# Scoobadood/TSDF

Hardware: AMD Instinct MI355X
Metric: Mvoxels/s integrate + Mrays/s raycast, 512^3 grid, 640x480 depth; 1/2/4/8 GPU (higher is better)
Workload: dtype f32

## Files before the change

### include/tsdf_amd.h

```cpp
#ifndef TSDF_AMD_H
#define TSDF_AMD_H

#include <stddef.h>
#include <stdint.h>

#ifdef __cplusplus
extern "C" {
#endif

#define TSDF_OK 0
#define TSDF_ERR_INVALID 1
#define TSDF_ERR_DEVICE 2
#define TSDF_ERR_NOMEM 3

typedef struct tsdf_volume tsdf_volume;
typedef struct tsdf_bilateral tsdf_bilateral;
typedef struct tsdf_icp tsdf_icp;

typedef struct tsdf_volume_info {
    uint32_t size[3];
    uint32_t z_begin, z_end;
    uint32_t z_store_begin, z_store_end;
    float physical_size[3];
    float voxel_size[3];
// ... 2 lines not shown
    float truncation_distance;
    float max_weight;
    float global_translation[3];
    float global_rotation[3];
    int32_t deformation_materialised;
    int32_t fast_division_verified;
} tsdf_volume_info;

typedef struct tsdf_deformation_node {
    float translation[3];
    float rotation[3];
} tsdf_deformation_node;

const char *tsdf_last_error(void);
int tsdf_device_count(int *count);
int tsdf_set_device(int device);
int tsdf_get_device(int *device);
const char *tsdf_build_arch(void);

int tsdf_device_alloc(size_t bytes, void **device_ptr);
int tsdf_device_free(void *device_ptr);
int tsdf_device_upload(void *device_dst, const void *host_src, size_t bytes);
int tsdf_device_download(void *host_dst, const void *device_src, size_t bytes);
int tsdf_stream_synchronize(void *hip_stream);

int tsdf_volume_create(uint32_t size_x, uint32_t size_y, uint32_t size_z, float physical_x,
                       float physical_y, float physical_z, tsdf_volume **out);
int tsdf_volume_create_slab(uint32_t size_x, uint32_t size_y, uint32_t size_z, float physical_x,
                            float physical_y, float physical_z, uint32_t z_begin, uint32_t z_end,
                            tsdf_volume **out);
int tsdf_volume_destroy(tsdf_volume *volume);
int tsdf_volume_set_stream(tsdf_volume *volume, void *hip_stream);
int tsdf_volume_stream(const tsdf_volume *volume, void **hip_stream);
int tsdf_volume_synchronize(const tsdf_volume *volume);
int tsdf_volume_clear(tsdf_volume *volume);
int tsdf_volume_get_info(const tsdf_volume *volume, tsdf_volume_info *info);
int tsdf_volume_set_offset(tsdf_volume *volume, float ox, float oy, float oz);

int tsdf_volume_set_header(tsdf_volume *volume, const float offset[3], float truncation_distance,
                           float max_weight, const float global_translation[3],
                           const float global_rotation[3]);

int tsdf_volume_distances(const tsdf_volume *volume, float **device_ptr);
int tsdf_volume_mark_dirty(tsdf_volume *volume);
int tsdf_volume_weights(const tsdf_volume *volume, float **device_ptr);
int tsdf_volume_weight_storage(const tsdf_volume *volume, int *bits_per_weight, int *pinned);
int tsdf_volume_set_weight_storage(tsdf_volume *volume, int bits_per_weight);
int tsdf_selftest_count_division(uint32_t b_begin, uint32_t b_end, unsigned long long *mismatches);
int tsdf_volume_deformation(tsdf_volume *volume, tsdf_deformation_node **device_ptr);
int tsdf_volume_set_distance_data(tsdf_volume *volume, const float *host);
int tsdf_volume_set_weight_data(tsdf_volume *volume, const float *host);
int tsdf_volume_set_deformation(tsdf_volume *volume, const tsdf_deformation_node *host);
int tsdf_volume_deform_points(const tsdf_volume *volume, int num_points, float *host_points);
int tsdf_volume_deform_points_device(const tsdf_volume *volume, int num_points, float *device_points);
int tsdf_volume_get_distance_data(const tsdf_volume *volume, float *host);
int tsdf_volume_get_weight_data(const tsdf_volume *volume, float *host);
int tsdf_volume_get_deformation_planes(const tsdf_volume *volume, uint32_t plane_begin, uint32_t plane_count,
                                       tsdf_deformation_node *host);
int tsdf_volume_set_offset_at_clear(tsdf_volume *volume, const float offset_at_clear[3]);

int tsdf_integrate(tsdf_volume *volume, const uint16_t *host_depth, uint32_t width, uint32_t height,
                   const float pose[16], const float inv_pose[16], const float k[9], const float kinv[9]);
int tsdf_integrate_device(tsdf_volume *volume, const uint16_t *device_depth, uint32_t width,
                          uint32_t height, const float pose[16], const float inv_pose[16],
                          const float k[9], const float kinv[9]);
int tsdf_integrate_device_tiles(tsdf_volume *volume, const uint16_t *device_depth, uint32_t width,
                                uint32_t height, const float pose[16], const float inv_pose[16],
                                const float k[9], const float kinv[9], const uint16_t *device_tile_max);
int tsdf_integrate_prepare_device_tiles(tsdf_volume *volume, const uint16_t *device_depth, uint32_t width,
                                        uint32_t height, const float pose[16], const float inv_pose[16],
                                        const float k[9], const float kinv[9], const uint16_t *device_tile_max,
                                        void *hip_stream);
int tsdf_integrate_discard_prepared(tsdf_volume *volume);
int tsdf_volume_set_timing(tsdf_volume *volume, int enabled);
int tsdf_volume_kernel_time(tsdf_volume *volume, int which, uint32_t *launches, float *average_ms);

int tsdf_volume_set_counting(tsdf_volume *volume, int enabled);
int tsdf_volume_last_updated_voxels(const tsdf_volume *volume, uint64_t *count);

int tsdf_raycast(const tsdf_volume *volume, uint32_t width, uint32_t height, const float pose[16],
                 const float kinv[9], float *host_vertices, float *host_normals);
int tsdf_raycast_device(const tsdf_volume *volume, uint32_t width, uint32_t height,
                        const float pose[16], const float kinv[9], float *device_vertices,
                        float *device_normals);
int tsdf_normals_device(uint32_t width, uint32_t height, const float *device_vertices,
                        float *device_normals, void *hip_stream);
int tsdf_vertices_to_depth_device(uint32_t width, uint32_t height, const float *device_vertices,
                                  const float inv_pose[16], uint16_t *device_depth, void *hip_stream);
int tsdf_raycast_depth_device(const tsdf_volume *volume, uint32_t width, uint32_t height, const float pose[16],
                              const float inv_pose[16], const float kinv[9], uint16_t *device_depth, float *device_vertices);
int tsdf_volume_last_raycast_kind(const tsdf_volume *volume, int *cell_parallel);
int tsdf_volume_last_cell_list(const tsdf_volume *volume, uint32_t *listed);
int tsdf_raycast_stats(const tsdf_volume *volume, uint32_t width, uint32_t height, const float pose[16],
                       const float kinv[9], uint64_t *samples, uint64_t *touched_voxels, uint64_t *hits);

int tsdf_raycast_evaluated_samples(const tsdf_volume *volume, uint32_t width, uint32_t height,
                                   const float pose[16], const float kinv[9], uint64_t *evaluated,
                                   float *host_per_ray );
int tsdf_volume_occupancy(const tsdf_volume *volume, uint64_t *occupied_bricks, uint64_t *total_bricks);
int tsdf_volume_get_occupancy_data(const tsdf_volume *volume, int force_rebuild, uint8_t *host_fine, uint8_t *host_cell,
                                   uint8_t *host_reach);

int tsdf_volume_marching_cubes(const tsdf_volume *volume, const int8_t *table, uint64_t *n_vertices, float *host_vertices,
                               uint64_t capacity);

#define TSDF_NO_HIT 0xffffffffu
typedef struct tsdf_hit_record {
    uint32_t k;
    float t;
} tsdf_hit_record;
int tsdf_raycast_slab_device(const tsdf_volume *volume, uint32_t width, uint32_t height,
                             const float pose[16], const float kinv[9], tsdf_hit_record *device_hits);
int tsdf_merge_hits_device(const tsdf_volume *volume, const tsdf_hit_record *device_hits_all, uint32_t n_slabs,
                           uint32_t width, uint32_t height, const float pose[16], const float kinv[9],
                           float *device_vertices, void *hip_stream);
int tsdf_merge_hits_normals_device(const tsdf_volume *volume, const tsdf_hit_record *device_hits_all, uint32_t n_slabs,
                                   uint32_t width, uint32_t height, const float pose[16], const float kinv[9],
                                   float *device_vertices, float *device_normals, void *hip_stream);

typedef struct tsdf_slab_exchange tsdf_slab_exchange;
#define TSDF_EXCHANGE_ID_BYTES 128
int tsdf_slab_exchange_unique_id(uint8_t id[TSDF_EXCHANGE_ID_BYTES], const char *rccl_library);
int tsdf_slab_exchange_create(int rank, int world, const uint8_t id[TSDF_EXCHANGE_ID_BYTES], const char *rccl_library,
                              tsdf_slab_exchange **out);
typedef int (*tsdf_exchange_fn)(void *user, const tsdf_hit_record *device_mine, tsdf_hit_record *device_all, uint32_t n_pixels,
                                void *hip_stream);
int tsdf_slab_exchange_create_callback(int rank, int world, tsdf_exchange_fn all_gather, void *user, tsdf_slab_exchange **out);
int tsdf_slab_exchange_create_loopback(int rank, int world, tsdf_slab_exchange **out);
int tsdf_slab_exchange_world(const tsdf_slab_exchange *exchange, int *rank, int *world);
int tsdf_slab_exchange_ranks_seen(const tsdf_slab_exchange *exchange, int *ranks);
int tsdf_slab_validate_merge(tsdf_volume *slab_volume, tsdf_slab_exchange *exchange, uint32_t width, uint32_t height,
                             const float pose[16], const float kinv[9], const float *device_merged_vertices,
                             const float *device_merged_normals, uint64_t *differing_words);
int tsdf_slab_exchange_all_gather(tsdf_slab_exchange *exchange, const tsdf_hit_record *device_mine, tsdf_hit_record *device_all,
                                  uint32_t n_pixels, void *hip_stream);
int tsdf_slab_exchange_destroy(tsdf_slab_exchange *exchange);

typedef struct tsdf_pipeline tsdf_pipeline;
typedef struct tsdf_camera_matrices {
    float pose[16], inv_pose[16], k[9], kinv[9];
} tsdf_camera_matrices;
#define TSDF_PIPELINE_OVERLAP 1
#define TSDF_PIPELINE_EQUAL_PRIORITY 2
#define TSDF_PIPELINE_EXCHANGE_STREAM 4
#define TSDF_PIPELINE_NO_TIGHTEN_AHEAD 8
int tsdf_pipeline_create(tsdf_volume *volume, const tsdf_bilateral *filter, uint32_t width, uint32_t height, int flags,
                         tsdf_slab_exchange *exchange , tsdf_pipeline **out);
int tsdf_pipeline_step(tsdf_pipeline *pipeline, const uint16_t *device_depth, const tsdf_camera_matrices *camera,
                       float *device_vertices, float *device_normals, const uint16_t *next_device_depth ,
                       const tsdf_camera_matrices *next_camera );
int tsdf_pipeline_synchronize(tsdf_pipeline *pipeline);
int tsdf_pipeline_streams(const tsdf_pipeline *pipeline, void **main_stream, void **side_stream);
int tsdf_pipeline_hit_buffers(const tsdf_pipeline *pipeline, tsdf_hit_record **device_mine, tsdf_hit_record **device_all);
int tsdf_pipeline_destroy(tsdf_pipeline *pipeline);

typedef struct tsdf_tracker tsdf_tracker;
int tsdf_tracker_create(tsdf_volume *volume, const tsdf_bilateral *filter, tsdf_icp *icp, uint32_t width, uint32_t height,
                        float depth_cutoff, int flags , tsdf_tracker **out);
int tsdf_tracker_filter(tsdf_tracker *tracker, const uint16_t *device_depth);
int tsdf_tracker_align(tsdf_tracker *tracker, const tsdf_camera_matrices *previous, double T_prev_curr[16] ,
                       float *last_error, float *last_inliers);
int tsdf_tracker_integrate(tsdf_tracker *tracker, const tsdf_camera_matrices *camera);
int tsdf_tracker_synchronize(tsdf_tracker *tracker);
int tsdf_tracker_streams(const tsdf_tracker *tracker, void **main_stream, void **side_stream);
int tsdf_tracker_buffers(const tsdf_tracker *tracker, const uint16_t **device_model, const uint16_t **device_filtered);
int tsdf_tracker_destroy(tsdf_tracker *tracker);

int tsdf_icp_create(int width, int height, float cx, float cy, float fx, float fy, float dist_thresh, float angle_thresh,
                    tsdf_icp **out);
void tsdf_icp_destroy(tsdf_icp *icp);
int tsdf_icp_set_stream(tsdf_icp *icp, void *hip_stream);
int tsdf_icp_stream(const tsdf_icp *icp, void **hip_stream);
int tsdf_icp_init(tsdf_icp *icp, int model, const uint16_t *host_depth, float depth_cutoff);
int tsdf_icp_init_device(tsdf_icp *icp, int model, const uint16_t *device_depth, float depth_cutoff);
int tsdf_icp_estimate_step(tsdf_icp *icp, int level, const float R[9], const float t[3], float A[36], float b[6],
                           float residual_inliers[2]);
int tsdf_icp_get_incremental_transformation(tsdf_icp *icp, double T_prev_curr[16], float *last_error, float *last_inliers);
int tsdf_icp_get_map(const tsdf_icp *icp, int which, int level, float *host_map);
int tsdf_icp_get_depth_level(const tsdf_icp *icp, int level, uint16_t *host_depth);

int tsdf_bilateral_create(float sigma_colour, float sigma_space, tsdf_bilateral **out);
int tsdf_bilateral_destroy(tsdf_bilateral *filter);
int tsdf_bilateral_filter_u8(const tsdf_bilateral *filter, uint8_t *host_image, int width, int height);
int tsdf_bilateral_filter_u16(const tsdf_bilateral *filter, uint16_t *host_image, int width, int height);
int tsdf_bilateral_filter_u8_device(const tsdf_bilateral *filter, const uint8_t *device_in,
                                    uint8_t *device_out, int width, int height, void *hip_stream);
int tsdf_bilateral_filter_u16_device(const tsdf_bilateral *filter, const uint16_t *device_in,
                                     uint16_t *device_out, int width, int height, void *hip_stream);
#define TSDF_DEPTH_TILE 16
int tsdf_bilateral_filter_u16_device_tiles(const tsdf_bilateral *filter, const uint16_t *device_in,
                                           uint16_t *device_out, int width, int height,
                                           uint16_t *device_tile_max, void *hip_stream);

int tsdf_measure_copy_bandwidth(size_t bytes, int reps, void *hip_stream, double *gb_per_s);
int tsdf_measure_update_bandwidth(int reps, void *hip_stream, double *gb_per_s);

#ifdef __cplusplus
}
#endif
#endif
```

### tsdf_amd/_capi.py

```python
import ctypes as C
import os

_HERE = os.path.dirname(os.path.abspath(__file__))
LIB_PATH = os.environ.get("TSDF_HIP_LIB") or os.path.join(_HERE, "lib", "libtsdf_hip.so")

TSDF_OK, TSDF_ERR_INVALID, TSDF_ERR_DEVICE, TSDF_ERR_NOMEM = 0, 1, 2, 3


class TsdfError(RuntimeError):
    """A C-ABI call failed with TSDF_ERR_DEVICE / TSDF_ERR_NOMEM."""


class VolumeInfo(C.Structure):
    _fields_ = [("size", C.c_uint32 * 3), ("z_begin", C.c_uint32), ("z_end", C.c_uint32),
                ("z_store_begin", C.c_uint32), ("z_store_end", C.c_uint32),
                ("physical_size", C.c_float * 3), ("voxel_size", C.c_float * 3), ("offset", C.c_float * 3),
                ("offset_at_clear", C.c_float * 3), ("truncation_distance", C.c_float),
                ("max_weight", C.c_float), ("global_translation", C.c_float * 3),
                ("global_rotation", C.c_float * 3), ("deformation_materialised", C.c_int32),
                ("fast_division_verified", C.c_int32)]


class CameraMatrices(C.Structure):
    _fields_ = [("pose", C.c_float * 16), ("inv_pose", C.c_float * 16), ("k", C.c_float * 9), ("kinv", C.c_float * 9)]


EXCHANGE_FN = C.CFUNCTYPE(C.c_int, C.c_void_p, C.c_void_p, C.c_void_p, C.c_uint32, C.c_void_p)


def _load():
    if not os.path.exists(LIB_PATH):
        raise ImportError(
            "tsdf_amd: %s is missing -- build it with `make hip` (or `python -c 'import __graft_entry__ as g; "
            "g.build()'`). There is no CPU fallback." % LIB_PATH)
    return C.CDLL(LIB_PATH, mode=C.RTLD_GLOBAL)


lib = _load()

_vp, _fp = C.c_void_p, C.POINTER(C.c_float)
_u32, _f, _i = C.c_uint32, C.c_float, C.c_int
_SIGS = {
    "tsdf_last_error": (C.c_char_p, []),
    "tsdf_build_arch": (C.c_char_p, []),
    "tsdf_device_count": (_i, [C.POINTER(_i)]),
    "tsdf_set_device": (_i, [_i]),
    "tsdf_get_device": (_i, [C.POINTER(_i)]),
    "tsdf_device_alloc": (_i, [C.c_size_t, C.POINTER(_vp)]),
    "tsdf_device_free": (_i, [_vp]),
    "tsdf_device_upload": (_i, [_vp, _vp, C.c_size_t]),
    "tsdf_device_download": (_i, [_vp, _vp, C.c_size_t]),
    "tsdf_stream_synchronize": (_i, [_vp]),
    "tsdf_volume_create": (_i, [_u32, _u32, _u32, _f, _f, _f, C.POINTER(_vp)]),
    "tsdf_volume_create_slab": (_i, [_u32, _u32, _u32, _f, _f, _f, _u32, _u32, C.POINTER(_vp)]),
    "tsdf_volume_destroy": (_i, [_vp]),
    "tsdf_volume_set_stream": (_i, [_vp, _vp]),
    "tsdf_volume_stream": (_i, [_vp, C.POINTER(_vp)]),
    "tsdf_volume_synchronize": (_i, [_vp]),
    "tsdf_volume_clear": (_i, [_vp]),
    "tsdf_volume_get_info": (_i, [_vp, C.POINTER(VolumeInfo)]),
    "tsdf_volume_set_offset": (_i, [_vp, _f, _f, _f]),
    "tsdf_volume_set_header": (_i, [_vp, _fp, _f, _f, _fp, _fp]),
    "tsdf_volume_mark_dirty": (_i, [_vp]),
    "tsdf_volume_distances": (_i, [_vp, C.POINTER(_vp)]),
    "tsdf_volume_weights": (_i, [_vp, C.POINTER(_vp)]),
    "tsdf_volume_weight_storage": (_i, [_vp, C.POINTER(_i), C.POINTER(_i)]),
    "tsdf_volume_last_raycast_kind": (_i, [_vp, C.POINTER(_i)]),
    "tsdf_volume_last_cell_list": (_i, [_vp, C.POINTER(C.c_uint32)]),
    "tsdf_volume_set_weight_storage": (_i, [_vp, _i]),
    "tsdf_selftest_count_division": (_i, [_u32, _u32, C.POINTER(C.c_uint64)]),
    "tsdf_volume_deformation": (_i, [_vp, C.POINTER(_vp)]),
    "tsdf_volume_set_distance_data": (_i, [_vp, _vp]),
    "tsdf_volume_set_weight_data": (_i, [_vp, _vp]),
    "tsdf_volume_set_deformation": (_i, [_vp, _vp]),
    "tsdf_volume_get_distance_data": (_i, [_vp, _vp]),
    "tsdf_measure_copy_bandwidth": (_i, [C.c_size_t, _i, _vp, C.POINTER(C.c_double)]),
    "tsdf_measure_update_bandwidth": (_i, [_i, _vp, C.POINTER(C.c_double)]),
    "tsdf_volume_get_weight_data": (_i, [_vp, _vp]),
    "tsdf_volume_get_deformation_planes": (_i, [_vp, C.c_uint32, C.c_uint32, _vp]),
    "tsdf_volume_set_offset_at_clear": (_i, [_vp, _vp]),
    "tsdf_integrate": (_i, [_vp, _vp, _u32, _u32, _fp, _fp, _fp, _fp]),
    "tsdf_integrate_device": (_i, [_vp, _vp, _u32, _u32, _fp, _fp, _fp, _fp]),
    "tsdf_integrate_device_tiles": (_i, [_vp, _vp, _u32, _u32, _fp, _fp, _fp, _fp, _vp]),
    "tsdf_integrate_prepare_device_tiles": (_i, [_vp, _vp, _u32, _u32, _fp, _fp, _fp, _fp, _vp, _vp]),
    "tsdf_integrate_discard_prepared": (_i, [_vp]),
    "tsdf_volume_set_timing": (_i, [_vp, _i]),
    "tsdf_volume_kernel_time": (_i, [_vp, _i, C.POINTER(C.c_uint32), C.POINTER(C.c_float)]),
    "tsdf_volume_set_counting": (_i, [_vp, _i]),
    "tsdf_volume_last_updated_voxels": (_i, [_vp, C.POINTER(C.c_uint64)]),
    "tsdf_raycast": (_i, [_vp, _u32, _u32, _fp, _fp, _vp, _vp]),
    "tsdf_raycast_device": (_i, [_vp, _u32, _u32, _fp, _fp, _vp, _vp]),
    "tsdf_normals_device": (_i, [_u32, _u32, _vp, _vp, _vp]),
    "tsdf_raycast_stats": (_i, [_vp, _u32, _u32, _fp, _fp, C.POINTER(C.c_uint64), C.POINTER(C.c_uint64),
                                C.POINTER(C.c_uint64)]),
    "tsdf_raycast_evaluated_samples": (_i, [_vp, _u32, _u32, _fp, _fp, C.POINTER(C.c_uint64), _vp]),
    "tsdf_volume_deform_points": (_i, [_vp, _i, _vp]),
    "tsdf_volume_deform_points_device": (_i, [_vp, _i, _vp]),
    "tsdf_volume_occupancy": (_i, [_vp, C.POINTER(C.c_uint64), C.POINTER(C.c_uint64)]),
    "tsdf_volume_get_occupancy_data": (_i, [_vp, C.c_int, _vp, _vp, _vp]),
    "tsdf_raycast_slab_device": (_i, [_vp, _u32, _u32, _fp, _fp, _vp]),
    "tsdf_vertices_to_depth_device": (_i, [_u32, _u32, _vp, _vp, _vp, _vp]),
    "tsdf_raycast_depth_device": (_i, [_vp, _u32, _u32, _fp, _fp, _fp, _vp, _vp]),
    "tsdf_volume_marching_cubes": (_i, [_vp, _vp, _vp, _vp, C.c_uint64]),
    "tsdf_merge_hits_device": (_i, [_vp, _vp, _u32, _u32, _u32, _fp, _fp, _vp, _vp]),
    "tsdf_merge_hits_normals_device": (_i, [_vp, _vp, _u32, _u32, _u32, _fp, _fp, _vp, _vp, _vp]),
    "tsdf_slab_exchange_unique_id": (_i, [_vp, C.c_char_p]),
    "tsdf_slab_exchange_create": (_i, [_i, _i, _vp, C.c_char_p, C.POINTER(_vp)]),
    "tsdf_slab_exchange_create_callback": (_i, [_i, _i, EXCHANGE_FN, _vp, C.POINTER(_vp)]),
    "tsdf_slab_exchange_create_loopback": (_i, [_i, _i, C.POINTER(_vp)]),
    "tsdf_slab_exchange_world": (_i, [_vp, C.POINTER(_i), C.POINTER(_i)]),
    "tsdf_slab_exchange_ranks_seen": (_i, [_vp, C.POINTER(_i)]),
    "tsdf_slab_validate_merge": (_i, [_vp, _vp, _u32, _u32, _fp, _fp, _vp, _vp, C.POINTER(C.c_uint64)]),
    "tsdf_slab_exchange_all_gather": (_i, [_vp, _vp, _vp, _u32, _vp]),
    "tsdf_slab_exchange_destroy": (_i, [_vp]),
    "tsdf_pipeline_create": (_i, [_vp, _vp, _u32, _u32, _i, _vp, C.POINTER(_vp)]),
    "tsdf_pipeline_step": (_i, [_vp, _vp, C.POINTER(CameraMatrices), _vp, _vp, _vp, C.POINTER(CameraMatrices)]),
    "tsdf_pipeline_synchronize": (_i, [_vp]),
    "tsdf_pipeline_streams": (_i, [_vp, C.POINTER(_vp), C.POINTER(_vp)]),
    "tsdf_pipeline_hit_buffers": (_i, [_vp, C.POINTER(_vp), C.POINTER(_vp)]),
    "tsdf_pipeline_destroy": (_i, [_vp]),
    "tsdf_tracker_create": (_i, [_vp, _vp, _vp, _u32, _u32, _f, _i, C.POINTER(_vp)]),
    "tsdf_tracker_filter": (_i, [_vp, _vp]),
    "tsdf_tracker_align": (_i, [_vp, C.POINTER(CameraMatrices), _vp, C.POINTER(C.c_float), C.POINTER(C.c_float)]),
    "tsdf_tracker_integrate": (_i, [_vp, C.POINTER(CameraMatrices)]),
    "tsdf_tracker_synchronize": (_i, [_vp]),
    "tsdf_tracker_streams": (_i, [_vp, C.POINTER(_vp), C.POINTER(_vp)]),
    "tsdf_tracker_buffers": (_i, [_vp, C.POINTER(_vp), C.POINTER(_vp)]),
    "tsdf_tracker_destroy": (_i, [_vp]),
    "tsdf_icp_create": (_i, [_i, _i, _f, _f, _f, _f, _f, _f, C.POINTER(_vp)]),
    "tsdf_icp_destroy": (None, [_vp]),
    "tsdf_icp_set_stream": (_i, [_vp, _vp]),
    "tsdf_icp_stream": (_i, [_vp, C.POINTER(_vp)]),
    "tsdf_icp_init": (_i, [_vp, _i, _vp, _f]),
    "tsdf_icp_init_device": (_i, [_vp, _i, _vp, _f]),
    "tsdf_icp_estimate_step": (_i, [_vp, _i, _vp, _vp, _vp, _vp, _vp]),
    "tsdf_icp_get_incremental_transformation": (_i, [_vp, _vp, C.POINTER(C.c_float), C.POINTER(C.c_float)]),
    "tsdf_icp_get_map": (_i, [_vp, _i, _i, _vp]),
    "tsdf_icp_get_depth_level": (_i, [_vp, _i, _vp]),
    "tsdf_bilateral_create": (_i, [_f, _f, C.POINTER(_vp)]),
    "tsdf_bilateral_destroy": (_i, [_vp]),
    "tsdf_bilateral_filter_u8": (_i, [_vp, _vp, _i, _i]),
    "tsdf_bilateral_filter_u16": (_i, [_vp, _vp, _i, _i]),
    "tsdf_bilateral_filter_u8_device": (_i, [_vp, _vp, _vp, _i, _i, _vp]),
    "tsdf_bilateral_filter_u16_device": (_i, [_vp, _vp, _vp, _i, _i, _vp]),
    "tsdf_bilateral_filter_u16_device_tiles": (_i, [_vp, _vp, _vp, _i, _i, _vp, _vp]),
}
EXPORTS = tuple(_SIGS)
for _name, (_res, _args) in _SIGS.items():
    _fn = getattr(lib, _name)
    _fn.restype = _res
    _fn.argtypes = _args


def last_error():
    return lib.tsdf_last_error().decode("utf-8", "replace")


def check(rc):
    if rc == TSDF_OK:
        return
    msg = last_error()
    if rc == TSDF_ERR_INVALID:
        raise ValueError(msg)
    if rc == TSDF_ERR_NOMEM:
        raise MemoryError(msg)
    raise TsdfError(msg)

HOST_LIB_PATH = os.path.join(_HERE, "lib", "libtsdf_host.so")
if not os.path.exists(HOST_LIB_PATH):
    raise ImportError("tsdf_amd: %s is missing -- build it with `make host`." % HOST_LIB_PATH)
host = C.CDLL(HOST_LIB_PATH)
_ip = C.POINTER(C.c_int)
_HOST_SIGS = {
    "tsdf_camera_create": (_vp, [_f, _f, _f, _f]),
    "tsdf_camera_destroy": (None, [_vp]),
    "tsdf_camera_get": (None, [_vp, _fp, _fp, _fp, _fp]),
    "tsdf_camera_set_pose": (None, [_vp, _fp]),
    "tsdf_camera_set_pose_tum": (None, [_vp, _fp]),
    "tsdf_camera_move_to": (None, [_vp, _f, _f, _f]),
    "tsdf_camera_look_at": (None, [_vp, _f, _f, _f]),
    "tsdf_camera_world_to_camera": (None, [_vp, _fp, _fp]),
    "tsdf_camera_camera_to_world": (None, [_vp, _fp, _fp]),
    "tsdf_camera_world_to_pixel": (None, [_vp, _fp, _ip]),
    "tsdf_camera_pixel_to_image_plane": (None, [_vp, C.c_uint16, C.c_uint16, _fp]),
    "tsdf_camera_image_plane_to_pixel": (None, [_vp, _fp, _ip]),
    "tsdf_host_marching_cubes_c": (C.c_size_t, [_vp, C.c_uint, C.c_uint, C.c_uint, _vp, _vp, _vp, C.c_size_t]),
    "tsdf_host_mc_table": (None, [_vp]),
    "tsdf_host_tum_open": (_vp, [C.c_char_p]),
    "tsdf_host_tum_next": (_i, [_vp, _vp, C.c_size_t, C.POINTER(C.c_uint), _fp]),
    "tsdf_host_tum_close": (None, [_vp]),
    "tsdf_host_block_loader_parse": (_i, [C.c_char_p, _vp, _vp, _vp, _vp, C.c_size_t]),
    "tsdf_host_write_ply": (None, [C.c_char_p, _vp, C.c_size_t, _vp, C.c_size_t]),
    "tsdf_host_read_nyu_depth_map": (C.c_size_t, [C.c_char_p, C.POINTER(C.c_uint), _vp, C.c_size_t]),
    "tsdf_host_match_file_name": (_i, [C.c_char_p, _i, C.c_char_p, C.c_char_p, C.c_char_p]),
    "tsdf_host_process_file_by_lines": (C.c_size_t, [C.c_char_p, C.POINTER(_i), C.c_char_p, C.c_size_t]),
    "tsdf_host_read_last_line": (C.c_size_t, [C.c_char_p, C.c_char_p, C.POINTER(_i), C.c_char_p, C.c_size_t]),
    "tsdf_host_files_in_directory": (C.c_size_t, [C.c_char_p, C.c_char_p, _i, C.c_char_p, C.c_char_p, C.c_char_p, C.c_size_t]),
    "tsdf_host_file_exists": (_i, [C.c_char_p, C.POINTER(_i)]),
}
for _name, (_res, _args) in _HOST_SIGS.items():
    _fn = getattr(host, _name)
    _fn.restype = _res
    _fn.argtypes = _args
```

### tsdf_amd/csrc/bilateral.hip

```cpp
#include <cmath>
#include <cstdlib>
#include <new>
#include <type_traits>
#include <vector>

#include "common.hpp"

namespace tsdf {

constexpr int kBTile = 16;
constexpr int kMaxRadius = 24;

constexpr int kSimLds = 4096;

__device__ inline void bilateral_tap(float weight, double intensity, float &sum, float &total_weight) {
    sum = (float)__builtin_fma((double)weight, intensity, (double)sum);
    total_weight = total_weight + weight;
}

__device__ inline unsigned sad_u32(unsigned a, unsigned b) {
    unsigned d;
    asm("v_sad_u32 %0, %1, %2, 0" : "=v"(d) : "v"(a), "v"(b));
    return d;
}

template <typename PIX, int R>
__global__ __launch_bounds__(256) void bilateral_kernel(const PIX *__restrict__ in, PIX *__restrict__ out,
                                                        int width, int height, int radius_arg,
                                                        const float *__restrict__ kernel,
                                                        const float *__restrict__ similarity,
                                                        uint16_t *__restrict__ tile_max) {
    constexpr bool STAGED = R > 0;
    __shared__ unsigned wg_max;
    if (threadIdx.x == 0) wg_max = 0u;
    extern __shared__ __align__(16) unsigned char smem_raw[];
    const int radius = R > 0 ? R : radius_arg;
    const int n = 2 * radius + 1;
    const int span = kBTile + 2 * radius;
    double *tile_d = reinterpret_cast<double *>(smem_raw);
    float *kern_lds = reinterpret_cast<float *>(tile_d + (STAGED ? 0 : span * span));
    float *sim_lds = kern_lds + n * n;
    uint32_t *tile4 = reinterpret_cast<uint32_t *>(sim_lds + (STAGED ? kSimLds : 0));
    const int tx0 = blockIdx.x * kBTile - radius;
    const int ty0 = blockIdx.y * kBTile - radius;
    {
        constexpr int kAhead = 4;
        for (int i0 = threadIdx.x; i0 < span * span; i0 += 256 * kAhead) {
            unsigned v_[kAhead];
#pragma unroll
            for (int u = 0; u < kAhead; u++) {
                const int i = min(i0 + u * 256, span * span - 1);
                const int ly = i / span, lx = i - ly * span;
                const int gx = min(max(tx0 + lx, 0), width - 1), gy = min(max(ty0 + ly, 0), height - 1);
                v_[u] = in[(size_t)gy * width + gx];
            }
#pragma unroll
            for (int u = 0; u < kAhead; u++) {
                const int i = i0 + u * 256;
                const int ly = i / span, lx = i - ly * span;
                const int gx = tx0 + lx, gy = ty0 + ly;
                const unsigned v = (gx >= 0 && gx < width && gy >= 0 && gy < height) ? v_[u] : 0u;
                if (i < span * span) {
                    tile4[i] = v * 4u;
                    if (!STAGED) tile_d[i] = (double)(int)v;
                }
            }
        }
    }
    {
        const int n_sim = !STAGED ? 0 : (sizeof(PIX) == 1 ? 256 : kSimLds);
        constexpr int kAhead = 16;
        float k_ = 0.0f;
        if ((int)threadIdx.x < n * n) k_ = kernel[threadIdx.x];
        for (int i0 = threadIdx.x; i0 < n_sim; i0 += 256 * kAhead) {
            float s_[kAhead];
#pragma unroll
            for (int u = 0; u < kAhead; u++) s_[u] = similarity[min(i0 + u * 256, n_sim - 1)];
#pragma unroll
            for (int u = 0; u < kAhead; u++)
                if (i0 + u * 256 < n_sim) sim_lds[i0 + u * 256] = s_[u];
        }
        if ((int)threadIdx.x < n * n) kern_lds[threadIdx.x] = k_;
        for (int i = threadIdx.x + 256; i < n * n; i += 256) kern_lds[i] = kernel[i];
    }
    __syncthreads();

    const int lx = threadIdx.x & 15, ly = threadIdx.x >> 4;
    const int x = blockIdx.x * kBTile + lx;
    const int y = blockIdx.y * kBTile + ly;
    const uint32_t *t0 = tile4 + ly * span + lx;
    const double *d0 = tile_d + ly * span + lx;
    const unsigned current4 = t0[radius * span + radius];
    float total_weight = 0;
    float sum = 0;
    const int wy0 = (blockIdx.y * kBTile + (ly & ~3)) - radius;
    const bool interior = tx0 >= 0 && tx0 + span <= width && wy0 >= 0 && wy0 + 4 + 2 * radius <= height;
    const bool inside = x < width && y < height;
    const int i0 = max(0, radius - x), i1 = inside ? min(n - 1, width - 1 - x + radius) : -1;
    const int j0 = max(0, radius - y), j1 = inside ? min(n - 1, height - 1 - y + radius) : -1;
    const int nyv = j1 - j0 + 1;

    if (STAGED) {
        constexpr int N = 2 * (R > 0 ? R : 1) + 1;
        constexpr int SPAN = kBTile + 2 * (R > 0 ? R : 1);
        constexpr unsigned kStagedBytes = (sizeof(PIX) == 1 ? 256u : (unsigned)kSimLds) * 4u;
        constexpr int NA = (N + 1) / 2, NB = N - NA;
        float w_a[NA], w_b[NB > 0 ? NB : 1];
        unsigned v_a[NA], v_b[NB > 0 ? NB : 1];
        auto fetch = [&](const int i, auto first_row, auto count, float *w, unsigned *v4, const auto rim) {
            constexpr int J0 = decltype(first_row)::value, CNT = decltype(count)::value;
            unsigned delta4[CNT];
#pragma unroll
            for (int j = 0; j < CNT; j++) {
                v4[j] = t0[(J0 + j) * SPAN + i];
                delta4[j] = sad_u32(v4[j], current4);
            }
#pragma unroll
            for (int j = 0; j < CNT; j++)
                w[j] = *reinterpret_cast<const float *>(reinterpret_cast<const char *>(sim_lds) + delta4[j]);
            if (sizeof(PIX) != 1) {
                unsigned big = delta4[0];
#pragma unroll
                for (int j = 1; j < CNT; j++) big = max(big, delta4[j]);
                if (__builtin_expect(big >= kStagedBytes, 0)) {
#pragma unroll
                    for (int j = 0; j < CNT; j++)
                        if (delta4[j] >= kStagedBytes) {
                            const char *p = reinterpret_cast<const char *>(similarity) + delta4[j];
                            asm volatile("global_load_dword %0, %1, off\n\ts_waitcnt vmcnt(0)" : "=v"(w[j]) : "v"(p) : "memory");
                        }
                }
            }
            if (!decltype(rim)::value) {
#pragma unroll
                for (int j = 0; j < CNT; j++) w[j] = kernel[i * N + J0 + j] * w[j];
            } else {
                const bool col_ok = i >= i0 && i <= i1;
                const int base = (i - i0) * nyv - j0;
#pragma unroll
                for (int j = 0; j < CNT; j++) {
                    const bool ok = col_ok && J0 + j >= j0 && J0 + j <= j1;
                    const float k = kern_lds[(base + J0 + j) & (ok ? 255 : 0)];
                    w[j] = __builtin_bit_cast(float, __builtin_bit_cast(unsigned, k * w[j]) & (ok ? 0xffffffffu : 0u));
                }
            }
        };
        auto chain = [&](const int i, auto first_row, auto count, const float *w, const unsigned *v4) {
            constexpr int CNT = decltype(count)::value;
            (void)i;
#pragma unroll
            for (int j = 0; j < CNT; j++) bilateral_tap(w[j], (double)v4[j], sum, total_weight);
        };
        using Lo = std::integral_constant<int, 0>;
        using Hi = std::integral_constant<int, NA>;
        using CntA = std::integral_constant<int, NA>;
        using CntB = std::integral_constant<int, NB>;
        auto run = [&](const auto rim) {
            fetch(0, Lo{}, CntA{}, w_a, v_a, rim);
#pragma unroll 1
            for (int i = 0; i + 1 < N; i++) {
                fetch(i, Hi{}, CntB{}, w_b, v_b, rim);
                chain(i, Lo{}, CntA{}, w_a, v_a);
                fetch(i + 1, Lo{}, CntA{}, w_a, v_a, rim);
                chain(i, Hi{}, CntB{}, w_b, v_b);
            }
            fetch(N - 1, Hi{}, CntB{}, w_b, v_b, rim);
            chain(N - 1, Lo{}, CntA{}, w_a, v_a);
            chain(N - 1, Hi{}, CntB{}, w_b, v_b);
        };
        if (interior) {
            run(std::false_type{});
        } else {
            __builtin_amdgcn_s_setprio(3);
            run(std::true_type{});
        }
        sum *= 0.25f;
    } else {
#pragma unroll 1
        for (int i = 0; i < n; i++) {
            const bool col_ok = i >= i0 && i <= i1;
            const int base = (i - i0) * nyv - j0;
#pragma unroll 1
            for (int j = 0; j < n; j++) {
                const int o = j * span + i;
                const bool ok = col_ok && j >= j0 && j <= j1;
                const unsigned delta = sad_u32(t0[o], current4) >> 2;
                const float k = kern_lds[ok ? base + j : 0];
                const float weight = ok ? k * similarity[delta] : 0.0f;
                bilateral_tap(weight, d0[o], sum, total_weight);
            }
        }
    }
    const PIX filtered = inside ? (PIX)(int)floorf(sum / total_weight) : (PIX)0;
    if (inside) out[(size_t)y * width + x] = filtered;
    if (tile_max) {
        unsigned m = (unsigned)filtered;
        for (int o = 32; o > 0; o >>= 1) m = max(m, (unsigned)__shfl_down((int)m, o));
        if ((threadIdx.x & 63) == 0 && m) atomicMax(&wg_max, m);
        __syncthreads();
        if (threadIdx.x == 0) tile_max[blockIdx.y * gridDim.x + blockIdx.x] = (uint16_t)wg_max;
    }
}

template <typename PIX>
static int launch_bilateral(const tsdf_bilateral *f, const PIX *in, PIX *out, int width, int height, hipStream_t s,
                            uint16_t *tile_max = nullptr) {
    dim3 grid((width + kBTile - 1) / kBTile, (height + kBTile - 1) / kBTile);
    const int span = kBTile + 2 * f->radius, n = 2 * f->radius + 1;
    const bool staged = f->radius == 7 && f->scale_exact;
    size_t smem = (size_t)span * span * ((staged ? 0 : sizeof(double)) + sizeof(uint32_t)) + (size_t)n * n * sizeof(float) +
                  (staged ? kSimLds * sizeof(float) : 0);
    if (staged)
        hipLaunchKernelGGL((bilateral_kernel<PIX, 7>), grid, dim3(256), smem, s, in, out, width, height, f->radius, f->kernel_dev,
                           f->similarity_dev, tile_max);
    else
        hipLaunchKernelGGL((bilateral_kernel<PIX, 0>), grid, dim3(256), smem, s, in, out, width, height, f->radius, f->kernel_dev,
                           f->similarity_dev, tile_max);
    TSDF_HIP(hipGetLastError(), "bilateral filter kernel failed");
    return TSDF_OK;
}

template <typename PIX>
static int filter_host(const tsdf_bilateral *cf, PIX *host_image, int width, int height) {
    TSDF_REQUIRE(cf && host_image && width > 0 && height > 0, "tsdf_bilateral_filter: bad argument");
    tsdf_bilateral *f = const_cast<tsdf_bilateral *>(cf);
    size_t bytes = (size_t)width * height * sizeof(PIX);
    if (f->img_cap < bytes) {
        if (f->img_in) (void)hipFree(f->img_in);
        if (f->img_out) (void)hipFree(f->img_out);
        f->img_in = f->img_out = nullptr;
        f->img_cap = 0;
        TSDF_HIP(hipMalloc(&f->img_in, bytes), "bilateral image alloc");
        TSDF_HIP(hipMalloc(&f->img_out, bytes), "bilateral image alloc");
        f->img_cap = bytes;
    }
    TSDF_HIP(hipMemcpy(f->img_in, host_image, bytes, hipMemcpyHostToDevice), "bilateral H2D");
    int rc = launch_bilateral<PIX>(f, (const PIX *)f->img_in, (PIX *)f->img_out, width, height, nullptr);
    if (rc != TSDF_OK) return rc;
    TSDF_HIP(hipMemcpy(host_image, f->img_out, bytes, hipMemcpyDeviceToHost), "bilateral D2H");
    return TSDF_OK;
}

}

using namespace tsdf;

extern "C" {

int tsdf_bilateral_create(float sigma_colour, float sigma_space, tsdf_bilateral **out) {
    TSDF_REQUIRE(out, "tsdf_bilateral_create: null out pointer");
    *out = nullptr;
    TSDF_REQUIRE(sigma_colour > 0 && sigma_space > 0, "tsdf_bilateral_create: sigmas must be positive");
    int kernel_radius = (int)std::ceil(sigma_space * 1.5f);
    TSDF_REQUIRE(kernel_radius <= kMaxRadius, "tsdf_bilateral_create: kernel radius %d exceeds %d", kernel_radius, kMaxRadius);
    float inv_sigma_colour_squared = 1.0f / (sigma_colour * sigma_colour);
    float inv_sigma_space_squared = 1.0f / (sigma_space * sigma_space);
    int kernel_size = kernel_radius * 2 + 1;
    int center = (kernel_size - 1) / 2;
    std::vector<float> kernel((size_t)kernel_size * kernel_size);
    int idx = 0;
    for (int x = -center; x < kernel_size - center; x++) {
        for (int y = -center; y < kernel_size - center; y++) {
            float dist_squared = (float)(x * x + y * y);
            kernel[idx] = std::exp(-dist_squared * inv_sigma_space_squared);
            idx++;
        }
    }
    std::vector<float> similarity(65536);
    for (int i = 0; i < 65536; i++) similarity[i] = std::exp(-i * inv_sigma_colour_squared);

    tsdf_bilateral *f = new (std::nothrow) tsdf_bilateral();
    if (!f) {
        set_error("out of host memory");
        return TSDF_ERR_NOMEM;
    }
    memset(f, 0, sizeof(*f));
    f->sigma_colour = sigma_colour;
    f->sigma_space = sigma_space;
    f->radius = kernel_radius;
    {
        float min_k = 0.0f, min_s = 0.0f;
        for (float k : kernel) if (k > 0.0f && (min_k == 0.0f || k < min_k)) min_k = k;
        for (float x : similarity) if (x > 0.0f && (min_s == 0.0f || x < min_s)) min_s = x;
        f->scale_exact = (min_k * min_s >= 0x1p-120f) ? 1 : 0;
    }
    hipError_t e = hipGetDevice(&f->device);
    if (e == hipSuccess) e = hipMalloc((void **)&f->kernel_dev, kernel.size() * sizeof(float));
    if (e == hipSuccess) e = hipMalloc((void **)&f->similarity_dev, similarity.size() * sizeof(float));

    if (e == hipSuccess) e = hipMemcpy(f->kernel_dev, kernel.data(), kernel.size() * sizeof(float), hipMemcpyHostToDevice);
    if (e == hipSuccess) e = hipMemcpy(f->similarity_dev, similarity.data(), similarity.size() * sizeof(float), hipMemcpyHostToDevice);
    if (e != hipSuccess) {
        int rc = hip_fail(e, "bilateral filter tables");
        tsdf_bilateral_destroy(f);
        return rc;
    }
    *out = f;
    return TSDF_OK;
}

int tsdf_bilateral_destroy(tsdf_bilateral *f) {
    if (!f) return TSDF_OK;
    if (f->kernel_dev) (void)hipFree(f->kernel_dev);
    if (f->similarity_dev) (void)hipFree(f->similarity_dev);
    if (f->img_in) (void)hipFree(f->img_in);
    if (f->img_out) (void)hipFree(f->img_out);
    delete f;
    return TSDF_OK;
}

int tsdf_bilateral_filter_u8(const tsdf_bilateral *f, uint8_t *host_image, int width, int height) {
    return filter_host<uint8_t>(f, host_image, width, height);
}

int tsdf_bilateral_filter_u16(const tsdf_bilateral *f, uint16_t *host_image, int width, int height) {
    return filter_host<uint16_t>(f, host_image, width, height);
}

int tsdf_bilateral_filter_u8_device(const tsdf_bilateral *f, const uint8_t *in, uint8_t *out, int width,
                                    int height, void *hip_stream) {
    TSDF_REQUIRE(f && in && out && in != out && width > 0 && height > 0, "tsdf_bilateral_filter: bad argument");
    return launch_bilateral<uint8_t>(f, in, out, width, height, (hipStream_t)hip_stream);
}

int tsdf_bilateral_filter_u16_device(const tsdf_bilateral *f, const uint16_t *in, uint16_t *out, int width,
                                     int height, void *hip_stream) {
    TSDF_REQUIRE(f && in && out && in != out && width > 0 && height > 0, "tsdf_bilateral_filter: bad argument");
    return launch_bilateral<uint16_t>(f, in, out, width, height, (hipStream_t)hip_stream);
}

int tsdf_bilateral_filter_u16_device_tiles(const tsdf_bilateral *f, const uint16_t *in, uint16_t *out, int width,
                                           int height, uint16_t *tile_max, void *hip_stream) {
    TSDF_REQUIRE(f && in && out && in != out && tile_max && width > 0 && height > 0, "tsdf_bilateral_filter: bad argument");
    static_assert(kBTile == TSDF_DEPTH_TILE, "the filter's workgroup tile is the depth tile of integrate's culling");
    return launch_bilateral<uint16_t>(f, in, out, width, height, (hipStream_t)hip_stream, tile_max);
}

}
```

### tsdf_amd/csrc/common.hpp

```cpp
#pragma once

#include <hip/hip_runtime.h>
#include <hip/hip_ext.h>

#include <cstdarg>
#include <cstdint>
#include <cstdio>
#include <cstring>
#include <vector>

#include "tsdf_amd.h"

struct tsdf_volume;

namespace tsdf {

struct PreparedCull {
    const uint16_t *depth, *tile_max;
    uint32_t width, height;
    float inv_pose[16], k[9], kinv[9];
};

#ifndef TSDF_CHUNK_Z
#define TSDF_CHUNK_Z 32
#endif
constexpr int kIntBrickX = 64, kIntBrickY = 4, kIntBrickZ = TSDF_CHUNK_Z;

void set_error(const char *fmt, ...);
int hip_fail(hipError_t e, const char *what);
struct Tuning {
    int ray_segments;
    int ray_slab_ranges;
    int ray_trip_budget;
    int ray_tail_lanes;
    int ray_tail_grid;
    int ray_tail_piece;
    int ray_range_order;
    int ray_tile_map;
    int ray_learned_order;
    int ray_heavy_passes;
    int ray_cells;
    int ray_cells_limit;
    float ray_cells_footprint;
    int ray_cells_pairs;
    int ray_cells_look;
    int ray_cells_grid;
    int ray_cells_sort;
    int ray_chooser;
    int ray_entry_bound;
    int icp_persistent;
    int occ_rebuild_period;
    int occ_scan_all;
    int reach_lds;
    int int_grid_per_cu;
    int weight_pack;
    int pipe_release;
    int pipe_word_release;
    int pipe_host_wait;
    int event_scope;
    int timing_bracket;
    int verbose;
    int debug_rays;
};
const Tuning &tuning();
inline unsigned stream_order_event_flags() {
    const int scope = tuning().event_scope;
    return hipEventDisableTiming | (scope == 1 ? hipEventReleaseToDevice : scope == 2 ? hipEventDisableSystemFence : 0u);
}
int occupancy_rebuild(struct ::tsdf_volume *v);
int occupancy_join(struct ::tsdf_volume *v);
int occupancy_tighten_on(struct ::tsdf_volume *v, hipStream_t stream);
struct EntryParams;
int occupancy_refresh(struct ::tsdf_volume *v, const EntryParams *entry = nullptr);
bool raycast_takes_cells(const struct ::tsdf_volume *v, uint32_t width, uint32_t height, const float pose[16], const float kinv[9]);
int occupancy_flags_refresh(struct ::tsdf_volume *v);
int build_t_table(struct ::tsdf_volume *v);
bool timing_pair(struct ::tsdf_volume *v, int which, hipEvent_t *start, hipEvent_t *stop);
void timing_begin(struct ::tsdf_volume *v, int which);
void timing_end(struct ::tsdf_volume *v, int which);
#define TSDF_LAUNCH_TIMED_LDS(v, which, kernel, grid, block, lds_bytes, ...)                                            \
    do {                                                                                                                \
        hipEvent_t ts0__ = nullptr, ts1__ = nullptr;                                                                    \
        if (tsdf::timing_pair(v, which, &ts0__, &ts1__))                                                                \
            hipExtLaunchKernelGGL(kernel, grid, block, (uint32_t)(lds_bytes), (v)->stream, ts0__, ts1__, 0, __VA_ARGS__); \
        else {                                                                                                          \
            tsdf::timing_begin(v, which);                                                                               \
            hipLaunchKernelGGL(kernel, grid, block, (uint32_t)(lds_bytes), (v)->stream, __VA_ARGS__);                   \
            tsdf::timing_end(v, which);                                                                                 \
        }                                                                                                               \
    } while (0)
#define TSDF_LAUNCH_TIMED(v, which, kernel, grid, block, ...) TSDF_LAUNCH_TIMED_LDS(v, which, kernel, grid, block, 0, __VA_ARGS__)
int verify_fast_division(struct ::tsdf_volume *v);
int weights_create(struct ::tsdf_volume *v);
void weights_destroy(struct ::tsdf_volume *v);
int weights_clear(struct ::tsdf_volume *v);
int weights_require_f32(struct ::tsdf_volume *v);
int weights_make_room(struct ::tsdf_volume *v);
int weights_upload(struct ::tsdf_volume *v, const float *host);
int weights_download(const struct ::tsdf_volume *v, float *host);

#define TSDF_HIP(call, what)                                  \
    do {                                                      \
        hipError_t e__ = (call);                              \
        if (e__ != hipSuccess) return tsdf::hip_fail(e__, what); \
    } while (0)

#define TSDF_REQUIRE(cond, ...)              \
    do {                                     \
        if (!(cond)) {                       \
            tsdf::set_error(__VA_ARGS__);    \
            return TSDF_ERR_INVALID;         \
        }                                    \
    } while (0)

struct Mat44 {
    float m11, m21, m31, m41;
    float m12, m22, m32, m42;
    float m13, m23, m33, m43;
    float m14, m24, m34, m44;
};
struct Mat33 {
    float m11, m21, m31;
    float m12, m22, m32;
    float m13, m23, m33;
};
struct F3 {
    float x, y, z;
};

struct Geom {
    uint32_t X, Y, Z;
    uint32_t z_store_begin;
    uint32_t z_store_end;
    F3 vs;
    F3 offset;
    F3 offset_clear;
    F3 phys;
    float trunc;
};

constexpr float kFastDivMin = 1.0e-30f;
constexpr int kBrick = 4;
constexpr int kBrickShift = 2;
constexpr int kBrickGrow = 2;
constexpr int kReachLevels = 5;
constexpr int kSlabSkip = 32;
constexpr int kSlabSkipShift = 5;
struct OccGrid {
    uint8_t *fine;
    uint8_t *cell;
    uint8_t *reach;
    uint32_t nbx, nby, nbz;
    float tau;
    float flat_lo, flat_hi;
    __host__ __device__ bool in_rim_zone(uint32_t v, uint32_t nb) const { return v < (uint32_t)(kBrick + kBrickGrow) || v + kBrickGrow >= (uint32_t)kBrick * (nb - 1u); }
    __host__ __device__ bool not_flat(float d) const { return !(d >= flat_lo && d <= flat_hi); }
    __host__ __device__ size_t fine_count() const { return (size_t)nbx * nby * nbz; }
};

constexpr int kEntryTile = 16;
constexpr uint32_t kEntryFar = 0x7f7f7f7fu;
struct EntryParams {
    float r[3][4];
    float r_scale;
    float k[2][3];
    F3 vs, offset;
    uint32_t width, height, tiles_x, tiles_y;
    float slack_z;
    float z_clip;
    float z_near;
    uint32_t cell_pairs;
    uint32_t *ztile;
    uint32_t *ztile_next;
    uint32_t units_x, units_y, units_z;
};

__host__ __device__ inline int f2i_sat(float f) {
    if (f != f) return 0;
    if (f >= 2147483648.0f) return 2147483647;
    if (f <= -2147483648.0f) return (-2147483647 - 1);
    return (int)f;
}

}

namespace tsdf {
struct CastChooser {
    float ms[2];
    uint32_t seen[2];
    uint64_t measured_at[2];
    uint64_t casts, next_trial;
    uint32_t gap;
    bool pending, pending_trial, blocked;
    int pending_kind, last_kind, trial_kind, trial_left;
    hipEvent_t ev[2];
    float trial_origin[3], trial_axis[3];
};
}

struct tsdf_volume {
    tsdf::Geom g;
    uint32_t z_begin, z_end;
    float max_weight;
    float global_translation[3];
    float global_rotation[3];
    int device;
    hipStream_t stream;
    const void *attached;
    float *dist;
    float *weight;
    uint32_t *wpacked;
    int wmode;
    uint32_t weight_bound;
    int weight_pinned;
    tsdf_deformation_node *nodes;
    uint16_t *depth_buf;
    size_t depth_cap;
    float *vert_buf;
    float *norm_buf;
    size_t ray_cap;
    uint32_t *release_word;
    uint32_t release_value;
    hipEvent_t after_bulk;
    uint64_t *ray_best;
    size_t ray_best_cap;
    int ray_best_side;
    size_t ray_best_pixels;
    int ray_best_dirty;
    void *tail_entries;
    uint32_t *tail_count;
    size_t tail_cap;
    void *cell_rays;
    size_t cell_rays_cap;
    uint32_t *cell_bricks;
    uint32_t *cell_count_scratch;
    tsdf::CastChooser chooser;
    int cell_recount_wait;
    size_t cell_bricks_cap;
    uint32_t *cell_cast_host;
    int last_cast_cells;
    uint8_t *ray_heavy;
    uint32_t *ray_order;
    uint32_t ray_order_tiles, ray_order_ranges;
    int ray_order_valid;
    uint32_t *ztile;
    size_t ztile_words;
    int ztile_side;
    float *t_table;
    int fast_div;
    unsigned long long fast_div_mismatches;
    tsdf::OccGrid occ;
    int occ_dirty;
    int occ_tighten_due;
    hipEvent_t occ_tightened;
    int occ_tighten_pending;
    int reach_dirty;
    uint16_t *occ_bits;
    uint8_t *occ_rim_bits;
    uint8_t *touched;
    uint32_t touched_nx, touched_ny, touched_nz;
    int occ_scan_all;
    uint32_t integrations_since_rebuild;
    uint32_t integrations_total;
    uint32_t *brick_list;
    size_t brick_list_cap;
    tsdf::PreparedCull prepared;
    int prepared_valid;
    uint32_t brick_count_side;
    uint32_t *brick_boxes;
    size_t brick_box_cap;
    uint16_t *tile_max;
    size_t tile_max_cap;
    float *plane_const;
    uint16_t *depth_pad;
    uint32_t depth_pad_w, depth_pad_h;
    int timing;
    uint32_t timing_launches[3];
    std::vector<hipEvent_t> *tev[3];
    int counting;
    unsigned long long *counter_dev;
    uint64_t last_updated;
    size_t resident_voxels() const { return (size_t)g.X * g.Y * (g.z_store_end - g.z_store_begin); }
};

struct tsdf_bilateral {
    float sigma_colour, sigma_space;
    int radius;
    int device;
    int scale_exact;
    float *kernel_dev;
    float *similarity_dev;
    void *img_in;
    void *img_out;
    size_t img_cap;
};
```

### tsdf_amd/csrc/pipeline.hip

```cpp
#include <dlfcn.h>

#include <new>

#include <cstdlib>
#include <cstring>

#include <algorithm>
#include <vector>

#include "common.hpp"

namespace {
struct NcclUniqueId {
    char internal[128];
};
typedef int (*nccl_get_unique_id_fn)(NcclUniqueId *);
typedef int (*nccl_comm_init_rank_fn)(void **comm, int nranks, NcclUniqueId id, int rank);
typedef int (*nccl_all_gather_fn)(const void *send, void *recv, size_t count, int dtype, void *comm, hipStream_t stream);
typedef int (*nccl_comm_destroy_fn)(void *comm);
typedef const char *(*nccl_get_error_string_fn)(int);
typedef int (*nccl_comm_count_fn)(const void *comm, int *count);
constexpr int kNcclUint8 = 1;

struct Rccl {
    void *dl = nullptr;
    nccl_get_unique_id_fn get_unique_id = nullptr;
    nccl_comm_init_rank_fn comm_init_rank = nullptr;
    nccl_all_gather_fn all_gather = nullptr;
    nccl_comm_destroy_fn comm_destroy = nullptr;
    nccl_get_error_string_fn error_string = nullptr;
    nccl_comm_count_fn comm_count = nullptr;
};

int open_rccl(const char *library, Rccl &r) {
    const char *fallbacks[] = {"librccl.so", "librccl.so.1", "/opt/rocm/lib/librccl.so.1", "/opt/rocm/lib/librccl.so"};
    if (library && *library) {
        r.dl = dlopen(library, RTLD_NOW | RTLD_LOCAL);
    } else {
        for (const char *f : fallbacks)
            if (!r.dl) r.dl = dlopen(f, RTLD_NOW | RTLD_LOCAL | RTLD_NOLOAD);
        for (const char *f : fallbacks)
            if (!r.dl) r.dl = dlopen(f, RTLD_NOW | RTLD_LOCAL);
    }
    if (!r.dl) {
        tsdf::set_error("slab exchange: cannot open librccl (%s)", dlerror());
        return TSDF_ERR_DEVICE;
    }
    r.get_unique_id = (nccl_get_unique_id_fn)dlsym(r.dl, "ncclGetUniqueId");
    r.comm_init_rank = (nccl_comm_init_rank_fn)dlsym(r.dl, "ncclCommInitRank");
    r.all_gather = (nccl_all_gather_fn)dlsym(r.dl, "ncclAllGather");
    r.comm_destroy = (nccl_comm_destroy_fn)dlsym(r.dl, "ncclCommDestroy");
    r.error_string = (nccl_get_error_string_fn)dlsym(r.dl, "ncclGetErrorString");
    r.comm_count = (nccl_comm_count_fn)dlsym(r.dl, "ncclCommCount");
    if (!r.get_unique_id || !r.comm_init_rank || !r.all_gather || !r.comm_destroy || !r.error_string) {
        tsdf::set_error("slab exchange: librccl lacks a symbol (ncclGetUniqueId / ncclCommInitRank / ncclAllGather / ncclCommDestroy / ncclGetErrorString)");
        dlclose(r.dl);
        r.dl = nullptr;
        return TSDF_ERR_DEVICE;
    }
    return TSDF_OK;
}

int rccl_fail(const Rccl &r, int rc, const char *what) {
    tsdf::set_error("%s failed: %s", what, r.error_string ? r.error_string(rc) : "?");
    return TSDF_ERR_DEVICE;
}
}

struct tsdf_slab_exchange {
    Rccl rccl;
    void *comm;
    int rank, world;
    tsdf_exchange_fn callback;
    void *user;
};

struct tsdf_pipeline {
    tsdf_volume *volume;
    const tsdf_bilateral *filter;
    tsdf_slab_exchange *exchange;
    uint32_t width, height;
    int flags;
    hipStream_t main, side, xstream;
    hipStream_t volume_stream_before;
    uint16_t *filtered[2], *tile_max[2];
    hipEvent_t done[2], ready[2];
    hipEvent_t bulk;
    uint32_t *release_word;
    uint32_t release_seq;
    hipEvent_t cast, merged;
    bool merged_pending;
    const uint16_t *ahead_depth;
    int ahead_buf;
    bool ahead_culled;
    uint64_t frames;
    tsdf_hit_record *hits_mine, *hits_all;
};

struct tsdf_tracker {
    tsdf_volume *volume;
    const tsdf_bilateral *filter;
    tsdf_icp *icp;
    uint32_t width, height;
    float depth_cutoff;
    hipStream_t main, side;
    hipStream_t volume_stream_before, icp_stream_before;
    uint16_t *filtered[2], *tile_max[2], *model;
    hipEvent_t integrated[2];
    hipEvent_t ready;
    bool ready_pending;
    int cur;
    bool have_frame;
    uint64_t frames;
};

using namespace tsdf;

static int run_filter(tsdf_pipeline *p, const uint16_t *depth, int b, hipStream_t s) {
    return tsdf_bilateral_filter_u16_device_tiles(p->filter, depth, p->filtered[b], (int)p->width, (int)p->height, p->tile_max[b], s);
}

extern "C" {

int tsdf_slab_exchange_unique_id(uint8_t id[TSDF_EXCHANGE_ID_BYTES], const char *rccl_library) {
    TSDF_REQUIRE(id, "tsdf_slab_exchange_unique_id: null argument");
    Rccl r;
    int rc = open_rccl(rccl_library, r);
    if (rc != TSDF_OK) return rc;
    NcclUniqueId u;
    memset(&u, 0, sizeof(u));
    const int e = r.get_unique_id(&u);
    if (e != 0) return rccl_fail(r, e, "ncclGetUniqueId");
    static_assert(sizeof(u) == TSDF_EXCHANGE_ID_BYTES, "unique id size");
    memcpy(id, &u, sizeof(u));
    return TSDF_OK;
}

int tsdf_slab_exchange_create(int rank, int world, const uint8_t id[TSDF_EXCHANGE_ID_BYTES], const char *rccl_library,
                              tsdf_slab_exchange **out) {
    TSDF_REQUIRE(out && id, "tsdf_slab_exchange_create: null argument");
    *out = nullptr;
    TSDF_REQUIRE(world >= 1 && rank >= 0 && rank < world, "tsdf_slab_exchange_create: rank %d outside a world of %d", rank, world);
    tsdf_slab_exchange *x = new (std::nothrow) tsdf_slab_exchange();
    if (!x) {
        set_error("out of host memory");
        return TSDF_ERR_NOMEM;
    }
    x->comm = nullptr;
    x->rank = rank;
    x->world = world;
    x->callback = nullptr;
    x->user = nullptr;
    int rc = open_rccl(rccl_library, x->rccl);
    if (rc != TSDF_OK) {
        delete x;
        return rc;
    }
    NcclUniqueId u;
    memcpy(&u, id, sizeof(u));
    const int e = x->rccl.comm_init_rank(&x->comm, world, u, rank);
    if (e != 0) {
        rc = rccl_fail(x->rccl, e, "ncclCommInitRank");
        delete x;
        return rc;
    }
    *out = x;
    return TSDF_OK;
}

int tsdf_slab_exchange_create_callback(int rank, int world, tsdf_exchange_fn all_gather, void *user, tsdf_slab_exchange **out) {
    TSDF_REQUIRE(out && all_gather, "tsdf_slab_exchange_create_callback: null argument");
    *out = nullptr;
    TSDF_REQUIRE(world >= 1 && rank >= 0 && rank < world, "tsdf_slab_exchange_create_callback: rank %d outside a world of %d", rank, world);
    tsdf_slab_exchange *x = new (std::nothrow) tsdf_slab_exchange();
    if (!x) {
        set_error("out of host memory");
        return TSDF_ERR_NOMEM;
    }
    x->comm = nullptr;
    x->rank = rank;
    x->world = world;
    x->callback = all_gather;
    x->user = user;
    *out = x;
    return TSDF_OK;
}

static int loopback_all_gather(void *user, const tsdf_hit_record *device_mine, tsdf_hit_record *device_all, uint32_t n_pixels, void *hip_stream) {
    const tsdf_slab_exchange *x = static_cast<const tsdf_slab_exchange *>(user);
    for (int r = 0; r < x->world; r++)
        if (hipMemcpyAsync(device_all + (size_t)r * n_pixels, device_mine, (size_t)n_pixels * sizeof(tsdf_hit_record), hipMemcpyDeviceToDevice,
                           (hipStream_t)hip_stream) != hipSuccess)
            return TSDF_ERR_DEVICE;
    return TSDF_OK;
}

int tsdf_slab_exchange_create_loopback(int rank, int world, tsdf_slab_exchange **out) {
    const int rc = tsdf_slab_exchange_create_callback(rank, world, loopback_all_gather, nullptr, out);
    if (rc == TSDF_OK) (*out)->user = *out;
    return rc;
}

int tsdf_slab_exchange_world(const tsdf_slab_exchange *x, int *rank, int *world) {
    TSDF_REQUIRE(x, "null exchange");
    if (rank) *rank = x->rank;
    if (world) *world = x->world;
    return TSDF_OK;
}

int tsdf_slab_exchange_ranks_seen(const tsdf_slab_exchange *x, int *ranks) {
    TSDF_REQUIRE(x && ranks, "null argument");
    *ranks = x->world;
    if (!x->callback && x->comm && x->rccl.comm_count) {
        int n = 0;
        const int e = x->rccl.comm_count(x->comm, &n);
        if (e != 0) return rccl_fail(x->rccl, e, "ncclCommCount");
        *ranks = n;
    }
    return TSDF_OK;
}

namespace {
__global__ __launch_bounds__(256) void count_differing_words_kernel(const float *__restrict__ a, const float *__restrict__ b, size_t n,
                                                                    unsigned long long *__restrict__ count) {
    unsigned long long c = 0;
    for (size_t i = (size_t)blockIdx.x * 256 + threadIdx.x; i < n; i += (size_t)gridDim.x * 256) {
        const float x = a[i], y = b[i];
        c += (__float_as_uint(x) != __float_as_uint(y) && !(x != x && y != y)) ? 1ull : 0ull;
    }
    for (int o = 32; o > 0; o >>= 1) c += __shfl_down(c, o);
    if ((threadIdx.x & 63u) == 0 && c) atomicAdd(count, c);
}
}

int tsdf_slab_validate_merge(tsdf_volume *slab, tsdf_slab_exchange *x, uint32_t width, uint32_t height, const float pose[16],
                             const float kinv[9], const float *device_merged_vertices, const float *device_merged_normals,
                             uint64_t *differing_words) {
    TSDF_REQUIRE(slab && x && pose && kinv && device_merged_vertices && differing_words, "tsdf_slab_validate_merge: null argument");
    *differing_words = ~0ull;
    const Geom &g = slab->g;
    const size_t xy = (size_t)g.X * g.Y;
    hipStream_t s = slab->stream;
    int rc = occupancy_join(slab);
    if (rc != TSDF_OK) return rc;
    tsdf_hit_record *ranges_dev = nullptr;
    std::vector<tsdf_hit_record> ranges((size_t)x->world);
// ... 81 lines not shown
        memcpy(&zb, reinterpret_cast<const char *>(&ranges[r]), 4);
        memcpy(&ze, reinterpret_cast<const char *>(&ranges[r]) + 4, 4);
        e = hipMemcpyAsync(whole->dist + (size_t)zb * xy, reinterpret_cast<const float *>(recv + (size_t)r * per_rank), (size_t)(ze - zb) * xy * sizeof(float),
                           hipMemcpyDeviceToDevice, s);
    }
    if (e != hipSuccess) { cleanup(); return hip_fail(e, "validate merge: assembling the volume"); }
    rc = tsdf_volume_mark_dirty(whole);
    if (rc == TSDF_OK) rc = tsdf_raycast_device(whole, width, height, pose, kinv, V, device_merged_normals ? N : nullptr);
    if (rc != TSDF_OK) { cleanup(); return rc; }
    hipLaunchKernelGGL(count_differing_words_kernel, dim3(256), dim3(256), 0, s, V, device_merged_vertices, words, count_dev);
    if (device_merged_normals) hipLaunchKernelGGL(count_differing_words_kernel, dim3(256), dim3(256), 0, s, N, device_merged_normals, words, count_dev);
    unsigned long long n_diff = 0;
    e = hipGetLastError();
    if (e == hipSuccess) e = hipMemcpyAsync(&n_diff, count_dev, sizeof(n_diff), hipMemcpyDeviceToHost, s);
    if (e == hipSuccess) e = hipStreamSynchronize(s);
    cleanup();
    if (e != hipSuccess) return hip_fail(e, "validate merge: comparing the pictures");
    *differing_words = n_diff;
    return TSDF_OK;
}

int tsdf_slab_exchange_all_gather(tsdf_slab_exchange *x, const tsdf_hit_record *device_mine, tsdf_hit_record *device_all,
                                  uint32_t n_pixels, void *hip_stream) {
    TSDF_REQUIRE(x && device_mine && device_all && n_pixels > 0, "tsdf_slab_exchange_all_gather: bad argument");
    if (x->callback) {
        const int rc = x->callback(x->user, device_mine, device_all, n_pixels, hip_stream);
        if (rc != TSDF_OK) {
            set_error("slab exchange: the caller's all-gather returned %d", rc);
            return TSDF_ERR_DEVICE;
        }
        return TSDF_OK;
    }
    const int e = x->rccl.all_gather(device_mine, device_all, (size_t)n_pixels * sizeof(tsdf_hit_record), kNcclUint8, x->comm,
                                     (hipStream_t)hip_stream);
    if (e != 0) return rccl_fail(x->rccl, e, "ncclAllGather");
    return TSDF_OK;
}

int tsdf_slab_exchange_destroy(tsdf_slab_exchange *x) {
    if (!x) return TSDF_OK;
    if (x->comm && x->rccl.comm_destroy) (void)x->rccl.comm_destroy(x->comm);
    delete x;
    return TSDF_OK;
}

int tsdf_pipeline_destroy(tsdf_pipeline *p) {
    if (!p) return TSDF_OK;
    if (p->main) (void)hipStreamSynchronize(p->main);
    if (p->side) (void)hipStreamSynchronize(p->side);
    if (p->xstream) (void)hipStreamSynchronize(p->xstream);
    if (p->volume && p->volume->attached == p) {
        (void)tsdf_integrate_discard_prepared(p->volume);
        (void)tsdf_volume_set_stream(p->volume, p->volume_stream_before);
        p->volume->attached = nullptr;
    }
    for (int b = 0; b < 2; b++) {
        if (p->filtered[b]) (void)hipFree(p->filtered[b]);
        if (p->tile_max[b]) (void)hipFree(p->tile_max[b]);
        if (p->done[b]) (void)hipEventDestroy(p->done[b]);
        if (p->ready[b]) (void)hipEventDestroy(p->ready[b]);
    }
    if (p->bulk) (void)hipEventDestroy(p->bulk);
    if (p->cast) (void)hipEventDestroy(p->cast);
    if (p->merged) (void)hipEventDestroy(p->merged);
    if (p->hits_mine) (void)hipFree(p->hits_mine);
    if (p->hits_all) (void)hipFree(p->hits_all);
    if (p->release_word) (void)hipFree(p->release_word);
    if (p->side) (void)hipStreamDestroy(p->side);
    if (p->xstream) (void)hipStreamDestroy(p->xstream);
    if (p->main) (void)hipStreamDestroy(p->main);
    delete p;
    return TSDF_OK;
}

int tsdf_pipeline_create(tsdf_volume *volume, const tsdf_bilateral *filter, uint32_t width, uint32_t height, int flags,
                         tsdf_slab_exchange *exchange, tsdf_pipeline **out) {
    TSDF_REQUIRE(out, "tsdf_pipeline_create: null out pointer");
    *out = nullptr;
    TSDF_REQUIRE(volume && filter && width > 0 && height > 0 && width <= 65535 && height <= 65535, "tsdf_pipeline_create: bad argument");
    const bool slab = volume->z_begin != 0 || volume->z_end != volume->g.Z;
    TSDF_REQUIRE(exchange || !slab, "tsdf_pipeline_create: a Z-slab needs a slab exchange");
    TSDF_REQUIRE(!volume->attached, "tsdf_pipeline_create: the volume is attached to another pipeline or tracker (destroy that one first)");
    tsdf_pipeline *p = new (std::nothrow) tsdf_pipeline();
    if (!p) {
        set_error("out of host memory");
        return TSDF_ERR_NOMEM;
    }
    memset(p, 0, sizeof(*p));
    p->volume = volume;
    p->filter = filter;
    p->exchange = exchange;
    p->width = width;
    p->height = height;
    p->flags = flags;
    p->volume_stream_before = volume->stream;
    int least = 0, greatest = 0;
    hipError_t e = hipDeviceGetStreamPriorityRange(&least, &greatest);
    const bool overlap = (flags & TSDF_PIPELINE_OVERLAP) != 0;
    const bool equal = (flags & TSDF_PIPELINE_EQUAL_PRIORITY) != 0 || exchange != nullptr || !overlap;
    const int normal = (greatest <= 0 && 0 <= least) ? 0 : least;
    if (e == hipSuccess) e = hipStreamCreateWithPriority(&p->main, hipStreamNonBlocking, equal ? normal : greatest);
    if (e == hipSuccess && overlap) e = hipStreamCreateWithPriority(&p->side, hipStreamNonBlocking, normal);
    if (e == hipSuccess && exchange && (flags & TSDF_PIPELINE_EXCHANGE_STREAM)) e = hipStreamCreateWithPriority(&p->xstream, hipStreamNonBlocking, normal);
    const size_t n = (size_t)width * height;
    const size_t tiles = (size_t)((width + TSDF_DEPTH_TILE - 1) / TSDF_DEPTH_TILE) * ((height + TSDF_DEPTH_TILE - 1) / TSDF_DEPTH_TILE);
    for (int b = 0; b < 2 && e == hipSuccess; b++) {
        e = hipMalloc((void **)&p->filtered[b], n * sizeof(uint16_t));
        if (e == hipSuccess) e = hipMalloc((void **)&p->tile_max[b], tiles * sizeof(uint16_t));
        if (e == hipSuccess) e = hipEventCreateWithFlags(&p->done[b], stream_order_event_flags());
        if (e == hipSuccess) e = hipEventCreateWithFlags(&p->ready[b], stream_order_event_flags());
    }
    if (e == hipSuccess && overlap) e = hipEventCreateWithFlags(&p->bulk, stream_order_event_flags());
    if (e == hipSuccess && overlap && !exchange && tuning().pipe_word_release) {
        if (hipExtMallocWithFlags((void **)&p->release_word, 2 * sizeof(uint32_t), hipMallocSignalMemory) != hipSuccess) {
            (void)hipGetLastError();
            p->release_word = nullptr;
        } else if (hipMemset(p->release_word, 0, 2 * sizeof(uint32_t)) != hipSuccess) {
            (void)hipFree(p->release_word);
            p->release_word = nullptr;
        }
    }
    if (e == hipSuccess && p->xstream) e = hipEventCreateWithFlags(&p->cast, hipEventDisableTiming);
    if (e == hipSuccess && p->xstream) e = hipEventCreateWithFlags(&p->merged, hipEventDisableTiming);
    if (e == hipSuccess && exchange) {
        e = hipMalloc((void **)&p->hits_mine, n * sizeof(tsdf_hit_record));
        if (e == hipSuccess) e = hipMalloc((void **)&p->hits_all, n * sizeof(tsdf_hit_record) * (size_t)exchange->world);
    }
    if (e != hipSuccess) {
        const int rc = hip_fail(e, "tsdf_pipeline_create");
        tsdf_pipeline_destroy(p);
        return rc;
    }
    (void)hipStreamSynchronize(volume->stream);
    (void)tsdf_volume_set_stream(volume, p->main);
    volume->attached = p;
    *out = p;
    return TSDF_OK;
}

int tsdf_pipeline_streams(const tsdf_pipeline *p, void **main_stream, void **side_stream) {
    TSDF_REQUIRE(p, "null pipeline");
    if (main_stream) *main_stream = p->main;
    if (side_stream) *side_stream = p->side;
    return TSDF_OK;
}

int tsdf_pipeline_hit_buffers(const tsdf_pipeline *p, tsdf_hit_record **device_mine, tsdf_hit_record **device_all) {
    TSDF_REQUIRE(p, "null pipeline");
    if (device_mine) *device_mine = p->hits_mine;
    if (device_all) *device_all = p->hits_all;
    return TSDF_OK;
}

int tsdf_pipeline_step(tsdf_pipeline *p, const uint16_t *device_depth, const tsdf_camera_matrices *cam, float *device_vertices,
                       float *device_normals, const uint16_t *next_device_depth, const tsdf_camera_matrices *next_cam) {
    TSDF_REQUIRE(p && device_depth && cam && device_vertices, "tsdf_pipeline_step: null argument");
    const uint32_t W = p->width, H = p->height;
    const int b = (int)(p->frames & 1u);
    int rc;
    const bool early_filter = p->side && next_device_depth && !p->exchange && tuning().pipe_release == 2;
    if (early_filter) {
        TSDF_HIP(hipEventRecord(p->bulk, p->main), "pipeline: previous step done");
        TSDF_HIP(hipStreamWaitEvent(p->side, p->bulk, 0), "pipeline: release the next frame's filter");
        rc = run_filter(p, next_device_depth, 1 - b, p->side);
        if (rc != TSDF_OK) return rc;
    }
    if (p->ahead_depth && p->ahead_depth == device_depth && p->ahead_buf == b) {
        if (hipEventQuery(p->ready[b]) != hipSuccess) {
            if (tuning().pipe_host_wait) TSDF_HIP(hipEventSynchronize(p->ready[b]), "pipeline: wait for the frame filtered ahead");
            else TSDF_HIP(hipStreamWaitEvent(p->main, p->ready[b], 0), "pipeline: wait for the frame filtered ahead");
        }
    } else {
        if (p->ahead_depth) {
            TSDF_HIP(hipStreamWaitEvent(p->main, p->ready[p->ahead_buf], 0), "pipeline: wait for the side stream");
            (void)tsdf_integrate_discard_prepared(p->volume);
        }
        rc = run_filter(p, device_depth, b, p->main);
        if (rc != TSDF_OK) return rc;
    }
    p->ahead_depth = nullptr;
    rc = tsdf_integrate_device_tiles(p->volume, p->filtered[b], W, H, cam->pose, cam->inv_pose, cam->k, cam->kinv, p->tile_max[b]);
    if (rc != TSDF_OK) return rc;
    bool late_release = false;
    bool by_word = false;
    struct WordGuard {
        tsdf_pipeline *p = nullptr;
        ~WordGuard() {
            if (!p || !p->volume->release_word) return;
            p->volume->release_word = nullptr;
            if (hipStreamWriteValue32(p->main, p->release_word, p->release_seq, 0) != hipSuccess) {
                (void)hipGetLastError();
                set_error("tsdf_pipeline_step: the release word could not be stored; the side stream is left waiting (destroy the pipeline)");
            }
        }
    } word_guard;
    auto filter_ahead = [&](hipEvent_t release) -> int {
        if (by_word) TSDF_HIP(hipStreamWaitValue32(p->side, p->release_word, p->release_seq, hipStreamWaitValueGte, 0xffffffffu), "pipeline: release the next frame's filter");
        else TSDF_HIP(hipStreamWaitEvent(p->side, release, 0), "pipeline: release the next frame's filter");
        int rc_ = early_filter ? TSDF_OK : run_filter(p, next_device_depth, 1 - b, p->side);
        if (rc_ != TSDF_OK) return rc_;
        if (next_cam) {
            rc_ = tsdf_integrate_prepare_device_tiles(p->volume, p->filtered[1 - b], W, H, next_cam->pose, next_cam->inv_pose, next_cam->k,
                                                      next_cam->kinv, p->tile_max[1 - b], p->side);
            if (rc_ != TSDF_OK) return rc_;
        }
        TSDF_HIP(hipEventRecord(p->ready[1 - b], p->side), "pipeline: next frame ready");
        p->ahead_depth = next_device_depth;
        p->ahead_buf = 1 - b;
        return TSDF_OK;
    };
    if (p->side) {
        const bool tighten_ahead = p->volume->occ_tighten_due && !p->volume->occ_dirty && !(p->flags & TSDF_PIPELINE_NO_TIGHTEN_AHEAD);
        by_word = p->release_word && next_device_depth && !p->exchange && !tighten_ahead && tuning().pipe_release == 0 &&
                  raycast_takes_cells(p->volume, W, H, cam->pose, cam->kinv);
        if (by_word) {
            p->release_seq++;
            p->volume->release_word = p->release_word;
            p->volume->release_value = p->release_seq;
            word_guard.p = p;
        } else {
            TSDF_HIP(hipEventRecord(p->done[b], p->main), "pipeline: integrate done");
        }
        if (p->volume->occ_tighten_due && !p->volume->occ_dirty && !(p->flags & TSDF_PIPELINE_NO_TIGHTEN_AHEAD)) {
            TSDF_HIP(hipStreamWaitEvent(p->side, p->done[b], 0), "pipeline: release the occupancy rebuild");
            rc = occupancy_tighten_on(p->volume, p->side);
            if (rc != TSDF_OK) return rc;
        }
        late_release = next_device_depth && !p->exchange && tuning().pipe_release == 1;
        if (next_device_depth && !late_release) {
            rc = filter_ahead(p->done[b]);
            if (rc != TSDF_OK) return rc;
        }
    }
    if (!p->exchange) {
        p->volume->after_bulk = late_release ? p->bulk : nullptr;
        rc = tsdf_raycast_device(p->volume, W, H, cam->pose, cam->kinv, device_vertices, device_normals);
        p->volume->after_bulk = nullptr;
        if (rc != TSDF_OK) return rc;
        if (late_release) {
            rc = filter_ahead(p->bulk);
            if (rc != TSDF_OK) return rc;
        }
    } else {
        if (p->xstream && p->merged_pending)
            TSDF_HIP(hipStreamWaitEvent(p->main, p->merged, 0), "pipeline: wait for the previous exchange");
        rc = tsdf_raycast_slab_device(p->volume, W, H, cam->pose, cam->kinv, p->hits_mine);
        if (rc != TSDF_OK) return rc;
        hipStream_t xs = p->main;
        if (p->xstream) {
            TSDF_HIP(hipEventRecord(p->cast, p->main), "pipeline: slab cast done");
            TSDF_HIP(hipStreamWaitEvent(p->xstream, p->cast, 0), "pipeline: exchange after the slab cast");
            xs = p->xstream;
        }
        rc = tsdf_slab_exchange_all_gather(p->exchange, p->hits_mine, p->hits_all, W * H, xs);
        if (rc != TSDF_OK) return rc;
        if (device_normals)
            rc = tsdf_merge_hits_normals_device(p->volume, p->hits_all, (uint32_t)p->exchange->world, W, H, cam->pose, cam->kinv, device_vertices,
                                                device_normals, xs);
        else
            rc = tsdf_merge_hits_device(p->volume, p->hits_all, (uint32_t)p->exchange->world, W, H, cam->pose, cam->kinv, device_vertices, xs);
        if (rc != TSDF_OK) return rc;
        if (p->xstream) {
            TSDF_HIP(hipEventRecord(p->merged, p->xstream), "pipeline: merge done");
            p->merged_pending = true;
        }
    }
    p->frames++;
    return TSDF_OK;
}

int tsdf_pipeline_synchronize(tsdf_pipeline *p) {
    TSDF_REQUIRE(p, "null pipeline");
    TSDF_HIP(hipStreamSynchronize(p->main), "pipeline synchronize");
    if (p->side) TSDF_HIP(hipStreamSynchronize(p->side), "pipeline synchronize");
    if (p->xstream) TSDF_HIP(hipStreamSynchronize(p->xstream), "pipeline synchronize");
    return TSDF_OK;
}

int tsdf_tracker_destroy(tsdf_tracker *t) {
    if (!t) return TSDF_OK;
    if (t->main) (void)hipStreamSynchronize(t->main);
    if (t->side) (void)hipStreamSynchronize(t->side);
    if (t->volume && t->volume->attached == t) {
        (void)tsdf_volume_set_stream(t->volume, t->volume_stream_before);
        t->volume->attached = nullptr;
        if (t->icp) (void)tsdf_icp_set_stream(t->icp, t->icp_stream_before);
    }
    for (int b = 0; b < 2; b++) {
        if (t->filtered[b]) (void)hipFree(t->filtered[b]);
        if (t->tile_max[b]) (void)hipFree(t->tile_max[b]);
        if (t->integrated[b]) (void)hipEventDestroy(t->integrated[b]);
    }
    if (t->ready) (void)hipEventDestroy(t->ready);
    if (t->model) (void)hipFree(t->model);
    if (t->side) (void)hipStreamDestroy(t->side);
    if (t->main) (void)hipStreamDestroy(t->main);
    delete t;
    return TSDF_OK;
}

int tsdf_tracker_create(tsdf_volume *volume, const tsdf_bilateral *filter, tsdf_icp *icp, uint32_t width, uint32_t height,
                        float depth_cutoff, int flags, tsdf_tracker **out) {
    TSDF_REQUIRE(out, "tsdf_tracker_create: null out pointer");
    *out = nullptr;
    TSDF_REQUIRE(volume && filter && icp && width > 0 && height > 0 && width <= 65535 && height <= 65535, "tsdf_tracker_create: bad argument");
    TSDF_REQUIRE(volume->z_begin == 0 && volume->z_end == volume->g.Z, "tsdf_tracker_create: tracking needs a whole volume");
    TSDF_REQUIRE(!volume->attached, "tsdf_tracker_create: the volume is attached to another pipeline or tracker (destroy that one first)");
    tsdf_tracker *t = new (std::nothrow) tsdf_tracker();
    if (!t) {
        set_error("out of host memory");
        return TSDF_ERR_NOMEM;
    }
    memset(t, 0, sizeof(*t));
    t->filter = filter;
    t->width = width;
    t->height = height;
    t->depth_cutoff = depth_cutoff;
    t->volume_stream_before = volume->stream;
    int least = 0, greatest = 0;
    hipError_t e = hipDeviceGetStreamPriorityRange(&least, &greatest);
    const bool overlap = (flags & TSDF_PIPELINE_OVERLAP) != 0;
    const int normal = (greatest <= 0 && 0 <= least) ? 0 : least;
    if (e == hipSuccess) e = hipStreamCreateWithPriority(&t->main, hipStreamNonBlocking, overlap ? greatest : normal);
    if (e == hipSuccess && overlap) e = hipStreamCreateWithPriority(&t->side, hipStreamNonBlocking, normal);
    const size_t n = (size_t)width * height;
    const size_t tiles = (size_t)((width + TSDF_DEPTH_TILE - 1) / TSDF_DEPTH_TILE) * ((height + TSDF_DEPTH_TILE - 1) / TSDF_DEPTH_TILE);
    for (int b = 0; b < 2 && e == hipSuccess; b++) {
        e = hipMalloc((void **)&t->filtered[b], n * sizeof(uint16_t));
        if (e == hipSuccess) e = hipMalloc((void **)&t->tile_max[b], tiles * sizeof(uint16_t));
        if (e == hipSuccess) e = hipEventCreateWithFlags(&t->integrated[b], stream_order_event_flags());
    }
    if (e == hipSuccess) e = hipEventCreateWithFlags(&t->ready, stream_order_event_flags());
    if (e == hipSuccess) e = hipMalloc((void **)&t->model, n * sizeof(uint16_t));
    if (e != hipSuccess) {
        const int rc = hip_fail(e, "tsdf_tracker_create");
        tsdf_tracker_destroy(t);
        return rc;
    }
    (void)hipStreamSynchronize(volume->stream);
    t->volume = volume;
    t->icp = icp;
    {
        void *before = nullptr;
        (void)tsdf_icp_stream(icp, &before);
        t->icp_stream_before = (hipStream_t)before;
    }
    (void)tsdf_volume_set_stream(volume, t->main);
    (void)tsdf_icp_set_stream(icp, t->main);
    volume->attached = t;
    *out = t;
    return TSDF_OK;
}

int tsdf_tracker_streams(const tsdf_tracker *t, void **main_stream, void **side_stream) {
    TSDF_REQUIRE(t, "null tracker");
    if (main_stream) *main_stream = t->main;
    if (side_stream) *side_stream = t->side;
    return TSDF_OK;
}

int tsdf_tracker_buffers(const tsdf_tracker *t, const uint16_t **device_model, const uint16_t **device_filtered) {
    TSDF_REQUIRE(t, "null tracker");
    if (device_model) *device_model = t->model;
    if (device_filtered) *device_filtered = t->filtered[t->cur];
    return TSDF_OK;
}

int tsdf_tracker_filter(tsdf_tracker *t, const uint16_t *device_depth) {
    TSDF_REQUIRE(t && device_depth, "tsdf_tracker_filter: null argument");
    const int b = (int)(t->frames & 1u);
    const hipStream_t s = t->side ? t->side : t->main;
    if (t->side) TSDF_HIP(hipStreamWaitEvent(t->side, t->integrated[b], 0), "tracker: the frame buffer is free");
    int rc = tsdf_bilateral_filter_u16_device_tiles(t->filter, device_depth, t->filtered[b], (int)t->width, (int)t->height, t->tile_max[b], s);
    if (rc != TSDF_OK) return rc;
    if (t->frames > 0) {
        (void)tsdf_icp_set_stream(t->icp, s);
        rc = tsdf_icp_init_device(t->icp, 0, t->filtered[b], t->depth_cutoff);
        (void)tsdf_icp_set_stream(t->icp, t->main);
        if (rc != TSDF_OK) return rc;
    }
    if (t->side) {
        TSDF_HIP(hipEventRecord(t->ready, t->side), "tracker: frame ready");
        t->ready_pending = true;
    }
    t->cur = b;
    t->have_frame = true;
    return TSDF_OK;
}

static int tracker_join(tsdf_tracker *t) {
    if (t->ready_pending) {
        TSDF_HIP(hipStreamWaitEvent(t->main, t->ready, 0), "tracker: wait for the filtered frame");
        t->ready_pending = false;
// ... 41 lines not shown
```

### tsdf_amd/csrc/raycast.hip

```cpp
#include <algorithm>
#include <cmath>
#include <cstdlib>

#include "common.hpp"

namespace tsdf {

struct InvDiv {
    float b, y;
};

struct TriConst {
    float max_x, max_y, max_z;
    float clamp_x, clamp_y, clamp_z;
    InvDiv dx, dy, dz;
    uint32_t row, plane;
};
__host__ __device__ inline TriConst make_tri_const(const Geom &g) {
    TriConst c;
    c.max_x = g.X * g.vs.x;
    c.max_y = g.Y * g.vs.y;
    c.max_z = g.Z * g.vs.z;
    c.clamp_x = c.max_x - (g.vs.x / 10.0f);
    c.clamp_y = c.max_y - (g.vs.y / 10.0f);
    c.clamp_z = c.max_z - (g.vs.z / 10.0f);
    c.dx = {g.vs.x, 1.0f / g.vs.x};
    c.dy = {g.vs.y, 1.0f / g.vs.y};
    c.dz = {g.vs.z, 1.0f / g.vs.z};
    c.row = g.X;
    c.plane = g.X * g.Y;
    return c;
}

struct RayParams {
    F3 origin;
    Mat33 rot;
    Mat33 kinv;
    F3 space_min;
    F3 space_max;
    uint32_t width, height;
    uint32_t own_lo, own_hi;
    uint32_t seg_len;
    uint32_t slab_ranges;
    uint32_t tile_map;
    uint32_t range_order;
    TriConst tc;
    const uint32_t *ztile;
    uint32_t ztile_pitch, ztile_count;
};

template <bool FASTDIV>
__device__ inline float div_by(float a, const InvDiv &d) {
    if (FASTDIV) {
        const float mag = fabsf(a);
        const bool verified = mag >= kFastDivMin && mag < INFINITY;
        const float q0 = a * d.y;
        const float r = __builtin_fmaf(-d.b, q0, a);
        float q = __builtin_fmaf(r, d.y, q0);
        if (__builtin_expect(__ballot(!verified) != 0ull, 0)) {
            if (!verified) q = a / d.b;
        }
        return q;
    }
    return a / d.b;
}

template <bool SLAB, bool STATS, bool FASTDIV>
__device__ inline float trilinear(float px, float py, float pz, const float *__restrict__ dist, const Geom &g,
                                  const TriConst &tc, const RayParams &rp, bool &owned,
                                  unsigned int *__restrict__ touched) {
    float ax = px, ay = py, az = pz;
    if (px >= tc.max_x) ax = tc.clamp_x;
    if (py >= tc.max_y) ay = tc.clamp_y;
    if (pz >= tc.max_z) az = tc.clamp_z;
    if (px < 0.0f) ax = 0.0f;
    if (py < 0.0f) ay = 0.0f;
    if (pz < 0.0f) az = 0.0f;

    int vx = f2i_sat(floorf(div_by<FASTDIV>(ax, tc.dx)));
    int vy = f2i_sat(floorf(div_by<FASTDIV>(ay, tc.dy)));
    int vz = f2i_sat(floorf(div_by<FASTDIV>(az, tc.dz)));

    owned = true;
    if (vx < 0 || vy < 0 || vz < 0 || (uint32_t)vx >= g.X || (uint32_t)vy >= g.Y || (uint32_t)vz >= g.Z) {
        return NAN;
    }

    float ccx = (vx + 0.5f) * g.vs.x + 0.0f;
    float ccy = (vy + 0.5f) * g.vs.y + 0.0f;
    float ccz = (vz + 0.5f) * g.vs.z + 0.0f;

    int lx = (px < ccx) ? vx - 1 : vx;
    int ly = (py < ccy) ? vy - 1 : vy;
    int lz = (pz < ccz) ? vz - 1 : vz;
    lx = max(lx, 0);
    ly = max(ly, 0);
    lz = max(lz, 0);

    if (SLAB) {
        if (!((uint32_t)lz >= rp.own_lo && (uint32_t)lz < rp.own_hi)) {
            owned = false;
            return NAN;
        }
    }

    float lcx = (lx + 0.5f) * g.vs.x + 0.0f;
    float lcy = (ly + 0.5f) * g.vs.y + 0.0f;
    float lcz = (lz + 0.5f) * g.vs.z + 0.0f;
    float u = div_by<FASTDIV>(px - lcx, tc.dx);
    float v = div_by<FASTDIV>(py - lcy, tc.dy);
    float w = div_by<FASTDIV>(pz - lcz, tc.dz);

    const uint32_t ox = ((uint32_t)lx + 1 < g.X) ? 1u : 0u;
    const uint32_t oy = ((uint32_t)ly + 1 < g.Y) ? tc.row : 0u;
    const uint32_t oz = ((uint32_t)lz + 1 < g.Z) ? tc.plane : 0u;
    const float *b000 = dist + ((size_t)tc.plane * ((uint32_t)lz - g.z_store_begin) + (__umul24(tc.row, (uint32_t)ly) + (uint32_t)lx));
    if (STATS) {
        const size_t gi = (size_t)tc.plane * (uint32_t)lz + (size_t)tc.row * (uint32_t)ly + (uint32_t)lx;
        const uint32_t offs[8] = {0, oz, oy, oy + oz, ox, ox + oz, ox + oy, ox + oy + oz};
        for (int i = 0; i < 8; i++) {
            size_t q = gi + offs[i];
            atomicOr(&touched[q >> 5], 1u << (q & 31));
        }
    }
    float c000 = b000[0];
    float c001 = b000[oz];
    float c010 = b000[oy];
    float c011 = b000[oy + oz];
    float c100 = b000[ox];
    float c101 = b000[ox + oz];
    float c110 = b000[ox + oy];
    float c111 = b000[ox + oy + oz];

    float interpolated = c000 * (1 - u) * (1 - v) * (1 - w) +
                         c001 * (1 - u) * (1 - v) * w +
                         c010 * (1 - u) * v * (1 - w) +
                         c011 * (1 - u) * v * w +
                         c100 * u * (1 - v) * (1 - w) +
                         c101 * u * (1 - v) * w +
                         c110 * u * v * (1 - w) +
                         c111 * u * v * w;
    return interpolated;
}

__device__ inline bool can_intersect_in_dimension(float space_min, float space_max, float origin, float direction,
                                                  float &near_t, float &far_t) {
    bool can_intersect = true;
    if (direction == 0) {
        if (origin < space_min || origin > space_max) can_intersect = false;
    } else {
        float dmin = (space_min - origin) / direction;
        float dmax = (space_max - origin) / direction;
        if (dmin > dmax) {
            float t = dmin;
            dmin = dmax;
            dmax = t;
// ... 785 lines not shown
            kind = other;
            c.trial_kind = other;
            c.trial_left = kTrialCasts - 1;
            c.next_trial = c.casts + c.gap;
            c.blocked = false;
            c.trial_origin[0] = rp.origin.x; c.trial_origin[1] = rp.origin.y; c.trial_origin[2] = rp.origin.z;
            c.trial_axis[0] = rp.rot.m13; c.trial_axis[1] = rp.rot.m23; c.trial_axis[2] = rp.rot.m33;
        } else {
            c.next_trial = c.casts + c.gap;
        }
    }
    if (kind == 1 && (v->cell_cast_host ? *v->cell_cast_host : 0u) > (uint32_t)tuning().ray_cells_limit) kind = 0;
    if (!c.pending && c.casts > 1u && (trial || (c.trial_left == 0 && (c.seen[kind] < 3u || (c.casts & 15u) == 0u)))) {
        if (!c.ev[0]) {
            if (hipEventCreate(&c.ev[0]) != hipSuccess || hipEventCreate(&c.ev[1]) != hipSuccess) { (void)hipGetLastError(); c.ev[0] = nullptr; }
        }
        if (c.ev[0]) {
            *sample = true;
            c.pending_kind = kind;
            c.pending_trial = trial;
        }
    }
    c.last_kind = kind;
    return kind == 1;
}
static int cast_whole(tsdf_volume *v, RayParams &rp, float *out, float *normals, const float *depth_inv_pose, uint16_t *depth_out);

template <bool SLAB>
static int march_and_resolve(tsdf_volume *v, RayParams &rp, float *out, float *normals = nullptr, const float *depth_inv_pose = nullptr,
                             uint16_t *depth_out = nullptr, const EntryParams *cells = nullptr) {
    const size_t n_pix = (size_t)rp.width * rp.height;
    const int n_segments = SLAB ? slab_ray_ranges(v) : ray_segments();
    const int max_len = (kMaxSamples + n_segments - 1) / n_segments;
    const int max_pieces = std::min(kTailPieces, (max_len + tail_piece_min() - 1) / tail_piece_min());
    const size_t n_entries = n_pix * n_segments * (size_t)std::max(max_pieces, 1);
    if (v->ray_best_cap < n_pix) {
        if (v->ray_best) (void)hipFree(v->ray_best);
        v->ray_best = nullptr;
        v->ray_best_cap = 0;
        TSDF_HIP(hipMalloc((void **)&v->ray_best, 2 * n_pix * sizeof(uint64_t)), "ray result alloc");
        v->ray_best_cap = n_pix;
        v->ray_best_dirty = 1;
    }
    if (cells) {
        const size_t n_bricks_max = cell_list_capacity(v->occ.fine_count());
        if (v->cell_rays_cap < n_pix) {
            if (v->cell_rays) (void)hipFree(v->cell_rays);
            v->cell_rays = nullptr;
            v->cell_rays_cap = 0;
            TSDF_HIP(hipMalloc(&v->cell_rays, n_pix * sizeof(RayRecord)), "ray record alloc");
            v->cell_rays_cap = n_pix;
        }
        if (v->cell_bricks_cap < n_bricks_max) {
            if (v->cell_bricks) (void)hipFree(v->cell_bricks);
            v->cell_bricks = nullptr;
            v->cell_bricks_cap = 0;
            TSDF_HIP(hipMalloc((void **)&v->cell_bricks, 2 * n_bricks_max * sizeof(uint2)), "brick list alloc");
            v->cell_bricks_cap = n_bricks_max;
        }
        if (!v->cell_cast_host) {
            TSDF_HIP(hipHostMalloc((void **)&v->cell_cast_host, sizeof(uint32_t), hipHostMallocDefault), "brick count mirror alloc");
            *v->cell_cast_host = 0;
        }
    }
    if (v->tail_cap < n_entries) {
        if (v->tail_entries) (void)hipFree(v->tail_entries);
        v->tail_entries = nullptr;
        v->tail_cap = 0;
        TSDF_HIP(hipMalloc(&v->tail_entries, n_entries * sizeof(uint2)), "ray tail queue alloc");
        v->tail_cap = n_entries;
    }
    if (!v->tail_count) {
        TSDF_HIP(hipMalloc((void **)&v->tail_count, kTailSignals * sizeof(uint32_t)), "ray tail counter alloc");
        v->ray_best_dirty = 1;
    }
    if (v->ray_best_pixels != n_pix) {
        v->ray_best_pixels = n_pix;
        v->ray_best_dirty = 1;
    }
    if (v->ray_best_dirty) {
        TSDF_HIP(hipMemsetAsync(v->ray_best, 0xff, 2 * v->ray_best_cap * sizeof(uint64_t), v->stream), "ray result reset");
        TSDF_HIP(hipMemsetAsync(v->tail_count, 0, kTailSignals * sizeof(uint32_t), v->stream), "ray tail counter reset");
    }
    v->ray_best_dirty = 1;
    TailQueue tail = {reinterpret_cast<uint2 *>(v->tail_entries), v->tail_count, (uint32_t)trip_budget(), (uint32_t)tail_lanes(), v->ray_best + (size_t)v->ray_best_side * v->ray_best_cap, tail_piece_min(), nullptr};
    uint64_t *best_next = v->ray_best + (size_t)(1 - v->ray_best_side) * v->ray_best_cap;
    const bool learn_order = tuning().ray_learned_order != 0;
    const uint32_t n_tiles = ((rp.width + 15) / 16) * ((rp.height + 15) / 16);
    OrderJob order_job = {nullptr, nullptr, 0, 0, 0};
    if (learn_order && n_tiles <= 65535u && (uint32_t)n_segments <= kOrderMaxRanges) {
        if (!v->ray_heavy || v->ray_order_tiles != n_tiles || v->ray_order_ranges != (uint32_t)n_segments) {
            if (v->ray_heavy) (void)hipFree(v->ray_heavy);
            if (v->ray_order) (void)hipFree(v->ray_order);
            v->ray_heavy = nullptr;
            v->ray_order = nullptr;
            v->ray_order_valid = 0;
            TSDF_HIP(hipMalloc((void **)&v->ray_heavy, (size_t)2 * n_tiles * n_segments), "ray order alloc");
            TSDF_HIP(hipMalloc((void **)&v->ray_order, (size_t)n_tiles * n_segments * sizeof(uint32_t)), "ray order alloc");
            TSDF_HIP(hipMemsetAsync(v->ray_heavy, 0, (size_t)2 * n_tiles * n_segments, v->stream), "ray order reset");
            v->ray_order_tiles = n_tiles;
            v->ray_order_ranges = (uint32_t)n_segments;
        }
        tail.heavy_passes = tuning().ray_heavy_passes > 0 ? (uint32_t)tuning().ray_heavy_passes : std::max(1u, tail.trip_budget * 3u / 4u);
        tail.heavy = v->ray_heavy;
        tail.order = v->ray_order_valid ? v->ray_order : nullptr;
        order_job = {v->ray_heavy, v->ray_order, n_tiles, (uint32_t)n_segments, 0};
    }
    bool order_built = false;
    v->last_cast_cells = cells ? 1 : 0;
    if (cells) {
        const bool sort_list = tuning().ray_cells_sort == 2 || (tuning().ray_cells_sort == 1 && cells->z_clip == 0.0f);
        float depth0 = 0.0f, depth_scale = 0.0f;
        if (sort_list) {
            float dmin = INFINITY, dmax = -INFINITY;
            for (int c = 0; c < 8; c++) {
                const float wx = v->g.offset.x + ((c & 1) ? v->g.phys.x : 0.0f), wy = v->g.offset.y + ((c & 2) ? v->g.phys.y : 0.0f), wz = v->g.offset.z + ((c & 4) ? v->g.phys.z : 0.0f);
                const float d = cells->r[2][0] * wx + cells->r[2][1] * wy + cells->r[2][2] * wz + cells->r[2][3];
                dmin = std::min(dmin, d); dmax = std::max(dmax, d);
            }
            dmin = std::max(dmin, 0.0f);
            depth0 = dmin;
            depth_scale = dmax > dmin ? (float)kDepthBins / (dmax - dmin) : 0.0f;
            if (!std::isfinite(depth0) || !std::isfinite(depth_scale)) { depth0 = 0.0f; depth_scale = 0.0f; }
        }
        CellCast cc = {reinterpret_cast<RayRecord *>(v->cell_rays), reinterpret_cast<uint2 *>(v->cell_bricks), v->tail_count + 3, v->cell_cast_host, cells->cell_pairs,
                       sort_list ? v->tail_count + 4 : nullptr, reinterpret_cast<uint2 *>(v->cell_bricks) + v->cell_bricks_cap, depth0, depth_scale,
                       v->dist, tail.best, v->release_word, v->release_value};
        v->release_word = nullptr;
        const size_t table_lds = ((size_t)kMaxSamples + 1) * sizeof(float);
        const uint32_t n_ray_blocks = (uint32_t)((n_pix + 255) / 256);
        const uint32_t n_list_blocks = (uint32_t)std::min<size_t>((v->occ.fine_count() / 4 + 255) / 256 + 1, 2048);
        hipLaunchKernelGGL((cell_cast_prepare_kernel<SLAB>), dim3(n_ray_blocks + n_list_blocks), dim3(256), (uint32_t)table_lds, v->stream, v->g, rp, *cells, v->t_table,
                           v->occ, cc, n_list_blocks);
        if (sort_list) {
            hipLaunchKernelGGL(cell_list_sort_kernel, dim3(128), dim3(1024), 0, v->stream, v->g, *cells, cc);
        }
        if (getenv("TSDF_DEBUG_CELLS_SORT")) {
            TSDF_HIP(hipStreamSynchronize(v->stream), "cells sort");
            uint32_t n_listed = 0;
            TSDF_HIP(hipMemcpy(&n_listed, cc.n_bricks, sizeof(n_listed), hipMemcpyDeviceToHost), "cells sort");
            std::vector<uint2> list(n_listed);
            TSDF_HIP(hipMemcpy(list.data(), cc.bricks, n_listed * sizeof(uint2), hipMemcpyDeviceToHost), "cells sort");
            const bool back_first = atoi(getenv("TSDF_DEBUG_CELLS_SORT")) == 2;
            auto depth_of = [&](const uint2 &e_) {
                const float mid = 0.5f * ((float)kBrick + 1.5f);
                const float wx = ((float)((e_.y & 1023u) * kBrick) + mid) * v->g.vs.x + cells->offset.x, wy = ((float)(((e_.y >> 10) & 1023u) * kBrick) + mid) * v->g.vs.y + cells->offset.y,
                            wz = ((float)((e_.y >> 20) * kBrick) + mid) * v->g.vs.z + cells->offset.z;
                const float d = cells->r[2][0] * wx + cells->r[2][1] * wy + cells->r[2][2] * wz + cells->r[2][3];
                return back_first ? -d : d;
            };
            std::stable_sort(list.begin(), list.end(), [&](const uint2 &a_, const uint2 &b_) { return depth_of(a_) < depth_of(b_); });
            TSDF_HIP(hipMemcpy(cc.bricks, list.data(), n_listed * sizeof(uint2), hipMemcpyHostToDevice), "cells sort");
        }
        const dim3 cgrid((unsigned)tuning().ray_cells_grid + kShellWorkgroups);
        if (v->fast_div)
            TSDF_LAUNCH_TIMED(v, 1, (cast_cells_kernel<SLAB, true>), cgrid, dim3(256), v->dist, v->g, rp, *cells, v->occ, v->t_table, cc, tail.best);
        else
            TSDF_LAUNCH_TIMED(v, 1, (cast_cells_kernel<SLAB, false>), cgrid, dim3(256), v->dist, v->g, rp, *cells, v->occ, v->t_table, cc, tail.best);
        if (getenv("TSDF_DEBUG_CELLS_TWICE")) {
            if (v->fast_div)
                TSDF_LAUNCH_TIMED(v, 2, (cast_cells_kernel<SLAB, true>), cgrid, dim3(256), v->dist, v->g, rp, *cells, v->occ, v->t_table, cc, tail.best);
            else
                TSDF_LAUNCH_TIMED(v, 2, (cast_cells_kernel<SLAB, false>), cgrid, dim3(256), v->dist, v->g, rp, *cells, v->occ, v->t_table, cc, tail.best);
        }
        TSDF_HIP(hipGetLastError(), "cell-parallel cast failed");
        if (v->after_bulk) TSDF_HIP(hipEventRecord(v->after_bulk, v->stream), "process_ray: bulk kernel event");
    } else {
    rp.seg_len = (kMaxSamples + n_segments - 1) / n_segments;
    rp.slab_ranges = SLAB ? (uint32_t)n_segments : 0u;
    rp.tile_map = (uint32_t)tuning().ray_tile_map;
    rp.range_order = (uint32_t)tuning().ray_range_order;
    dim3 grid((rp.width + 15) / 16, (rp.height + 15) / 16, n_segments);
    const size_t table_lds = ray_table_lds_bytes(rp, (SLAB && rp.slab_ranges > 0) || tail.order != nullptr);
    if (v->fast_div)
        TSDF_LAUNCH_TIMED_LDS(v, 1, (process_ray_kernel<SLAB, false, true, true, true, true>), grid, dim3(256), table_lds, v->dist, v->g, rp,
                              (float *)nullptr, (unsigned long long *)nullptr, (unsigned int *)nullptr, v->occ, v->t_table, tail);
    else
        TSDF_LAUNCH_TIMED_LDS(v, 1, (process_ray_kernel<SLAB, false, true, false, true, true>), grid, dim3(256), table_lds, v->dist, v->g, rp,
                              (float *)nullptr, (unsigned long long *)nullptr, (unsigned int *)nullptr, v->occ, v->t_table, tail);
    TSDF_HIP(hipGetLastError(), "process_ray failed");
    if (v->after_bulk) TSDF_HIP(hipEventRecord(v->after_bulk, v->stream), "process_ray: bulk kernel event");
    const bool fixed_lanes = tail_lanes() == kTailLanesDefault;
    order_job.range_order = rp.range_order;
    dim3 tgrid_(tail_grid() + kOrderWorkgroups);
    order_built = order_job.n_ranges != 0;
    if (v->fast_div && fixed_lanes)
        TSDF_LAUNCH_TIMED(v, 2, (process_ray_tail_kernel<SLAB, true, kTailLanesDefault>), tgrid_, dim3(256), v->dist, v->g, rp, v->occ, v->t_table, tail, order_job);
    else if (v->fast_div)
        TSDF_LAUNCH_TIMED(v, 2, (process_ray_tail_kernel<SLAB, true, 0>), tgrid_, dim3(256), v->dist, v->g, rp, v->occ, v->t_table, tail, order_job);
    else if (fixed_lanes)
        TSDF_LAUNCH_TIMED(v, 2, (process_ray_tail_kernel<SLAB, false, kTailLanesDefault>), tgrid_, dim3(256), v->dist, v->g, rp, v->occ, v->t_table, tail, order_job);
    else
        TSDF_LAUNCH_TIMED(v, 2, (process_ray_tail_kernel<SLAB, false, 0>), tgrid_, dim3(256), v->dist, v->g, rp, v->occ, v->t_table, tail, order_job);
    TSDF_HIP(hipGetLastError(), "process_ray (tail) failed");
    if (tuning().debug_rays) {
        uint32_t n_tail = 0;
        (void)hipMemcpy(&n_tail, v->tail_count, sizeof(n_tail), hipMemcpyDeviceToHost);
        fprintf(stderr, "tsdf: %u pieces of the %zu (ray, range) pairs finished by the tail kernel\n", n_tail, n_pix * n_segments);
    }
    }
    const dim3 rgrid((unsigned)((n_pix + 255) / 256)), tgrid((rp.width + 15) / 16, (rp.height + 15) / 16);
    if (!SLAB && normals) {
        hipLaunchKernelGGL(resolve_normals_kernel, tgrid, dim3(kResolveThreads), 0, v->stream, v->g, rp, v->t_table, tail.best, best_next, out, normals,
                           v->tail_count);
    } else {
        Mat44 ip;
        memset(&ip, 0, sizeof(ip));
        if (depth_inv_pose) memcpy(&ip, depth_inv_pose, sizeof(ip));
        hipLaunchKernelGGL((resolve_hits_kernel<SLAB>), rgrid, dim3(256), 0, v->stream, v->g, rp, v->t_table, tail.best, best_next, out, v->tail_count, ip,
                           SLAB ? (uint16_t *)nullptr : depth_out);
    }
    if (order_built) v->ray_order_valid = 1;
    TSDF_HIP(hipGetLastError(), "resolve ray hits failed");
    v->ray_best_side = 1 - v->ray_best_side;
    v->ray_best_dirty = 0;
    return TSDF_OK;
}

static int cast_whole(tsdf_volume *v, RayParams &rp, float *out, float *normals, const float *depth_inv_pose, uint16_t *depth_out) {
    int rc = count_after_bulk_change(v);
    if (rc != TSDF_OK) return rc;
    EntryParams view;
    bool sample = false;
    const bool cells = choose_cast(v, rp, view, &sample);
    CastChooser &c = v->chooser;
    if (sample && hipEventRecord(c.ev[0], v->stream) != hipSuccess) { (void)hipGetLastError(); sample = false; }
    if (cells) rc = occupancy_flags_refresh(v); else rc = refresh_for_cast(v, rp);
    if (rc != TSDF_OK) return rc;
    rc = cells ? march_and_resolve<false>(v, rp, out, normals, depth_inv_pose, depth_out, &view) : march_and_resolve<false>(v, rp, out, normals, depth_inv_pose, depth_out);
    if (sample && rc == TSDF_OK) {
        if (hipEventRecord(c.ev[1], v->stream) == hipSuccess) c.pending = true; else (void)hipGetLastError();
    }
    return rc;
}

bool raycast_takes_cells(const tsdf_volume *v, uint32_t width, uint32_t height, const float pose[16], const float kinv[9]) {
    if (!v || v->z_begin != 0 || v->z_end != v->g.Z || check_ray_args(v, width, height, pose, kinv) != TSDF_OK) return false;
    if (count_after_bulk_change(const_cast<tsdf_volume *>(v)) != TSDF_OK) return false;
    RayParams rp = make_params(v, width, height, pose, kinv);
    EntryParams view;
    return choose_cell_cast(v, rp, view);
}

}

using namespace tsdf;

extern "C" {

#ifdef TSDF_DIAG_RAY_MIX
int tsdf_debug_ray_mix(unsigned long long out[64]) {
    (void)hipDeviceSynchronize();
    if (hipMemcpyFromSymbol(out, HIP_SYMBOL(g_ray_mix), 64 * sizeof(unsigned long long)) != hipSuccess) return TSDF_ERR_INVALID;
    unsigned long long zero[64] = {};
    (void)hipMemcpyToSymbol(HIP_SYMBOL(g_ray_mix), zero, sizeof(zero));
    return TSDF_OK;
}
#endif

int tsdf_raycast_device(const tsdf_volume *v, uint32_t width, uint32_t height, const float pose[16],
                        const float kinv[9], float *device_vertices, float *device_normals) {
    int rc = check_ray_args(v, width, height, pose, kinv);
    if (rc != TSDF_OK) return rc;
    TSDF_REQUIRE(device_vertices, "tsdf_raycast: null vertex buffer");
    TSDF_REQUIRE(v->z_begin == 0 && v->z_end == v->g.Z, "tsdf_raycast on a slab: use tsdf_raycast_slab_device");
    RayParams rp = make_params(v, width, height, pose, kinv);
    return cast_whole(const_cast<tsdf_volume *>(v), rp, device_vertices, device_normals, nullptr, nullptr);
}

int tsdf_raycast(const tsdf_volume *cv, uint32_t width, uint32_t height, const float pose[16], const float kinv[9],
                 float *host_vertices, float *host_normals) {
    int rc = check_ray_args(cv, width, height, pose, kinv);
    if (rc != TSDF_OK) return rc;
    TSDF_REQUIRE(host_vertices, "tsdf_raycast: null vertex buffer");
    tsdf_volume *v = const_cast<tsdf_volume *>(cv);
    size_t bytes = (size_t)width * height * 3 * sizeof(float);
    if (v->ray_cap < bytes) {
        if (v->vert_buf) (void)hipFree(v->vert_buf);
        if (v->norm_buf) (void)hipFree(v->norm_buf);
        v->vert_buf = v->norm_buf = nullptr;
        v->ray_cap = 0;
        TSDF_HIP(hipMalloc((void **)&v->vert_buf, bytes), "Vertices alloc failed");
        TSDF_HIP(hipMalloc((void **)&v->norm_buf, bytes), "Normals alloc failed");
        v->ray_cap = bytes;
    }
    rc = tsdf_raycast_device(v, width, height, pose, kinv, v->vert_buf, host_normals ? v->norm_buf : nullptr);
    if (rc != TSDF_OK) return rc;
    TSDF_HIP(hipMemcpyAsync(host_vertices, v->vert_buf, bytes, hipMemcpyDeviceToHost, v->stream), "Vertices Memcpy failed");
    if (host_normals)
        TSDF_HIP(hipMemcpyAsync(host_normals, v->norm_buf, bytes, hipMemcpyDeviceToHost, v->stream), "Normals Memcpy failed");
    TSDF_HIP(hipStreamSynchronize(v->stream), "process_ray failed");
    return TSDF_OK;
}

int tsdf_volume_last_raycast_kind(const tsdf_volume *v, int *cell_parallel) {
    TSDF_REQUIRE(v && cell_parallel, "null argument");
    *cell_parallel = v->last_cast_cells;
    return TSDF_OK;
}

int tsdf_volume_last_cell_list(const tsdf_volume *v, uint32_t *listed) {
    TSDF_REQUIRE(v && listed, "tsdf_volume_last_cell_list: null argument");
    TSDF_HIP(hipStreamSynchronize(v->stream), "tsdf_volume_last_cell_list");
    *listed = v->cell_cast_host ? *v->cell_cast_host : 0u;
    return TSDF_OK;
}

int tsdf_raycast_depth_device(const tsdf_volume *v, uint32_t width, uint32_t height, const float pose[16], const float inv_pose[16],
                              const float kinv[9], uint16_t *device_depth, float *device_vertices) {
    int rc = check_ray_args(v, width, height, pose, kinv);
    if (rc != TSDF_OK) return rc;
    TSDF_REQUIRE(device_depth && inv_pose, "tsdf_raycast_depth: null argument");
    TSDF_REQUIRE(v->z_begin == 0 && v->z_end == v->g.Z, "tsdf_raycast_depth needs a whole volume");
    RayParams rp = make_params(v, width, height, pose, kinv);
    return cast_whole(const_cast<tsdf_volume *>(v), rp, device_vertices, nullptr, inv_pose, device_depth);
}
// ... 135 lines not shown
```

### tsdf_amd/csrc/raycast_cells.hpp

```cpp

struct RayRecord {
    float near_t;
    uint32_t k_range;
};
static_assert(sizeof(RayRecord) == 8, "one 8-byte load");

struct CellCast {
    RayRecord *rays;
    uint2 *bricks;
    uint32_t *n_bricks;
    uint32_t *n_bricks_host;
    uint32_t pairs_per_task;
    uint32_t *depth_hist;
    uint2 *unsorted;
    float depth0, depth_scale;
    const float *dist;
    uint64_t *best;
    uint32_t *release_word;
    uint32_t release_value;
};
constexpr uint32_t kCellTasks = 1u << 31, kShellTasks = 1u << 30;
constexpr uint32_t kDepthBins = 256;
__device__ inline uint32_t depth_bin(const CellCast &cc, const EntryParams &ep, const Geom &g, uint32_t coords) {
    const float mid = 0.5f * ((float)kBrick + 1.5f);
// ... 267 lines not shown
        const uint32_t a0 = start[4u * t], a1 = start[4u * t + 1u], a2 = start[4u * t + 2u], a3 = start[4u * t + 3u];
        uint32_t incl = (a0 + a1) + (a2 + a3);
        for (int o = 1; o < 64; o <<= 1) {
            const uint32_t up = __shfl_up(incl, o);
            if ((int)t >= o) incl += up;
        }
        const uint32_t ex = incl - ((a0 + a1) + (a2 + a3));
        start[4u * t] = ex; start[4u * t + 1u] = ex + a0; start[4u * t + 2u] = ex + a0 + a1; start[4u * t + 3u] = ex + a0 + a1 + a2;
    }
    uint32_t *fill = cc.depth_hist + kDepthBins;
    for (uint32_t c0 = blockIdx.x * 1024u; c0 < n; c0 += gridDim.x * 1024u) {
        __syncthreads();
        if (t < kDepthBins) mine[t] = 0u;
        __syncthreads();
        const uint32_t i = c0 + t;
        uint2 e = make_uint2(0u, 0u);
        uint32_t bin = 0, rank = 0;
        if (i < n) {
            e = cc.unsorted[i];
            bin = depth_bin(cc, ep, g, e.y);
            rank = atomicAdd(&mine[bin], 1u);
        }
        __syncthreads();
        if (t < kDepthBins && mine[t]) base[t] = atomicAdd(&fill[t], mine[t]);
        __syncthreads();
        if (i < n) cc.bricks[start[bin] + base[bin] + rank] = e;
    }
}

constexpr float kIntervalSlack = 0.125f;
__device__ inline bool sample_interval(const RayState &r, float lox, float loy, float loz, float hix, float hiy, float hiz, float inv_step, float step,
                                       const float *T, int k_first, int k_end, int &k_lo, int &k_hi) {
    float tin = 0.0f, tout = INFINITY;
    bool miss = false;
    auto axis = [&](float s, float d, float lo, float hi) {
        if (d != 0.0f) {
            const float rd = __builtin_amdgcn_rcpf(d);
            const float t0 = (lo - s) * rd, t1 = (hi - s) * rd;
            tin = fmaxf(tin, fminf(t0, t1));
            tout = fminf(tout, fmaxf(t0, t1));
        } else if (s < lo || s > hi) {
            miss = true;
        }
    };
    axis(r.sx, r.dx, lox, hix);
    axis(r.sy, r.dy, loy, hiy);
    axis(r.sz, r.dz, loz, hiz);
    if (miss || !(tin <= tout * 1.00001f + 1.0e-3f)) return false;
    const float kc = fminf(fmaxf(rintf(tin * inv_step), 0.0f), (float)kMaxSamples);
    const float drift = T[(int)kc] - kc * step;
    const float a = ceilf((tin - drift) * inv_step - kIntervalSlack), b = floorf((tout - drift) * inv_step + kIntervalSlack);
    k_lo = max(k_first, a > 0.0f ? (a < 8192.0f ? (int)a : 8192) : 0);
    k_hi = min(k_end - 1, b < 8192.0f ? (b > 0.0f ? (int)b : 0) : 8192);
    return k_lo <= k_hi;
}

#ifndef TSDF_SHELL_WGS
#define TSDF_SHELL_WGS 512
#endif
constexpr uint32_t kShellWorkgroups = TSDF_SHELL_WGS;
template <bool SLAB, bool FASTDIV>
__device__ inline void cast_shell_bricks(const float *__restrict__ dist, const Geom &g, const RayParams &rp, const EntryParams &ep, const float *T,
                                         const CellCast &cc, uint64_t *__restrict__ best, uint32_t n_bricks, uint2 *mine, uint32_t *n_mine) {
    const TriConst &tc = rp.tc;
    const float step_size = T[1];
    const SkipCtx sc = make_skip_ctx(g, step_size);
    const float e = sc.eps;
    const float size_[3] = {(float)g.X, (float)g.Y, (float)g.Z}, vs_[3] = {g.vs.x, g.vs.y, g.vs.z};
    for (uint32_t j0 = 0; blockIdx.x + (size_t)j0 * kShellWorkgroups < n_bricks; j0 += 256) {
        __syncthreads();
        if (threadIdx.x == 0) *n_mine = 0;
        __syncthreads();
        const size_t ei = blockIdx.x + (size_t)(j0 + threadIdx.x) * kShellWorkgroups;
        if (ei < n_bricks) {
            const uint2 en = cc.bricks[ei];
            if (en.x & kShellTasks) mine[atomicAdd(n_mine, 1u)] = en;
        }
        __syncthreads();
        const uint32_t n_shell = *n_mine;
        for (uint32_t si = 0; si < n_shell; si++) {
            const uint2 entry2 = mine[si];
            const uint32_t o_[3] = {(entry2.y & 1023u) * kBrick, ((entry2.y >> 10) & 1023u) * kBrick, (entry2.y >> 20) * kBrick};
            float lo_[3], hi_[3];
#pragma unroll
            for (int a_ = 0; a_ < 3; a_++) {
                lo_[a_] = (float)o_[a_] - e;
                hi_[a_] = fminf((float)(o_[a_] + kBrick), size_[a_]) + e;
            }
            PixelBox sb;
            if (!project_box(ep, lo_[0] * vs_[0], lo_[1] * vs_[1], lo_[2] * vs_[2], hi_[0] * vs_[0], hi_[1] * vs_[1], hi_[2] * vs_[2], sb)) continue;
            const uint32_t part = (entry2.x >> 10) & (kMaxParts - 1u), parts = (entry2.x & (kMaxParts - 1u)) + 1u;
            const uint32_t share = ((uint32_t)(sb.w * sb.h) + parts - 1u) / parts;
            const int pi_begin = (int)min(part * share, (uint32_t)(sb.w * sb.h)), n_pix = (int)min((uint32_t)pi_begin + share, (uint32_t)(sb.w * sb.h));
            if (threadIdx.x == 0) { RAY_MIX(42); }
            const int sub = (int)(threadIdx.x & 7u);
            for (int pi = pi_begin + (int)(threadIdx.x >> 3); pi < n_pix; pi += 32) {
                const int py = pi / sb.w, px = pi - py * sb.w;
                if (sub == 0) { RAY_MIX(43); }
                const uint32_t idx = (uint32_t)(sb.v0 + py) * rp.width + (uint32_t)(sb.u0 + px);
                const RayRecord rec_ = cc.rays[idx];
                const uint32_t known = (uint32_t)(best[idx] >> 32);
                const RayState ray = ray_from_near(ray_direction(sb.u0 + px, sb.v0 + py, rp), rec_.near_t, rp);
                const int k_first = (int)(rec_.k_range & 0xffffu), k_end = (int)(rec_.k_range >> 16);
#pragma unroll
                for (int a_ = 0; a_ < 3; a_++) {
#pragma unroll
                    for (int side = 0; side < 2; side++) {
                        float slo[3] = {lo_[0], lo_[1], lo_[2]}, shi[3] = {hi_[0], hi_[1], hi_[2]};
                        if (side == 0) {
                            if (o_[a_] != 0u) continue;
                            shi[a_] = 0.5f + e;
                        } else {
                            if ((float)(o_[a_] + kBrick) < size_[a_]) continue;
                            slo[a_] = size_[a_] - 0.5f - e;
                        }
                        int k, k_hi;
                        if (!sample_interval(ray, slo[0] * vs_[0], slo[1] * vs_[1], slo[2] * vs_[2], shi[0] * vs_[0], shi[1] * vs_[1], shi[2] * vs_[2], sc.inv_step, step_size, T,
                                             k_first, k_end, k, k_hi))
                            continue;
                        if (known <= (uint32_t)k) continue;
                        for (k += sub; k <= k_hi; k += 8) {
                            RAY_MIX(44);
                            const float t = T[k];
                            const float ppx = (t * ray.dx) + ray.sx, ppy = (t * ray.dy) + ray.sy, ppz = (t * ray.dz) + ray.sz;
                            const float f_[3] = {ppx * sc.inv_vx, ppy * sc.inv_vy, ppz * sc.inv_vz};
                            if (!(f_[0] >= slo[0] && f_[0] <= shi[0] && f_[1] >= slo[1] && f_[1] <= shi[1] && f_[2] >= slo[2] && f_[2] <= shi[2])) continue;
                            bool owned;
                            const float tsdf = trilinear<SLAB, false, FASTDIV>(ppx, ppy, ppz, dist, g, tc, rp, owned, nullptr);
                            if (tsdf <= 0) {
                                RAY_MIX(41);
                                lower_best(&best[idx], k, tsdf);
                                break;
                            }
                        }
                    }
                }
            }
        }
    }
}

#ifndef TSDF_CELLS_WAVES
#define TSDF_CELLS_WAVES 4
#endif
#ifndef TSDF_CELLS_SCAN_DECODE
#define TSDF_CELLS_SCAN_DECODE 1
#endif
template <bool SLAB, bool FASTDIV>
#if TSDF_CELLS_WAVES
__attribute__((amdgpu_waves_per_eu(TSDF_CELLS_WAVES, TSDF_CELLS_WAVES)))
#endif
__global__ __launch_bounds__(256) void cast_cells_kernel(const float *__restrict__ dist, const Geom g, const RayParams rp, const EntryParams ep,
                                                         const OccGrid occ, const float *__restrict__ t_table, const CellCast cc,
                                                         uint64_t *__restrict__ best) {
    __shared__ __attribute__((aligned(16))) float T[kTableLen];
    __shared__ float corner[4][128];
    __shared__ __attribute__((aligned(16))) int box_of[4][64][4];
    __shared__ int prefix[4][64];
#if TSDF_CELLS_SCAN_DECODE
    __shared__ uint32_t mark[4][64];
    mark[threadIdx.x >> 6][threadIdx.x & 63u] = 0u;
    uint32_t round = 0u;
#endif
    static_assert(kTableLen % 4 == 0, "the table in 16-byte pieces");
    for (int i = (int)threadIdx.x; i < kTableLen / 4; i += 256) reinterpret_cast<float4 *>(T)[i] = reinterpret_cast<const float4 *>(t_table)[i];
    const uint32_t n_bricks = *cc.n_bricks;
    if (cc.n_bricks_host && blockIdx.x == 0 && threadIdx.x == 0) *cc.n_bricks_host = n_bricks;
    static_assert(sizeof(box_of) >= 256 * sizeof(uint2), "a shell workgroup's list of bricks");
    if (blockIdx.x < kShellWorkgroups) {
        __syncthreads();
        cast_shell_bricks<SLAB, FASTDIV>(dist, g, rp, ep, T, cc, best, n_bricks, reinterpret_cast<uint2 *>(&box_of[0][0][0]), reinterpret_cast<uint32_t *>(&prefix[0][0]));
        return;
    }
    const uint32_t wave = threadIdx.x >> 6, lane = threadIdx.x & 63u;
    const float step_size = t_table[1];
    const TriConst &tc = rp.tc;
    const SkipCtx sc = make_skip_ctx(g, step_size);
    const float e = sc.eps;
    const size_t plane = (size_t)g.X * g.Y;
    const float ex = (1.0f + 2.0f * e) * g.vs.x, ey = (1.0f + 2.0f * e) * g.vs.y, ez = (1.0f + 2.0f * e) * g.vs.z;
    float nu_[3], nv_[3], nz_[3];
#pragma unroll
    for (int a_ = 0; a_ < 3; a_++) {
        const float ext = a_ == 0 ? ex : a_ == 1 ? ey : ez;
        const float cxa = ep.r[0][a_] * ext, cya = ep.r[1][a_] * ext, cza = ep.r[2][a_] * ext;
        nu_[a_] = ep.k[0][0] * cxa + ep.k[0][1] * cya + ep.k[0][2] * cza;
        nv_[a_] = ep.k[1][0] * cxa + ep.k[1][1] * cya + ep.k[1][2] * cza;
        nz_[a_] = cza;
    }
    const float half_dz = 0.5f * ((fabsf(nz_[0]) + fabsf(nz_[1])) + fabsf(nz_[2]));
    __syncthreads();
    auto wave_sync = [] {
        __builtin_amdgcn_fence(__ATOMIC_RELEASE, "wavefront");
        __builtin_amdgcn_s_waitcnt(0xc07f);
        __builtin_amdgcn_wave_barrier();
        __builtin_amdgcn_fence(__ATOMIC_ACQUIRE, "wavefront");
    };
    auto offset_of = [&](uint32_t i) { return (size_t)(i / 25u) * plane + (size_t)((i / 5u) % 5u) * g.X + (i % 5u); };
    const size_t off_a = offset_of(lane), off_b = offset_of(min(lane + 64u, 124u));
    auto brick_voxels = [&](uint2 entry_, float &va, float &vb) {
        va = vb = 0.0f;
        if (!(entry_.x & kCellTasks)) return;
        const uint32_t bx_ = entry_.y & 1023u, by_ = (entry_.y >> 10) & 1023u, bz_ = entry_.y >> 20;
        if (bx_ * kBrick + kBrick < g.X && by_ * kBrick + kBrick < g.Y && bz_ * kBrick >= g.z_store_begin && bz_ * kBrick + kBrick < g.z_store_end) {
            const float *first = dist + (plane * (bz_ * kBrick - g.z_store_begin) + (size_t)g.X * (by_ * kBrick) + bx_ * kBrick);
            va = first[off_a];
            vb = first[off_b];
            return;
        }
        auto voxel = [&](uint32_t i) {
            const uint32_t cx = i % 5u, cy = (i / 5u) % 5u, cz = i / 25u;
            const uint32_t vx = min(bx_ * kBrick + cx, g.X - 1u), vy = min(by_ * kBrick + cy, g.Y - 1u);
            const uint32_t vz = min(max(bz_ * kBrick + cz, g.z_store_begin), g.z_store_end - 1u);
            return dist[plane * (vz - g.z_store_begin) + (size_t)g.X * vy + vx];
        };
        va = voxel(lane);
        if (lane + 64u < 125u) vb = voxel(lane + 64u);
    };
    const uint32_t n_waves = (gridDim.x - kShellWorkgroups) * 4u;
    uint32_t ei = (blockIdx.x - kShellWorkgroups) * 4u + wave;
    uint2 entry_next = ei < n_bricks ? cc.bricks[ei] : make_uint2(0u, 0u);
    float va_next, vb_next;
    brick_voxels(entry_next, va_next, vb_next);
    for (; ei < n_bricks; ei += n_waves) {
        const uint2 entry2 = entry_next;
        const uint32_t entry = entry2.x;
        const float va = va_next, vb = vb_next;
        entry_next = ei + n_waves < n_bricks ? cc.bricks[ei + n_waves] : make_uint2(0u, 0u);
        brick_voxels(entry_next, va_next, vb_next);
        const uint32_t bx = entry2.y & 1023u, by = (entry2.y >> 10) & 1023u, bz = entry2.y >> 20;
        const uint32_t x0 = bx * kBrick, y0 = by * kBrick, z0 = bz * kBrick;
        wave_sync();
        corner[wave][lane] = va;
        corner[wave][lane + 64u] = vb;
        wave_sync();
        const uint32_t cx = lane & 3u, cy = (lane >> 2) & 3u, cz = lane >> 4;
        const uint32_t lx = x0 + cx, ly = y0 + cy, lz = z0 + cz;
        bool mixed = false;
        if (entry & kCellTasks) {
            bool valid = lx + 1u < g.X && ly + 1u < g.Y && lz + 1u < g.Z && lz >= g.z_store_begin && lz + 1u < g.z_store_end;
            if (SLAB) valid = valid && lz >= rp.own_lo && lz < rp.own_hi;
            const float *c = &corner[wave][cx + 5u * cy + 25u * cz];
            const bool positive = fminf(fminf(fminf(c[0], c[1]), fminf(c[5], c[6])), fminf(fminf(c[25], c[26]), fminf(c[30], c[31]))) > kCellPositive;
            mixed = valid && !positive;
        }
        PixelBox pb = {0, 0, 0, 0};
        if (mixed) {
            const float wx = ((float)lx + 1.0f) * g.vs.x + ep.offset.x, wy = ((float)ly + 1.0f) * g.vs.y + ep.offset.y, wz = ((float)lz + 1.0f) * g.vs.z + ep.offset.z;
            const float ccx = ep.r[0][0] * wx + ep.r[0][1] * wy + ep.r[0][2] * wz + ep.r[0][3];
            const float ccy = ep.r[1][0] * wx + ep.r[1][1] * wy + ep.r[1][2] * wz + ep.r[1][3];
            const float ccz = ep.r[2][0] * wx + ep.r[2][1] * wy + ep.r[2][2] * wz + ep.r[2][3];
            const float zmin = ccz - half_dz;
            if (zmin > ep.z_near) {
                const float rz = __builtin_amdgcn_rcpf(ccz), rm = __builtin_amdgcn_rcpf(zmin);
                const float uc = (ep.k[0][0] * ccx + ep.k[0][1] * ccy + ep.k[0][2] * ccz) * rz, vc = (ep.k[1][0] * ccx + ep.k[1][1] * ccy + ep.k[1][2] * ccz) * rz;
                const float su = 0.5f * ((fabsf(nu_[0] - uc * nz_[0]) + fabsf(nu_[1] - uc * nz_[1])) + fabsf(nu_[2] - uc * nz_[2]));
                const float sv = 0.5f * ((fabsf(nv_[0] - vc * nz_[0]) + fabsf(nv_[1] - vc * nz_[1])) + fabsf(nv_[2] - vc * nz_[2]));
                const float hu = su * rm * 1.0001f + 0.05f, hv = sv * rm * 1.0001f + 0.05f;
                const float a0 = fmaxf(ceilf(uc - hu), 0.0f), a1 = fminf(floorf(uc + hu), (float)(ep.width - 1u));
                const float b0 = fmaxf(ceilf(vc - hv), 0.0f), b1 = fminf(floorf(vc + hv), (float)(ep.height - 1u));
                mixed = a0 <= a1 && b0 <= b1;
                if (mixed) { pb.u0 = (int)a0; pb.v0 = (int)b0; pb.w = (int)a1 - (int)a0 + 1; pb.h = (int)b1 - (int)b0 + 1; }
            } else {
                const float clx = ((float)lx + 0.5f - e) * g.vs.x, chx = ((float)lx + 1.5f + e) * g.vs.x;
                const float cly = ((float)ly + 0.5f - e) * g.vs.y, chy = ((float)ly + 1.5f + e) * g.vs.y;
                const float clz = ((float)lz + 0.5f - e) * g.vs.z, chz = ((float)lz + 1.5f + e) * g.vs.z;
                mixed = project_box<false>(ep, clx, cly, clz, chx, chy, chz, pb);
            }
        }
        if (lane == 0) { RAY_MIX(32); }
        if (mixed) { RAY_MIX(33); }
#if TSDF_CELLS_SCAN_DECODE
        const int n_mine = mixed ? pb.w * pb.h : 0, incl = (int)wave_scan_add((uint32_t)n_mine);
        const int n_pairs = __builtin_amdgcn_readlane(incl, 63);
        const int first_mine = incl - n_mine;
        if (mixed) {
            box_of[wave][lane][0] = pb.u0; box_of[wave][lane][1] = pb.v0; box_of[wave][lane][2] = pb.w; box_of[wave][lane][3] = first_mine;
        }
#else
        int n_mine = mixed ? pb.w * pb.h : 0, incl = n_mine;
        for (int o = 1; o < 64; o <<= 1) {
            const int up = __shfl_up(incl, o);
            if ((int)lane >= o) incl += up;
        }
        const int n_pairs = __shfl(incl, 63);
        prefix[wave][lane] = incl - n_mine;
        if (mixed) {
            box_of[wave][lane][0] = pb.u0; box_of[wave][lane][1] = pb.v0; box_of[wave][lane][2] = pb.w; box_of[wave][lane][3] = pb.h;
        }
        wave_sync();
#endif
        int q_begin = 0, q_end = n_pairs;
        if (entry & (kMaxParts - 1u)) {
            const uint32_t part = (entry >> 10) & (kMaxParts - 1u), parts = (entry & (kMaxParts - 1u)) + 1u;
            const uint32_t share = ((uint32_t)n_pairs + parts - 1u) / parts;
            q_begin = (int)min(part * share, (uint32_t)n_pairs);
            q_end = (int)min((uint32_t)q_begin + share, (uint32_t)n_pairs);
        }
        for (int q0 = q_begin; q0 < q_end; q0 += 64) {
            const int q = q0 + (int)lane;
#if TSDF_CELLS_SCAN_DECODE
            round++;
            const int place = first_mine - q0;
            if (n_mine > 0 && place < 64 && place + n_mine > 0) mark[wave][max(place, 0)] = round << 6 | lane;
            wave_sync();
            const int cl = (int)(wave_scan_max(mark[wave][lane]) & 63u);
            if (q >= q_end) continue;
            const int4 box = *reinterpret_cast<const int4 *>(&box_of[wave][cl][0]);
            const int pi = q - box.w;
            const int u0 = box.x, v0 = box.y, bw = box.z;
#else
            if (q >= q_end) continue;
            int cl = 0, hi_ = 63;
#pragma unroll
            for (int it = 0; it < 6; it++) {
                const int mid = (cl + hi_ + 1) >> 1;
                if (prefix[wave][mid] <= q) cl = mid; else hi_ = mid - 1;
            }
            const int pi = q - prefix[wave][cl];
            const int u0 = box_of[wave][cl][0], v0 = box_of[wave][cl][1], bw = box_of[wave][cl][2];
#endif
            const uint32_t qx = (uint32_t)cl & 3u, qy = ((uint32_t)cl >> 2) & 3u, qz = (uint32_t)cl >> 4;
            const float lfx = (float)(x0 + qx), lfy = (float)(y0 + qy), lfz = (float)(z0 + qz);
            RAY_MIX(34);
            const int py = pi < (1 << 22) ? (int)(((float)pi + 0.5f) * __builtin_amdgcn_rcpf((float)bw)) : pi / bw, px = pi - py * bw;
            const int imx = u0 + px, imy = v0 + py;
            const uint32_t idx = (uint32_t)imy * rp.width + (uint32_t)imx;
            const RayRecord rec_ = cc.rays[idx];
            const uint32_t known = __hip_atomic_load(reinterpret_cast<const uint32_t *>(best + idx) + 1, __ATOMIC_RELAXED, __HIP_MEMORY_SCOPE_WORKGROUP);
            const RayState ray = ray_from_near(ray_direction(imx, imy, rp), rec_.near_t, rp);
            int k, k_hi;
            if (!sample_interval(ray, (lfx + 0.5f - e) * g.vs.x, (lfy + 0.5f - e) * g.vs.y, (lfz + 0.5f - e) * g.vs.z, (lfx + 1.5f + e) * g.vs.x,
                                 (lfy + 1.5f + e) * g.vs.y, (lfz + 1.5f + e) * g.vs.z, sc.inv_step, step_size, T, (int)(rec_.k_range & 0xffffu),
                                 (int)(rec_.k_range >> 16), k, k_hi))
                continue;
            RAY_MIX(35);
            if (known <= (uint32_t)k) continue;
            RAY_MIX(36);
            const float *c = &corner[wave][qx + 5u * qy + 25u * qz];
            const float d000 = c[0], d100 = c[1], d010 = c[5], d110 = c[6], d001 = c[25], d101 = c[26], d011 = c[30], d111 = c[31];
            const float lcx = (lfx + 0.5f) * g.vs.x, lcy = (lfy + 0.5f) * g.vs.y, lcz = (lfz + 0.5f) * g.vs.z;
            SkipCtx rs = sc;
            set_ray<true>(rs, ray, step_size, g);
            const CellBound cb = cell_bound(d000, d100, d010, d110, d001, d101, d011, d111, rs);
            bool entered = false;
            while (k <= k_hi) {
                RAY_MIX(37);
                const float t = T[k];
                const float ppx = (t * ray.dx) + ray.sx, ppy = (t * ray.dy) + ray.sy, ppz = (t * ray.dz) + ray.sz;
                const float rx = (ppx * rs.inv_vx - 0.5f) - lfx, ry = (ppy * rs.inv_vy - 0.5f) - lfy, rz = (ppz * rs.inv_vz - 0.5f) - lfz;
                const float far_ = fmaxf(fmaxf(fabsf(rx - 0.5f), fabsf(ry - 0.5f)), fabsf(rz - 0.5f));
                if (!(far_ <= 0.5f + e)) {
                    if (entered) break;
                    k++;
                    continue;
                }
                entered = true;
                if (far_ < 0.5f - e) {
                    RAY_MIX(38);
                    const float u = div_by<FASTDIV>(ppx - lcx, tc.dx);
                    const float v = div_by<FASTDIV>(ppy - lcy, tc.dy);
                    const float w = div_by<FASTDIV>(ppz - lcz, tc.dz);
                    const float val = d000 * (1 - u) * (1 - v) * (1 - w) +
                                      d001 * (1 - u) * (1 - v) * w +
                                      d010 * (1 - u) * v * (1 - w) +
                                      d011 * (1 - u) * v * w +
                                      d100 * u * (1 - v) * (1 - w) +
                                      d101 * u * (1 - v) * w +
                                      d110 * u * v * (1 - w) +
                                      d111 * u * v * w;
                    if (val <= 0) {
                        RAY_MIX(40);
// ... 26 lines not shown
```

### tsdf_amd/csrc/volume.hip

```cpp
#include <cmath>
#include <cstdlib>
#include <cstring>
#include <new>
#include <vector>

#include <algorithm>

#include "common.hpp"

namespace tsdf {

static thread_local char g_err[512] = "";

void set_error(const char *fmt, ...) {
    va_list ap;
    va_start(ap, fmt);
    vsnprintf(g_err, sizeof(g_err), fmt, ap);
    va_end(ap);
}

const Tuning &tuning() {
    static const Tuning t = [] {
        auto num = [](const char *name, int fallback) { const char *e = getenv(name); return e ? atoi(e) : fallback; };
        auto clamp = [](int v, int lo, int hi) { return v < lo ? lo : (v > hi ? hi : v); };
        Tuning u;
        u.ray_segments = clamp(num("TSDF_RAY_SEGMENTS", 6), 1, 64);
        u.ray_slab_ranges = clamp(num("TSDF_RAY_SLAB_RANGES", 0), 0, 64);
        u.ray_cells = clamp(num("TSDF_RAY_CELLS", 1), 0, 2);
        u.ray_cells_limit = std::max(num("TSDF_RAY_CELLS_LIMIT", 131072), 0);
        u.ray_cells_grid = clamp(num("TSDF_RAY_CELLS_GRID", 2048), 1, 65535);
        u.ray_cells_sort = clamp(num("TSDF_RAY_CELLS_SORT", 1), 0, 2);
        u.ray_chooser = clamp(num("TSDF_RAY_CHOOSER", 0), 0, 2);
        u.ray_cells_pairs = clamp(num("TSDF_RAY_CELLS_PAIRS", 1024), 0, 1 << 24);
        u.ray_cells_look = clamp(num("TSDF_RAY_CELLS_LOOK", 1), 0, 1);
        { const char *fp = getenv("TSDF_RAY_CELLS_FOOTPRINT"); u.ray_cells_footprint = fp ? (float)atof(fp) : 10.0f; }
        u.ray_trip_budget = std::max(num("TSDF_RAY_TRIP_BUDGET", 22), 1);
        u.ray_tail_lanes = num("TSDF_RAY_TAIL_LANES", 4);
        if (!(u.ray_tail_lanes >= 1 && u.ray_tail_lanes <= 64 && (u.ray_tail_lanes & (u.ray_tail_lanes - 1)) == 0)) u.ray_tail_lanes = 4;
        u.ray_tail_grid = std::max(num("TSDF_RAY_TAIL_GRID", 256 * 10), 1);
        u.ray_tail_piece = std::max(num("TSDF_RAY_TAIL_PIECE", 64), 1);
        u.ray_range_order = clamp(num("TSDF_RAY_RANGE_ORDER", 1), 0, 2);
        u.ray_tile_map = clamp(num("TSDF_RAY_TILE_MAP", 2), 0, 2);
        u.ray_learned_order = num("TSDF_RAY_LEARNED_ORDER", 1) != 0;
        u.ray_heavy_passes = std::max(num("TSDF_RAY_HEAVY_PASSES", 0), 0);
        u.ray_entry_bound = num("TSDF_RAY_ENTRY_BOUND", 1) != 0;
        u.icp_persistent = num("TSDF_ICP_PERSISTENT", 0);
        u.occ_rebuild_period = std::max(num("TSDF_OCC_REBUILD_PERIOD", 16), 0);
        u.occ_scan_all = num("TSDF_OCC_SCAN_ALL", 0) != 0;
        u.reach_lds = num("TSDF_REACH_LDS", 0) != 0;
        u.int_grid_per_cu = num("TSDF_INT_GRID_PER_CU", 0);
        u.weight_pack = num("TSDF_WEIGHT_PACK", 8);
        if (u.weight_pack != 0 && u.weight_pack != 16) u.weight_pack = 8;
        u.pipe_release = clamp(num("TSDF_PIPE_RELEASE", 0), 0, 2);
        u.pipe_host_wait = num("TSDF_PIPE_HOST_WAIT", 0) != 0;
        u.pipe_word_release = num("TSDF_PIPE_WORD_RELEASE", 0) != 0;
        u.event_scope = clamp(num("TSDF_EVENT_SCOPE", 2), 0, 2);
        u.timing_bracket = num("TSDF_TIMING_BRACKET", 0) != 0;
        u.verbose = getenv("TSDF_VERBOSE") != nullptr;
        u.debug_rays = getenv("TSDF_DEBUG_RAYS") != nullptr;
        return u;
    }();
    return t;
}

int hip_fail(hipError_t e, const char *what) {
    set_error("%s: %s", what, hipGetErrorString(e));
    return e == hipErrorOutOfMemory ? TSDF_ERR_NOMEM : TSDF_ERR_DEVICE;
}

__global__ __launch_bounds__(256) void fill_kernel(float *__restrict__ dist, size_t n, float dval) {
    size_t n4 = n >> 2;
    float4 d4 = make_float4(dval, dval, dval, dval);
    size_t stride = (size_t)gridDim.x * blockDim.x;
    for (size_t i = (size_t)blockIdx.x * blockDim.x + threadIdx.x; i < n4; i += stride) reinterpret_cast<float4 *>(dist)[i] = d4;
    size_t t = (n4 << 2) + (size_t)blockIdx.x * blockDim.x + threadIdx.x;
    if (t < n) dist[t] = dval;
}

__global__ __launch_bounds__(256) void copy4_kernel(const float4 *__restrict__ src, float4 *__restrict__ dst, size_t n) {
    const size_t stride = (size_t)gridDim.x * 256;
    size_t i = (size_t)blockIdx.x * 256 + threadIdx.x;
    for (; i + 3 * stride < n; i += 4 * stride) {
        const float4 a = src[i], b = src[i + stride], c = src[i + 2 * stride], d = src[i + 3 * stride];
        dst[i] = a; dst[i + stride] = b; dst[i + 2 * stride] = c; dst[i + 3 * stride] = d;
    }
    for (; i < n; i += stride) dst[i] = src[i];
}

__global__ __launch_bounds__(256) void update_walk_kernel(float *__restrict__ d, float *__restrict__ w) {
    const unsigned b = blockIdx.x, bx = b % 8, by = (b / 8) % 128, bz = b / (8 * 128);
    const size_t plane = (size_t)512 * 512;
    const size_t idx = (size_t)bz * 32 * plane + (size_t)(by * 4 + threadIdx.y) * 512 + bx * 64 + threadIdx.x;
#pragma unroll 1
    for (int z = 0; z < 32; z += 4) {
        float pd[4], pw[4];
#pragma unroll
        for (int j = 0; j < 4; j++) { pd[j] = d[idx + (z + j) * plane]; pw[j] = w[idx + (z + j) * plane]; }
#pragma unroll
        for (int j = 0; j < 4; j++) {
            const float nw = pw[j] + 1.0f;
            d[idx + (z + j) * plane] = (pd[j] * pw[j] + 3.0f) / nw;
            w[idx + (z + j) * plane] = nw;
        }
    }
}

__global__ __launch_bounds__(256) void init_nodes_kernel(tsdf_deformation_node *nodes, Geom g) {
    uint32_t vx = blockIdx.x * blockDim.x + threadIdx.x;
    uint32_t vy = blockIdx.y;
    uint32_t vz = g.z_store_begin + blockIdx.z;
    if (vx >= g.X) return;
    size_t idx = (size_t)g.X * g.Y * (vz - g.z_store_begin) + (size_t)g.X * vy + vx;
    tsdf_deformation_node nd;
    nd.translation[0] = (((int)vx + 0.5f) * g.vs.x) + g.offset.x;
    nd.translation[1] = (((int)vy + 0.5f) * g.vs.y) + g.offset.y;
    nd.translation[2] = (((int)vz + 0.5f) * g.vs.z) + g.offset.z;
    nd.rotation[0] = 0.0f;
    nd.rotation[1] = 0.0f;
    nd.rotation[2] = 0.0f;
    nodes[idx] = nd;
}

__global__ __launch_bounds__(256) void occupancy_init_kernel(OccGrid occ, uint32_t size_x, uint32_t size_y, uint32_t size_z) {
    size_t i = (size_t)blockIdx.x * 256 + threadIdx.x;
    if (i < occ.fine_count()) {
        uint32_t bx = i % occ.nbx, by = (i / occ.nbx) % occ.nby, bz = i / ((size_t)occ.nbx * occ.nby);
        occ.fine[i] = 0;
        bool partial = bx * kBrick + kBrick > size_x - 1 || by * kBrick + kBrick > size_y - 1 || bz * kBrick + kBrick > size_z - 1;
        occ.cell[i] = partial ? 1 : 0;
    }
}

constexpr uint32_t kScanRows = 8;
__global__ __launch_bounds__(256) void occupancy_scan_kernel(const float *__restrict__ dist, Geom g, OccGrid occ,
                                                             uint16_t *__restrict__ bits, uint8_t *__restrict__ rim_bits,
                                                             const uint8_t *__restrict__ touched,
                                                             const uint32_t tnx, const uint32_t tny, const uint32_t tnz) {
    __shared__ uint32_t acc[64];
    const uint32_t wave = threadIdx.x >> 6, lane = threadIdx.x & 63u;
    for (uint32_t row = 0; row < kScanRows; row++) {
    const uint32_t bx = blockIdx.x * 64 + lane, by = blockIdx.y * kScanRows + row, bz = blockIdx.z;
    if (by >= occ.nby) break;
    const uint32_t y = by * kBrick + wave;
    bool scan = true;
    if (touched) {
        const uint32_t z0 = bz * kBrick;
        const uint32_t ibx = min(bx * kBrick / kIntBrickX, tnx - 1u), iby = min(by * kBrick / kIntBrickY, tny - 1u);
        const uint32_t ibz = z0 >= g.z_store_begin ? min((z0 - g.z_store_begin) / kIntBrickZ, tnz - 1u) : 0u;
        scan = touched[((size_t)ibz * tny + iby) * tnx + ibx] != 0;
        scan = scan && bx < occ.nbx && occ.fine[((size_t)bz * occ.nby + by) * occ.nbx + bx] != 0;
        if (__syncthreads_or(scan) == 0) continue;
    }
    if (threadIdx.x < 64) acc[threadIdx.x] = 0;
    __syncthreads();
    uint32_t oct = 0, low = 0, rim = 0;
    if (scan && bx < occ.nbx && y < g.Y) {
        const uint32_t x0 = bx * kBrick;
        const bool vec = (g.X & 3u) == 0;
        const uint32_t y0f = wave == 0 ? 1u : 0u, yo = wave >> 1;
        for (uint32_t j = 0; j < (uint32_t)kBrick; j++) {
            const uint32_t z = bz * kBrick + j;
            if (z < g.z_store_begin || z >= g.z_store_end) continue;
            const float *row = dist + ((size_t)g.X * g.Y * (z - g.z_store_begin) + (size_t)g.X * y + x0);
            uint32_t m = 0;
            uint32_t nf = 0;
            if (vec) {
                const float4 d = *reinterpret_cast<const float4 *>(row);
                m = (!(d.x > occ.tau) ? 1u : 0u) | (!(d.y > occ.tau) ? 2u : 0u) | (!(d.z > occ.tau) ? 4u : 0u) | (!(d.w > occ.tau) ? 8u : 0u);
                nf = (occ.not_flat(d.x) ? 1u : 0u) | (occ.not_flat(d.y) ? 2u : 0u) | (occ.not_flat(d.z) ? 4u : 0u) | (occ.not_flat(d.w) ? 8u : 0u);
            } else {
                for (uint32_t i = 0; i < (uint32_t)kBrick; i++)
                    if (x0 + i < g.X) {
                        if (!(row[i] > occ.tau)) m |= 1u << i;
                        if (occ.not_flat(row[i])) nf |= 1u << i;
                    }
            }
            if (nf) {
                const uint32_t zo = j >> 1;
                if (nf & 3u) rim |= 1u << (0 + 2 * yo + 4 * zo);
                if (nf & 12u) rim |= 1u << (1 + 2 * yo + 4 * zo);
            }
            if (m) {
                const uint32_t zo = j >> 1, z0f = j == 0 ? 1u : 0u, fx = m & 1u;
                if (m & 3u) oct |= 1u << (0 + 2 * yo + 4 * zo);
                if (m & 12u) oct |= 1u << (1 + 2 * yo + 4 * zo);
                low |= 1u | (fx << 1) | (y0f << 2) | (z0f << 3) | ((fx & y0f) << 4) | ((fx & z0f) << 5) | ((y0f & z0f) << 6) |
                       ((fx & y0f & z0f) << 7);
            }
        }
    }
    const uint32_t both = oct | (low << 8) | (rim << 16);
    if (both) atomicOr(&acc[lane], both);
    __syncthreads();
    if (threadIdx.x < 64 && bx < occ.nbx && scan) {
        bits[((size_t)bz * occ.nby + by) * occ.nbx + bx] = (uint16_t)acc[lane];
        rim_bits[((size_t)bz * occ.nby + by) * occ.nbx + bx] = (uint8_t)(acc[lane] >> 16);
    }
    __syncthreads();
    }
}

__global__ __launch_bounds__(256) void occupancy_flags_kernel(const uint16_t *__restrict__ bits, const uint8_t *__restrict__ rim_bits, OccGrid occ, uint32_t size_x,
                                                              uint32_t size_y, uint32_t size_z, uint8_t *__restrict__ touched,
                                                              const uint32_t n_touched, const bool incremental) {
    for (size_t i = (size_t)blockIdx.x * 256 + threadIdx.x; i < max(occ.fine_count(), (size_t)n_touched); i += (size_t)gridDim.x * 256) {
    if (touched && i < n_touched) touched[i] = 0;
// ... 1059 lines not shown
```

### tsdf_amd/pipeline.py

```python
import ctypes as C

import numpy as np
import torch

from . import _capi
from ._capi import check, lib
from .api import _camera_matrices

OVERLAP, EQUAL_PRIORITY, EXCHANGE_STREAM, NO_TIGHTEN_AHEAD = 1, 2, 4, 8


def _matrices(camera):
    m = _capi.CameraMatrices()
    pose, ipose, k, kinv = _camera_matrices(camera)
    C.memmove(m.pose, pose.ctypes.data, 64)
    C.memmove(m.inv_pose, ipose.ctypes.data, 64)
    C.memmove(m.k, k.ctypes.data, 36)
    C.memmove(m.kinv, kinv.ctypes.data, 36)
    return m


class FusionPipeline:

    def __init__(self, volume, bilateral, raycaster, width, height, overlap=True, exchange=None, equal_priority=False, exchange_stream=False,
                 tighten_ahead=True):
        self.volume, self.bilateral, self.raycaster = volume, bilateral, raycaster
        self.width, self.height = int(width), int(height)
        self.overlap = bool(overlap)
        self.exchange = exchange
        flags = (OVERLAP if overlap else 0) | (EQUAL_PRIORITY if equal_priority else 0) | (EXCHANGE_STREAM if exchange_stream else 0) | \
            (0 if tighten_ahead else NO_TIGHTEN_AHEAD)
        self._h = C.c_void_p()
        check(lib.tsdf_pipeline_create(volume._h, bilateral._h, self.width, self.height, flags, exchange._h if exchange is not None else None,
                                       C.byref(self._h)))
        import weakref
        volume._dependents = list(getattr(volume, "_dependents", ())) + [weakref.ref(self)]
        m, s = C.c_void_p(), C.c_void_p()
        check(lib.tsdf_pipeline_streams(self._h, C.byref(m), C.byref(s)))
        dev = torch.device("cuda", torch.cuda.current_device())
        self.main = torch.cuda.ExternalStream(m.value, device=dev)
        self.side = torch.cuda.ExternalStream(s.value, device=dev) if s.value else None

    def hit_buffers(self):
        a, b = C.c_void_p(), C.c_void_p()
        check(lib.tsdf_pipeline_hit_buffers(self._h, C.byref(a), C.byref(b)))
        return a.value, b.value

    def step(self, depth_ptr, camera, vertices_ptr, normals_ptr=None, next_depth_ptr=None, next_camera=None):
        cam = _matrices(camera)
        nxt = _matrices(next_camera) if (next_camera is not None and next_depth_ptr is not None) else None
        check(lib.tsdf_pipeline_step(self._h, C.c_void_p(int(depth_ptr)), C.byref(cam), C.c_void_p(int(vertices_ptr)),
                                     C.c_void_p(int(normals_ptr)) if normals_ptr else None,
                                     C.c_void_p(int(next_depth_ptr)) if next_depth_ptr else None,
                                     C.byref(nxt) if nxt is not None else None))

    def synchronize(self):
        check(lib.tsdf_pipeline_synchronize(self._h))

    def close(self):
        if lib is not None and getattr(self, "_h", None) is not None and self._h.value:
            lib.tsdf_pipeline_destroy(self._h)
            self._h = C.c_void_p()

    __del__ = close
```

Before: 618,800.

## Fuse next-frame bilateral filter into raycast cell kernel on one stream

Moves the bilateral filter tile body into a shared header so it can run as extra workgroups appended to the cell-parallel raycast kernel, reusing that kernel's shared arrays as filter LDS. A new default-on one-stream pipeline mode launches the next frame's filter inside the cast launch and prepares integration tiles on the main stream, instead of using a side stream with events. This is meant to remove a separate kernel launch and cross-stream synchronisation. In exchange the cast kernel carries extra LDS aliasing constraints and a branch, and it applies only for radius 7 with an exact scale.

```diff
diff --git a/include/tsdf_amd.h b/include/tsdf_amd.h
--- a/include/tsdf_amd.h
+++ b/include/tsdf_amd.h
@@ -178,6 +178,8 @@
 int tsdf_pipeline_synchronize(tsdf_pipeline *pipeline);
 int tsdf_pipeline_streams(const tsdf_pipeline *pipeline, void **main_stream, void **side_stream);
 int tsdf_pipeline_hit_buffers(const tsdf_pipeline *pipeline, tsdf_hit_record **device_mine, tsdf_hit_record **device_all);
+int tsdf_pipeline_filtered_ahead(const tsdf_pipeline *pipeline, const uint16_t **device_filtered, const uint16_t **device_tile_max,
+                                 int *in_cast_launch);
 int tsdf_pipeline_destroy(tsdf_pipeline *pipeline);
 
 typedef struct tsdf_tracker tsdf_tracker;
diff --git a/tsdf_amd/_capi.py b/tsdf_amd/_capi.py
--- a/tsdf_amd/_capi.py
+++ b/tsdf_amd/_capi.py
@@ -118,6 +118,7 @@
     "tsdf_pipeline_synchronize": (_i, [_vp]),
     "tsdf_pipeline_streams": (_i, [_vp, C.POINTER(_vp), C.POINTER(_vp)]),
     "tsdf_pipeline_hit_buffers": (_i, [_vp, C.POINTER(_vp), C.POINTER(_vp)]),
+    "tsdf_pipeline_filtered_ahead": (_i, [_vp, C.POINTER(_vp), C.POINTER(_vp), C.POINTER(_i)]),
     "tsdf_pipeline_destroy": (_i, [_vp]),
     "tsdf_tracker_create": (_i, [_vp, _vp, _vp, _u32, _u32, _f, _i, C.POINTER(_vp)]),
     "tsdf_tracker_filter": (_i, [_vp, _vp]),
diff --git a/tsdf_amd/csrc/bilateral.hip b/tsdf_amd/csrc/bilateral.hip
--- a/tsdf_amd/csrc/bilateral.hip
+++ b/tsdf_amd/csrc/bilateral.hip
@@ -4,25 +4,9 @@
 #include <type_traits>
 #include <vector>
 
-#include "common.hpp"
+#include "bilateral_tile.hpp"
 
 namespace tsdf {
-
-constexpr int kBTile = 16;
-constexpr int kMaxRadius = 24;
-
-constexpr int kSimLds = 4096;
-
-__device__ inline void bilateral_tap(float weight, double intensity, float &sum, float &total_weight) {
-    sum = (float)__builtin_fma((double)weight, intensity, (double)sum);
-    total_weight = total_weight + weight;
-}
-
-__device__ inline unsigned sad_u32(unsigned a, unsigned b) {
-    unsigned d;
-    asm("v_sad_u32 %0, %1, %2, 0" : "=v"(d) : "v"(a), "v"(b));
-    return d;
-}
 
 template <typename PIX, int R>
 __global__ __launch_bounds__(256) void bilateral_kernel(const PIX *__restrict__ in, PIX *__restrict__ out,
@@ -32,174 +16,17 @@
                                                         uint16_t *__restrict__ tile_max) {
     constexpr bool STAGED = R > 0;
     __shared__ unsigned wg_max;
-    if (threadIdx.x == 0) wg_max = 0u;
     extern __shared__ __align__(16) unsigned char smem_raw[];
     const int radius = R > 0 ? R : radius_arg;
     const int n = 2 * radius + 1;
     const int span = kBTile + 2 * radius;
-    double *tile_d = reinterpret_cast<double *>(smem_raw);
-    float *kern_lds = reinterpret_cast<float *>(tile_d + (STAGED ? 0 : span * span));
-    float *sim_lds = kern_lds + n * n;
-    uint32_t *tile4 = reinterpret_cast<uint32_t *>(sim_lds + (STAGED ? kSimLds : 0));
-    const int tx0 = blockIdx.x * kBTile - radius;
-    const int ty0 = blockIdx.y * kBTile - radius;
-    {
-        constexpr int kAhead = 4;
-        for (int i0 = threadIdx.x; i0 < span * span; i0 += 256 * kAhead) {
-            unsigned v_[kAhead];
-#pragma unroll
-            for (int u = 0; u < kAhead; u++) {
-                const int i = min(i0 + u * 256, span * span - 1);
-                const int ly = i / span, lx = i - ly * span;
-                const int gx = min(max(tx0 + lx, 0), width - 1), gy = min(max(ty0 + ly, 0), height - 1);
-                v_[u] = in[(size_t)gy * width + gx];
-            }
-#pragma unroll
-            for (int u = 0; u < kAhead; u++) {
-                const int i = i0 + u * 256;
-                const int ly = i / span, lx = i - ly * span;
-                const int gx = tx0 + lx, gy = ty0 + ly;
-                const unsigned v = (gx >= 0 && gx < width && gy >= 0 && gy < height) ? v_[u] : 0u;
-                if (i < span * span) {
-                    tile4[i] = v * 4u;
-                    if (!STAGED) tile_d[i] = (double)(int)v;
-                }
-            }
-        }
-    }
-    {
-        const int n_sim = !STAGED ? 0 : (sizeof(PIX) == 1 ? 256 : kSimLds);
-        constexpr int kAhead = 16;
-        float k_ = 0.0f;
-        if ((int)threadIdx.x < n * n) k_ = kernel[threadIdx.x];
-        for (int i0 = threadIdx.x; i0 < n_sim; i0 += 256 * kAhead) {
-            float s_[kAhead];
-#pragma unroll
-            for (int u = 0; u < kAhead; u++) s_[u] = similarity[min(i0 + u * 256, n_sim - 1)];
-#pragma unroll
-            for (int u = 0; u < kAhead; u++)
-                if (i0 + u * 256 < n_sim) sim_lds[i0 + u * 256] = s_[u];
-        }
-        if ((int)threadIdx.x < n * n) kern_lds[threadIdx.x] = k_;
-        for (int i = threadIdx.x + 256; i < n * n; i += 256) kern_lds[i] = kernel[i];
-    }
-    __syncthreads();
-
-    const int lx = threadIdx.x & 15, ly = threadIdx.x >> 4;
-    const int x = blockIdx.x * kBTile + lx;
-    const int y = blockIdx.y * kBTile + ly;
-    const uint32_t *t0 = tile4 + ly * span + lx;
-    const double *d0 = tile_d + ly * span + lx;
-    const unsigned current4 = t0[radius * span + radius];
-    float total_weight = 0;
-    float sum = 0;
-    const int wy0 = (blockIdx.y * kBTile + (ly & ~3)) - radius;
-    const bool interior = tx0 >= 0 && tx0 + span <= width && wy0 >= 0 && wy0 + 4 + 2 * radius <= height;
-    const bool inside = x < width && y < height;
-    const int i0 = max(0, radius - x), i1 = inside ? min(n - 1, width - 1 - x + radius) : -1;
-    const int j0 = max(0, radius - y), j1 = inside ? min(n - 1, height - 1 - y + radius) : -1;
-    const int nyv = j1 - j0 + 1;
-
-    if (STAGED) {
-        constexpr int N = 2 * (R > 0 ? R : 1) + 1;
-        constexpr int SPAN = kBTile + 2 * (R > 0 ? R : 1);
-        constexpr unsigned kStagedBytes = (sizeof(PIX) == 1 ? 256u : (unsigned)kSimLds) * 4u;
-        constexpr int NA = (N + 1) / 2, NB = N - NA;
-        float w_a[NA], w_b[NB > 0 ? NB : 1];
-        unsigned v_a[NA], v_b[NB > 0 ? NB : 1];
-        auto fetch = [&](const int i, auto first_row, auto count, float *w, unsigned *v4, const auto rim) {
-            constexpr int J0 = decltype(first_row)::value, CNT = decltype(count)::value;
-            unsigned delta4[CNT];
-#pragma unroll
-            for (int j = 0; j < CNT; j++) {
-                v4[j] = t0[(J0 + j) * SPAN + i];
-                delta4[j] = sad_u32(v4[j], current4);
-            }
-#pragma unroll
-            for (int j = 0; j < CNT; j++)
-                w[j] = *reinterpret_cast<const float *>(reinterpret_cast<const char *>(sim_lds) + delta4[j]);
-            if (sizeof(PIX) != 1) {
-                unsigned big = delta4[0];
-#pragma unroll
-                for (int j = 1; j < CNT; j++) big = max(big, delta4[j]);
-                if (__builtin_expect(big >= kStagedBytes, 0)) {
-#pragma unroll
-                    for (int j = 0; j < CNT; j++)
-                        if (delta4[j] >= kStagedBytes) {
-                            const char *p = reinterpret_cast<const char *>(similarity) + delta4[j];
-                            asm volatile("global_load_dword %0, %1, off\n\ts_waitcnt vmcnt(0)" : "=v"(w[j]) : "v"(p) : "memory");
-                        }
-                }
-            }
-            if (!decltype(rim)::value) {
-#pragma unroll
-                for (int j = 0; j < CNT; j++) w[j] = kernel[i * N + J0 + j] * w[j];
-            } else {
-                const bool col_ok = i >= i0 && i <= i1;
-                const int base = (i - i0) * nyv - j0;
-#pragma unroll
-                for (int j = 0; j < CNT; j++) {
-                    const bool ok = col_ok && J0 + j >= j0 && J0 + j <= j1;
-                    const float k = kern_lds[(base + J0 + j) & (ok ? 255 : 0)];
-                    w[j] = __builtin_bit_cast(float, __builtin_bit_cast(unsigned, k * w[j]) & (ok ? 0xffffffffu : 0u));
-                }
-            }
-        };
-        auto chain = [&](const int i, auto first_row, auto count, const float *w, const unsigned *v4) {
-            constexpr int CNT = decltype(count)::value;
-            (void)i;
-#pragma unroll
-            for (int j = 0; j < CNT; j++) bilateral_tap(w[j], (double)v4[j], sum, total_weight);
-        };
-        using Lo = std::integral_constant<int, 0>;
-        using Hi = std::integral_constant<int, NA>;
-        using CntA = std::integral_constant<int, NA>;
-        using CntB = std::integral_constant<int, NB>;
-        auto run = [&](const auto rim) {
-            fetch(0, Lo{}, CntA{}, w_a, v_a, rim);
-#pragma unroll 1
-            for (int i = 0; i + 1 < N; i++) {
-                fetch(i, Hi{}, CntB{}, w_b, v_b, rim);
-                chain(i, Lo{}, CntA{}, w_a, v_a);
-                fetch(i + 1, Lo{}, CntA{}, w_a, v_a, rim);
-                chain(i, Hi{}, CntB{}, w_b, v_b);
-            }
-            fetch(N - 1, Hi{}, CntB{}, w_b, v_b, rim);
-            chain(N - 1, Lo{}, CntA{}, w_a, v_a);
-            chain(N - 1, Hi{}, CntB{}, w_b, v_b);
-        };
-        if (interior) {
-            run(std::false_type{});
-        } else {
-            __builtin_amdgcn_s_setprio(3);
-            run(std::true_type{});
-        }
-        sum *= 0.25f;
-    } else {
-#pragma unroll 1
-        for (int i = 0; i < n; i++) {
-            const bool col_ok = i >= i0 && i <= i1;
-            const int base = (i - i0) * nyv - j0;
-#pragma unroll 1
-            for (int j = 0; j < n; j++) {
-                const int o = j * span + i;
-                const bool ok = col_ok && j >= j0 && j <= j1;
-                const unsigned delta = sad_u32(t0[o], current4) >> 2;
-                const float k = kern_lds[ok ? base + j : 0];
-                const float weight = ok ? k * similarity[delta] : 0.0f;
-                bilateral_tap(weight, d0[o], sum, total_weight);
-            }
-        }
-    }
-    const PIX filtered = inside ? (PIX)(int)floorf(sum / total_weight) : (PIX)0;
-    if (inside) out[(size_t)y * width + x] = filtered;
-    if (tile_max) {
-        unsigned m = (unsigned)filtered;
-        for (int o = 32; o > 0; o >>= 1) m = max(m, (unsigned)__shfl_down((int)m, o));
-        if ((threadIdx.x & 63) == 0 && m) atomicMax(&wg_max, m);
-        __syncthreads();
-        if (threadIdx.x == 0) tile_max[blockIdx.y * gridDim.x + blockIdx.x] = (uint16_t)wg_max;
-    }
+    BilateralLds lds;
+    lds.tile_d = reinterpret_cast<double *>(smem_raw);
+    lds.kern = reinterpret_cast<float *>(lds.tile_d + (STAGED ? 0 : span * span));
+    lds.sim = lds.kern + n * n;
+    lds.tile4 = reinterpret_cast<uint32_t *>(lds.sim + (STAGED ? kSimLds : 0));
+    lds.wg_max = &wg_max;
+    bilateral_tile<PIX, R>(in, out, width, height, radius_arg, kernel, similarity, tile_max, blockIdx.x, blockIdx.y, gridDim.x, lds);
 }
 
 template <typename PIX>
@@ -218,6 +45,14 @@
                            f->similarity_dev, tile_max);
     TSDF_HIP(hipGetLastError(), "bilateral filter kernel failed");
     return TSDF_OK;
+}
+
+bool bilateral_fusable(const tsdf_bilateral *f, const uint16_t *in, uint16_t *out, int width, int height, uint16_t *tile_max, FusedFilter *ff) {
+    memset(ff, 0, sizeof(*ff));
+    if (!(f && in && out && in != out && tile_max && width > 0 && height > 0 && f->radius == 7 && f->scale_exact)) return false;
+    const uint32_t tiles_x = (uint32_t)(width + kBTile - 1) / kBTile, tiles_y = (uint32_t)(height + kBTile - 1) / kBTile;
+    *ff = {in, out, tile_max, f->kernel_dev, f->similarity_dev, width, height, tiles_x, tiles_x * tiles_y};
+    return true;
 }
 
 template <typename PIX>
diff --git a/tsdf_amd/csrc/bilateral_tile.hpp b/tsdf_amd/csrc/bilateral_tile.hpp
--- /dev/null
+++ b/tsdf_amd/csrc/bilateral_tile.hpp
@@ -0,0 +1,208 @@
+#pragma once
+#include <type_traits>
+
+#include "common.hpp"
+
+namespace tsdf {
+
+constexpr int kBTile = 16;
+constexpr int kMaxRadius = 24;
+
+constexpr int kSimLds = 4096;
+
+__device__ inline void bilateral_tap(float weight, double intensity, float &sum, float &total_weight) {
+    sum = (float)__builtin_fma((double)weight, intensity, (double)sum);
+    total_weight = total_weight + weight;
+}
+
+__device__ inline unsigned sad_u32(unsigned a, unsigned b) {
+    unsigned d;
+    asm("v_sad_u32 %0, %1, %2, 0" : "=v"(d) : "v"(a), "v"(b));
+    return d;
+}
+
+struct BilateralLds {
+    double *tile_d;
+    float *kern;
+    float *sim;
+    uint32_t *tile4;
+    unsigned *wg_max;
+};
+
+template <typename PIX, int R>
+__device__ __forceinline__ void bilateral_tile(const PIX *__restrict__ in, PIX *__restrict__ out, int width, int height, int radius_arg,
+                                               const float *__restrict__ kernel, const float *__restrict__ similarity,
+                                               uint16_t *__restrict__ tile_max, const uint32_t bx, const uint32_t by, const uint32_t tiles_x,
+                                               const BilateralLds lds) {
+    constexpr bool STAGED = R > 0;
+    unsigned &wg_max = *lds.wg_max;
+    if (threadIdx.x == 0) wg_max = 0u;
+    const int radius = R > 0 ? R : radius_arg;
+    const int n = 2 * radius + 1;
+    const int span = kBTile + 2 * radius;
+    double *tile_d = lds.tile_d;
+    float *kern_lds = lds.kern;
+    float *sim_lds = lds.sim;
+    uint32_t *tile4 = lds.tile4;
+    const int tx0 = bx * kBTile - radius;
+    const int ty0 = by * kBTile - radius;
+    {
+        constexpr int kAhead = 4;
+        for (int i0 = threadIdx.x; i0 < span * span; i0 += 256 * kAhead) {
+            unsigned v_[kAhead];
+#pragma unroll
+            for (int u = 0; u < kAhead; u++) {
+                const int i = min(i0 + u * 256, span * span - 1);
+                const int ly = i / span, lx = i - ly * span;
+                const int gx = min(max(tx0 + lx, 0), width - 1), gy = min(max(ty0 + ly, 0), height - 1);
+                v_[u] = in[(size_t)gy * width + gx];
+            }
+#pragma unroll
+            for (int u = 0; u < kAhead; u++) {
+                const int i = i0 + u * 256;
+                const int ly = i / span, lx = i - ly * span;
+                const int gx = tx0 + lx, gy = ty0 + ly;
+                const unsigned v = (gx >= 0 && gx < width && gy >= 0 && gy < height) ? v_[u] : 0u;
+                if (i < span * span) {
+                    tile4[i] = v * 4u;
+                    if (!STAGED) tile_d[i] = (double)(int)v;
+                }
+            }
+        }
+    }
+    {
+        const int n_sim = !STAGED ? 0 : (sizeof(PIX) == 1 ? 256 : kSimLds);
+        constexpr int kAhead = 16;
+        float k_ = 0.0f;
+        if ((int)threadIdx.x < n * n) k_ = kernel[threadIdx.x];
+        for (int i0 = threadIdx.x; i0 < n_sim; i0 += 256 * kAhead) {
+            float s_[kAhead];
+#pragma unroll
+            for (int u = 0; u < kAhead; u++) s_[u] = similarity[min(i0 + u * 256, n_sim - 1)];
+#pragma unroll
+            for (int u = 0; u < kAhead; u++)
+                if (i0 + u * 256 < n_sim) sim_lds[i0 + u * 256] = s_[u];
+        }
+        if ((int)threadIdx.x < n * n) kern_lds[threadIdx.x] = k_;
+        for (int i = threadIdx.x + 256; i < n * n; i += 256) kern_lds[i] = kernel[i];
+    }
+    __syncthreads();
+
+    const int lx = threadIdx.x & 15, ly = threadIdx.x >> 4;
+    const int x = bx * kBTile + lx;
+    const int y = by * kBTile + ly;
+    const uint32_t *t0 = tile4 + ly * span + lx;
+    const double *d0 = tile_d + ly * span + lx;
+    const unsigned current4 = t0[radius * span + radius];
+    float total_weight = 0;
+    float sum = 0;
+    const int wy0 = (by * kBTile + (ly & ~3)) - radius;
+    const bool interior = tx0 >= 0 && tx0 + span <= width && wy0 >= 0 && wy0 + 4 + 2 * radius <= height;
+    const bool inside = x < width && y < height;
+    const int i0 = max(0, radius - x), i1 = inside ? min(n - 1, width - 1 - x + radius) : -1;
+    const int j0 = max(0, radius - y), j1 = inside ? min(n - 1, height - 1 - y + radius) : -1;
+    const int nyv = j1 - j0 + 1;
+
+    if (STAGED) {
+        constexpr int N = 2 * (R > 0 ? R : 1) + 1;
+        constexpr int SPAN = kBTile + 2 * (R > 0 ? R : 1);
+        constexpr unsigned kStagedBytes = (sizeof(PIX) == 1 ? 256u : (unsigned)kSimLds) * 4u;
+        constexpr int NA = (N + 1) / 2, NB = N - NA;
+        float w_a[NA], w_b[NB > 0 ? NB : 1];
+        unsigned v_a[NA], v_b[NB > 0 ? NB : 1];
+        auto fetch = [&](const int i, auto first_row, auto count, float *w, unsigned *v4, const auto rim) {
+            constexpr int J0 = decltype(first_row)::value, CNT = decltype(count)::value;
+            unsigned delta4[CNT];
+#pragma unroll
+            for (int j = 0; j < CNT; j++) {
+                v4[j] = t0[(J0 + j) * SPAN + i];
+                delta4[j] = sad_u32(v4[j], current4);
+            }
+#pragma unroll
+            for (int j = 0; j < CNT; j++)
+                w[j] = *reinterpret_cast<const float *>(reinterpret_cast<const char *>(sim_lds) + delta4[j]);
+            if (sizeof(PIX) != 1) {
+                unsigned big = delta4[0];
+#pragma unroll
+                for (int j = 1; j < CNT; j++) big = max(big, delta4[j]);
+                if (__builtin_expect(big >= kStagedBytes, 0)) {
+#pragma unroll
+                    for (int j = 0; j < CNT; j++)
+                        if (delta4[j] >= kStagedBytes) {
+                            const char *p = reinterpret_cast<const char *>(similarity) + delta4[j];
+                            asm volatile("global_load_dword %0, %1, off\n\ts_waitcnt vmcnt(0)" : "=v"(w[j]) : "v"(p) : "memory");
+                        }
+                }
+            }
+            if (!decltype(rim)::value) {
+#pragma unroll
+                for (int j = 0; j < CNT; j++) w[j] = kernel[i * N + J0 + j] * w[j];
+            } else {
+                const bool col_ok = i >= i0 && i <= i1;
+                const int base = (i - i0) * nyv - j0;
+#pragma unroll
+                for (int j = 0; j < CNT; j++) {
+                    const bool ok = col_ok && J0 + j >= j0 && J0 + j <= j1;
+                    const float k = kern_lds[(base + J0 + j) & (ok ? 255 : 0)];
+                    w[j] = __builtin_bit_cast(float, __builtin_bit_cast(unsigned, k * w[j]) & (ok ? 0xffffffffu : 0u));
+                }
+            }
+        };
+        auto chain = [&](const int i, auto first_row, auto count, const float *w, const unsigned *v4) {
+            constexpr int CNT = decltype(count)::value;
+            (void)i;
+#pragma unroll
+            for (int j = 0; j < CNT; j++) bilateral_tap(w[j], (double)v4[j], sum, total_weight);
+        };
+        using Lo = std::integral_constant<int, 0>;
+        using Hi = std::integral_constant<int, NA>;
+        using CntA = std::integral_constant<int, NA>;
+        using CntB = std::integral_constant<int, NB>;
+        auto run = [&](const auto rim) {
+            fetch(0, Lo{}, CntA{}, w_a, v_a, rim);
+#pragma unroll 1
+            for (int i = 0; i + 1 < N; i++) {
+                fetch(i, Hi{}, CntB{}, w_b, v_b, rim);
+                chain(i, Lo{}, CntA{}, w_a, v_a);
+                fetch(i + 1, Lo{}, CntA{}, w_a, v_a, rim);
+                chain(i, Hi{}, CntB{}, w_b, v_b);
+            }
+            fetch(N - 1, Hi{}, CntB{}, w_b, v_b, rim);
+            chain(N - 1, Lo{}, CntA{}, w_a, v_a);
+            chain(N - 1, Hi{}, CntB{}, w_b, v_b);
+        };
+        if (interior) {
+            run(std::false_type{});
+        } else {
+            __builtin_amdgcn_s_setprio(3);
+            run(std::true_type{});
+        }
+        sum *= 0.25f;
+    } else {
+#pragma unroll 1
+        for (int i = 0; i < n; i++) {
+            const bool col_ok = i >= i0 && i <= i1;
+            const int base = (i - i0) * nyv - j0;
+#pragma unroll 1
+            for (int j = 0; j < n; j++) {
+                const int o = j * span + i;
+                const bool ok = col_ok && j >= j0 && j <= j1;
+                const unsigned delta = sad_u32(t0[o], current4) >> 2;
+                const float k = kern_lds[ok ? base + j : 0];
+                const float weight = ok ? k * similarity[delta] : 0.0f;
+                bilateral_tap(weight, d0[o], sum, total_weight);
+            }
+        }
+    }
+    const PIX filtered = inside ? (PIX)(int)floorf(sum / total_weight) : (PIX)0;
+    if (inside) out[(size_t)y * width + x] = filtered;
+    if (tile_max) {
+        unsigned m = (unsigned)filtered;
+        for (int o = 32; o > 0; o >>= 1) m = max(m, (unsigned)__shfl_down((int)m, o));
+        if ((threadIdx.x & 63) == 0 && m) atomicMax(&wg_max, m);
+        __syncthreads();
+        if (threadIdx.x == 0) tile_max[by * tiles_x + bx] = (uint16_t)wg_max;
+    }
+}
+
+}
diff --git a/tsdf_amd/csrc/common.hpp b/tsdf_amd/csrc/common.hpp
--- a/tsdf_amd/csrc/common.hpp
+++ b/tsdf_amd/csrc/common.hpp
@@ -56,6 +56,7 @@
     int weight_pack;
     int pipe_release;
     int pipe_word_release;
+    int pipe_one_stream;
     int pipe_host_wait;
     int event_scope;
     int timing_bracket;
@@ -72,6 +73,14 @@
 int occupancy_tighten_on(struct ::tsdf_volume *v, hipStream_t stream);
 struct EntryParams;
 int occupancy_refresh(struct ::tsdf_volume *v, const EntryParams *entry = nullptr);
+struct FusedFilter {
+    const uint16_t *in;
+    uint16_t *out, *tile_max;
+    const float *kernel, *similarity;
+    int width, height;
+    uint32_t tiles_x, n_wgs;
+};
+bool bilateral_fusable(const struct ::tsdf_bilateral *f, const uint16_t *in, uint16_t *out, int width, int height, uint16_t *tile_max, FusedFilter *ff);
 bool raycast_takes_cells(const struct ::tsdf_volume *v, uint32_t width, uint32_t height, const float pose[16], const float kinv[9]);
 int occupancy_flags_refresh(struct ::tsdf_volume *v);
 int build_t_table(struct ::tsdf_volume *v);
@@ -221,6 +230,7 @@
     size_t ray_cap;
     uint32_t *release_word;
     uint32_t release_value;
+    tsdf::FusedFilter fused_filter;
     hipEvent_t after_bulk;
     uint64_t *ray_best;
     size_t ray_best_cap;
diff --git a/tsdf_amd/csrc/pipeline.hip b/tsdf_amd/csrc/pipeline.hip
--- a/tsdf_amd/csrc/pipeline.hip
+++ b/tsdf_amd/csrc/pipeline.hip
@@ -92,6 +92,8 @@
     bool merged_pending;
     const uint16_t *ahead_depth;
     int ahead_buf;
+    bool ahead_on_main;
+    bool ahead_in_cast;
     bool ahead_culled;
     uint64_t frames;
     tsdf_hit_record *hits_mine, *hits_all;
@@ -479,6 +481,15 @@
     return TSDF_OK;
 }
 
+int tsdf_pipeline_filtered_ahead(const tsdf_pipeline *p, const uint16_t **device_filtered, const uint16_t **device_tile_max, int *in_cast_launch) {
+    TSDF_REQUIRE(p, "null pipeline");
+    const bool ahead = p->ahead_depth != nullptr;
+    if (device_filtered) *device_filtered = ahead ? p->filtered[p->ahead_buf] : nullptr;
+    if (device_tile_max) *device_tile_max = ahead ? p->tile_max[p->ahead_buf] : nullptr;
+    if (in_cast_launch) *in_cast_launch = ahead && p->ahead_in_cast ? 1 : 0;
+    return TSDF_OK;
+}
+
 int tsdf_pipeline_step(tsdf_pipeline *p, const uint16_t *device_depth, const tsdf_camera_matrices *cam, float *device_vertices,
                        float *device_normals, const uint16_t *next_device_depth, const tsdf_camera_matrices *next_cam) {
     TSDF_REQUIRE(p && device_depth && cam && device_vertices, "tsdf_pipeline_step: null argument");
@@ -493,19 +504,20 @@
         if (rc != TSDF_OK) return rc;
     }
     if (p->ahead_depth && p->ahead_depth == device_depth && p->ahead_buf == b) {
-        if (hipEventQuery(p->ready[b]) != hipSuccess) {
+        if (!p->ahead_on_main && hipEventQuery(p->ready[b]) != hipSuccess) {
             if (tuning().pipe_host_wait) TSDF_HIP(hipEventSynchronize(p->ready[b]), "pipeline: wait for the frame filtered ahead");
             else TSDF_HIP(hipStreamWaitEvent(p->main, p->ready[b], 0), "pipeline: wait for the frame filtered ahead");
         }
     } else {
         if (p->ahead_depth) {
-            TSDF_HIP(hipStreamWaitEvent(p->main, p->ready[p->ahead_buf], 0), "pipeline: wait for the side stream");
+            if (!p->ahead_on_main) TSDF_HIP(hipStreamWaitEvent(p->main, p->ready[p->ahead_buf], 0), "pipeline: wait for the side stream");
             (void)tsdf_integrate_discard_prepared(p->volume);
         }
         rc = run_filter(p, device_depth, b, p->main);
         if (rc != TSDF_OK) return rc;
     }
     p->ahead_depth = nullptr;
+    p->ahead_on_main = p->ahead_in_cast = false;
     rc = tsdf_integrate_device_tiles(p->volume, p->filtered[b], W, H, cam->pose, cam->inv_pose, cam->k, cam->kinv, p->tile_max[b]);
     if (rc != TSDF_OK) return rc;
     bool late_release = false;
@@ -536,11 +548,35 @@
         p->ahead_buf = 1 - b;
         return TSDF_OK;
     };
+    const bool tighten_due = p->volume->occ_tighten_due && !p->volume->occ_dirty && !(p->flags & TSDF_PIPELINE_NO_TIGHTEN_AHEAD);
+    FusedFilter fused;
+    const bool one_stream = p->side && next_device_depth && !tighten_due && !p->exchange && tuning().pipe_one_stream && tuning().pipe_release == 0 &&
+                            bilateral_fusable(p->filter, next_device_depth, p->filtered[1 - b], (int)W, (int)H, p->tile_max[1 - b], &fused) &&
+                            raycast_takes_cells(p->volume, W, H, cam->pose, cam->kinv);
+    auto ahead_on_main = [&]() -> int {
+        const bool in_cast = p->volume->fused_filter.n_wgs == 0;
+        if (!in_cast) {
+            p->volume->fused_filter.n_wgs = 0;
+            const int rc_ = run_filter(p, next_device_depth, 1 - b, p->main);
+            if (rc_ != TSDF_OK) return rc_;
+        }
+        if (next_cam) {
+            const int rc_ = tsdf_integrate_prepare_device_tiles(p->volume, p->filtered[1 - b], W, H, next_cam->pose, next_cam->inv_pose, next_cam->k,
+                                                                next_cam->kinv, p->tile_max[1 - b], p->main);
+            if (rc_ != TSDF_OK) return rc_;
+        }
+        p->ahead_depth = next_device_depth;
+        p->ahead_buf = 1 - b;
+        p->ahead_on_main = true;
+        p->ahead_in_cast = in_cast;
+        return TSDF_OK;
+    };
     if (p->side) {
         const bool tighten_ahead = p->volume->occ_tighten_due && !p->volume->occ_dirty && !(p->flags & TSDF_PIPELINE_NO_TIGHTEN_AHEAD);
-        by_word = p->release_word && next_device_depth && !p->exchange && !tighten_ahead && tuning().pipe_release == 0 &&
+        by_word = !one_stream && p->release_word && next_device_depth && !p->exchange && !tighten_ahead && tuning().pipe_release == 0 &&
                   raycast_takes_cells(p->volume, W, H, cam->pose, cam->kinv);
-        if (by_word) {
+        if (one_stream) {
+        } else if (by_word) {
             p->release_seq++;
             p->volume->release_word = p->release_word;
             p->volume->release_value = p->release_seq;
@@ -554,18 +590,24 @@
             if (rc != TSDF_OK) return rc;
         }
         late_release = next_device_depth && !p->exchange && tuning().pipe_release == 1;
-        if (next_device_depth && !late_release) {
+        if (next_device_depth && !late_release && !one_stream) {
             rc = filter_ahead(p->done[b]);
             if (rc != TSDF_OK) return rc;
         }
     }
     if (!p->exchange) {
         p->volume->after_bulk = late_release ? p->bulk : nullptr;
+        if (one_stream) p->volume->fused_filter = fused;
         rc = tsdf_raycast_device(p->volume, W, H, cam->pose, cam->kinv, device_vertices, device_normals);
         p->volume->after_bulk = nullptr;
+        if (rc != TSDF_OK) p->volume->fused_filter.n_wgs = 0;
         if (rc != TSDF_OK) return rc;
         if (late_release) {
             rc = filter_ahead(p->bulk);
+            if (rc != TSDF_OK) return rc;
+        }
+        if (one_stream) {
+            rc = ahead_on_main();
             if (rc != TSDF_OK) return rc;
         }
     } else {
diff --git a/tsdf_amd/csrc/raycast.hip b/tsdf_amd/csrc/raycast.hip
--- a/tsdf_amd/csrc/raycast.hip
+++ b/tsdf_amd/csrc/raycast.hip
@@ -2,6 +2,7 @@
 #include <cmath>
 #include <cstdlib>
 
+#include "bilateral_tile.hpp"
 #include "common.hpp"
 
 namespace tsdf {
@@ -1093,16 +1094,19 @@
             std::stable_sort(list.begin(), list.end(), [&](const uint2 &a_, const uint2 &b_) { return depth_of(a_) < depth_of(b_); });
             TSDF_HIP(hipMemcpy(cc.bricks, list.data(), n_listed * sizeof(uint2), hipMemcpyHostToDevice), "cells sort");
         }
-        const dim3 cgrid((unsigned)tuning().ray_cells_grid + kShellWorkgroups);
+        const FusedFilter ff = v->fused_filter, no_ff = {};
+        v->fused_filter.n_wgs = 0;
+        const dim3 cgrid((unsigned)tuning().ray_cells_grid + kShellWorkgroups + ff.n_wgs);
         if (v->fast_div)
-            TSDF_LAUNCH_TIMED(v, 1, (cast_cells_kernel<SLAB, true>), cgrid, dim3(256), v->dist, v->g, rp, *cells, v->occ, v->t_table, cc, tail.best);
+            TSDF_LAUNCH_TIMED(v, 1, (cast_cells_kernel<SLAB, true>), cgrid, dim3(256), v->dist, v->g, rp, *cells, v->occ, v->t_table, cc, tail.best, ff);
         else
-            TSDF_LAUNCH_TIMED(v, 1, (cast_cells_kernel<SLAB, false>), cgrid, dim3(256), v->dist, v->g, rp, *cells, v->occ, v->t_table, cc, tail.best);
+            TSDF_LAUNCH_TIMED(v, 1, (cast_cells_kernel<SLAB, false>), cgrid, dim3(256), v->dist, v->g, rp, *cells, v->occ, v->t_table, cc, tail.best, ff);
         if (getenv("TSDF_DEBUG_CELLS_TWICE")) {
+            const dim3 cgrid2((unsigned)tuning().ray_cells_grid + kShellWorkgroups);
             if (v->fast_div)
-                TSDF_LAUNCH_TIMED(v, 2, (cast_cells_kernel<SLAB, true>), cgrid, dim3(256), v->dist, v->g, rp, *cells, v->occ, v->t_table, cc, tail.best);
+                TSDF_LAUNCH_TIMED(v, 2, (cast_cells_kernel<SLAB, true>), cgrid2, dim3(256), v->dist, v->g, rp, *cells, v->occ, v->t_table, cc, tail.best, no_ff);
             else
-                TSDF_LAUNCH_TIMED(v, 2, (cast_cells_kernel<SLAB, false>), cgrid, dim3(256), v->dist, v->g, rp, *cells, v->occ, v->t_table, cc, tail.best);
+                TSDF_LAUNCH_TIMED(v, 2, (cast_cells_kernel<SLAB, false>), cgrid2, dim3(256), v->dist, v->g, rp, *cells, v->occ, v->t_table, cc, tail.best, no_ff);
         }
         TSDF_HIP(hipGetLastError(), "cell-parallel cast failed");
         if (v->after_bulk) TSDF_HIP(hipEventRecord(v->after_bulk, v->stream), "process_ray: bulk kernel event");
diff --git a/tsdf_amd/csrc/raycast_cells.hpp b/tsdf_amd/csrc/raycast_cells.hpp
--- a/tsdf_amd/csrc/raycast_cells.hpp
+++ b/tsdf_amd/csrc/raycast_cells.hpp
@@ -443,11 +443,20 @@
 #endif
 __global__ __launch_bounds__(256) void cast_cells_kernel(const float *__restrict__ dist, const Geom g, const RayParams rp, const EntryParams ep,
                                                          const OccGrid occ, const float *__restrict__ t_table, const CellCast cc,
-                                                         uint64_t *__restrict__ best) {
+                                                         uint64_t *__restrict__ best, const FusedFilter ff) {
     __shared__ __attribute__((aligned(16))) float T[kTableLen];
     __shared__ float corner[4][128];
     __shared__ __attribute__((aligned(16))) int box_of[4][64][4];
     __shared__ int prefix[4][64];
+    if (ff.n_wgs && blockIdx.x >= gridDim.x - ff.n_wgs) {
+        static_assert(sizeof(T) >= kSimLds * sizeof(float) && sizeof(corner) >= 15 * 15 * sizeof(float) &&
+                      sizeof(box_of) >= (kBTile + 14) * (kBTile + 14) * sizeof(uint32_t), "the filter's LDS in the cast's arrays");
+        const uint32_t t = blockIdx.x - (gridDim.x - ff.n_wgs);
+        const BilateralLds lds = {nullptr, &corner[0][0], T, reinterpret_cast<uint32_t *>(&box_of[0][0][0]), reinterpret_cast<unsigned *>(&prefix[0][0])};
+        bilateral_tile<uint16_t, 7>(ff.in, ff.out, ff.width, ff.height, 7, ff.kernel, ff.similarity, ff.tile_max, t % ff.tiles_x, t / ff.tiles_x,
+                                    ff.tiles_x, lds);
+        return;
+    }
 #if TSDF_CELLS_SCAN_DECODE
     __shared__ uint32_t mark[4][64];
     mark[threadIdx.x >> 6][threadIdx.x & 63u] = 0u;
@@ -508,7 +517,7 @@
         va = voxel(lane);
         if (lane + 64u < 125u) vb = voxel(lane + 64u);
     };
-    const uint32_t n_waves = (gridDim.x - kShellWorkgroups) * 4u;
+    const uint32_t n_waves = (gridDim.x - ff.n_wgs - kShellWorkgroups) * 4u;
     uint32_t ei = (blockIdx.x - kShellWorkgroups) * 4u + wave;
     uint2 entry_next = ei < n_bricks ? cc.bricks[ei] : make_uint2(0u, 0u);
     float va_next, vb_next;
diff --git a/tsdf_amd/csrc/volume.hip b/tsdf_amd/csrc/volume.hip
--- a/tsdf_amd/csrc/volume.hip
+++ b/tsdf_amd/csrc/volume.hip
@@ -52,6 +52,7 @@
         u.weight_pack = num("TSDF_WEIGHT_PACK", 8);
         if (u.weight_pack != 0 && u.weight_pack != 16) u.weight_pack = 8;
         u.pipe_release = clamp(num("TSDF_PIPE_RELEASE", 0), 0, 2);
+        u.pipe_one_stream = num("TSDF_PIPE_ONE_STREAM", 1) != 0;
         u.pipe_host_wait = num("TSDF_PIPE_HOST_WAIT", 0) != 0;
         u.pipe_word_release = num("TSDF_PIPE_WORD_RELEASE", 0) != 0;
         u.event_scope = clamp(num("TSDF_EVENT_SCOPE", 2), 0, 2);
diff --git a/tsdf_amd/pipeline.py b/tsdf_amd/pipeline.py
--- a/tsdf_amd/pipeline.py
+++ b/tsdf_amd/pipeline.py
@@ -46,6 +46,11 @@
         check(lib.tsdf_pipeline_hit_buffers(self._h, C.byref(a), C.byref(b)))
         return a.value, b.value
 
+    def filtered_ahead(self):
+        f, t, inside = C.c_void_p(), C.c_void_p(), C.c_int()
+        check(lib.tsdf_pipeline_filtered_ahead(self._h, C.byref(f), C.byref(t), C.byref(inside)))
+        return f.value, t.value, bool(inside.value)
+
     def step(self, depth_ptr, camera, vertices_ptr, normals_ptr=None, next_depth_ptr=None, next_camera=None):
         cam = _matrices(camera)
         nxt = _matrices(next_camera) if (next_camera is not None and next_depth_ptr is not None) else None
```

After: 623,000, median of 6. About the same (+0.7%).
